# churchill-lab/alntools

Hardware: AMD Instinct MI355X
Metric: alignments/sec BAM->EC (100M PE reads, 8-hap) at 1/2/4/8 MI355X (higher is better)
Workload: dtype u32

## Files before the change

### alntools_amd/csrc/ecb.hip

```cpp
#include <hip/hip_runtime.h>

#include <algorithm>
#include <climits>
#include <cstddef>
#include <cstdarg>
#include <cstdio>
#include <cstring>
#include <cstdlib>
#include <memory>
#include <mutex>
#include <string>
#include <vector>

#include "../../include/ecb.h"

namespace {

typedef unsigned long long u64;
typedef unsigned int u32;
typedef unsigned short u16;

constexpr int TPB = 256;
constexpr u32 MAX_PROBE = 256;
constexpr u32 PENDING = 0xFFFFFFFFu;
// ... 50 lines not shown
__device__ __forceinline__ u64 arena_alloc(Counters* ctr, u64 arena_cap, u32 n, u32 hint) {
    const u32 R = arena_regions(arena_cap);
    const u64 per = arena_cap / R;
    for (u32 t = 0; t < R; ++t) {
        const u32 r = (hint + t) % R;
        const u64 at = atomicAdd(&ctr->arena_reg[r], (u64)n);
        if (at + n <= (u64)(r + 1) * per) return at;
    }
    return ~0ull;
}

__device__ __forceinline__ u32 fmix32(u32 h) {
    h ^= h >> 16; h *= 0x85EBCA6Bu;
    h ^= h >> 13; h *= 0xC2B2AE35u;
    h ^= h >> 16;
    return h;
}
__device__ __forceinline__ u64 pair_hash64(u32 locus, u32 mask) {
    const u32 h0 = fmix32(locus * 0x9E3779B1u + mask * 0x85EBCA77u + 0x7F4A7C15u);
    const u32 h1 = fmix32((h0 ^ locus) * 0xC2B2AE3Du + mask);
    return ((u64)h1 << 32) | h0;
}
__device__ __forceinline__ u64 finish_hash(u64 s0, u32 n) { return (s0 + ((u64)n << 32) + n) | 1ull; }

__device__ __forceinline__ bool rec_valid(u32 hf) {
    if (hf & 0x4u) return false;
    if (hf & 0x1u) {
        if ((hf & 0x80u) || !(hf & 0x2u) || (hf & (ECB_FLAG_MATE_OTHER_REF | ECB_FLAG_NEXT_POS_NEG))) return false;
    }
    return true;
}

enum { ST_NONE = 0, ST_LOOK, ST_HIT, ST_CREATED, ST_PENDING, ST_FULL, ST_OTHER, ST_STUCK };
enum { CMP_EQUAL = 0, CMP_DIFFERENT, CMP_INCOMPLETE, CMP_UNSURE };
struct SlotView { u32 n, off; uint2 p[INL]; };

__device__ __forceinline__ u64 fresh64(u64* p) { return atomicOr(p, 0ull); }
__device__ __forceinline__ void store_wt64(u64* p, u64 v) { __hip_atomic_store(p, v, __ATOMIC_RELAXED, __HIP_MEMORY_SCOPE_AGENT); }
__device__ __forceinline__ u64 pack2(uint2 v) { return ((u64)v.y << 32) | v.x; }
__device__ __forceinline__ uint2 unpack2(u64 v) { return make_uint2((u32)v, (u32)(v >> 32)); }
__device__ __forceinline__ void publish_key(Slot* s, u32 n1, u32 off) { store_wt64(reinterpret_cast<u64*>(&s->n1), ((u64)off << 32) | n1); }
__device__ __forceinline__ uint2 key_pair(const Slot& s, const uint2* arena, u32 i) { return i < INL ? s.pair[i] : arena[(u64)s.off + (i - INL)]; }
__device__ __forceinline__ uint2 key_pair_fresh(Slot* s, uint2* arena, u32 off, u32 i) {
    return unpack2(fresh64(reinterpret_cast<u64*>(i < INL ? &s->pair[i] : arena + ((u64)off + (i - INL)))));
}

__device__ __forceinline__ SlotView make_view(uint4 a, uint4 b, uint4 c, uint4 d) {
    SlotView v;
    v.n = a.z - 1u; v.off = a.w;
    v.p[0] = make_uint2(b.z, b.w); v.p[1] = make_uint2(c.x, c.y); v.p[2] = make_uint2(c.z, c.w);
    v.p[3] = make_uint2(d.x, d.y); v.p[4] = make_uint2(d.z, d.w);
    return v;
}
constexpr u32 RANKED_MAX = 16;
template <class F>
__device__ __forceinline__ void ranked_pairs(const SlotView& v, const uint2* arena, F&& emit) {
    const u32 sn = v.n;
    u32 X[RANKED_MAX], Y[RANKED_MAX];
#pragma unroll
    for (u32 i = 0; i < INL; ++i) { X[i] = i < sn ? v.p[i].x : 0xFFFFFFFFu; Y[i] = v.p[i].y; }
    if (sn <= INL) {
#pragma unroll
        for (u32 i = 0; i < INL; ++i) {
            u32 r = 0;
#pragma unroll
            for (u32 j = 0; j < INL; ++j) r += X[j] < X[i] ? 1u : 0u;
            if (i < sn) emit(r, X[i], Y[i]);
        }
    } else {
#pragma unroll
        for (u32 k = 0; k < RANKED_MAX - INL; ++k) {
            const uint2 t = INL + k < sn ? arena[(u64)v.off + k] : make_uint2(0xFFFFFFFFu, 0u);
            X[INL + k] = t.x; Y[INL + k] = t.y;
        }
#pragma unroll
        for (u32 i = 0; i < RANKED_MAX; ++i) {
            u32 r = 0;
#pragma unroll
            for (u32 j = 0; j < RANKED_MAX; ++j) r += X[j] < X[i] ? 1u : 0u;
            if (i < sn) emit(r, X[i], Y[i]);
        }
    }
}
constexpr u32 BIG_LDS = 2048;
template <class F>
__device__ __forceinline__ void ranked_pairs_wave(const Slot& s, const uint2* arena, u32 sn, u32* sx, u32 lane, F&& emit) {
    const bool in_lds = sn <= BIG_LDS;
    if (in_lds) {
        for (u32 i = lane; i < sn; i += 64) sx[i] = key_pair(s, arena, i).x;
        __builtin_amdgcn_fence(__ATOMIC_ACQ_REL, "wavefront");
        __builtin_amdgcn_wave_barrier();
    }
    for (u32 i = lane; i < sn; i += 64) {
        const uint2 pi = key_pair(s, arena, i);
        u32 r = 0;
        if (in_lds) {
            u32 j = 0;
            for (; j + 4u <= sn; j += 4u) {
                const uint4 v = *reinterpret_cast<const uint4*>(&sx[j]);
                r += (v.x < pi.x ? 1u : 0u) + (v.y < pi.x ? 1u : 0u) + (v.z < pi.x ? 1u : 0u) + (v.w < pi.x ? 1u : 0u);
            }
            for (; j < sn; ++j) r += sx[j] < pi.x ? 1u : 0u;
        } else {
            for (u32 j = 0; j < sn; ++j) r += key_pair(s, arena, j).x < pi.x;
        }
        emit(r, pi.x, pi.y);
    }
    if (in_lds) {
        __builtin_amdgcn_fence(__ATOMIC_ACQ_REL, "wavefront");
        __builtin_amdgcn_wave_barrier();
    }
}
template <class Cmp>
__device__ __forceinline__ int table_lookup(Slot* table, u64 cap_mask, u64 lo, u64& j, u32& probes, const Cmp& cmp, u32 abl = 0u, u32* first_inv_seen = nullptr) {
    for (; probes < MAX_PROBE; ++probes, j = (j + 1) & cap_mask) {
        Slot* s = table + j;
        const uint4* q = reinterpret_cast<const uint4*>(s);
        if (first_inv_seen) *first_inv_seen = 0u;
        uint4 a = q[0], b = a, c = a, d = a;
        if (!(abl & 16u)) { b = q[1]; c = q[2]; d = q[3]; }
        u64 clo = ((u64)a.y << 32) | a.x;
        if (clo == 0ull) {
            clo = atomicCAS(&s->lo, 0ull, lo);
            if (clo == 0ull) return ST_CREATED;
            if (clo == lo) return ST_PENDING;
            continue;
        }
        if (clo != lo) continue;
        if (a.z == 0u) return ST_PENDING;
        if (a.z == DEAD_KEY) continue;
        if (first_inv_seen) *first_inv_seen = b.y;
        if (abl & 8u) return ST_HIT;
        const int r = cmp.quick(make_view(a, b, c, d));
        if (r == CMP_EQUAL) return ST_HIT;
        if (r != CMP_DIFFERENT) return ST_PENDING;
    }
    return ST_FULL;
}
template <class Cmp>
__device__ __forceinline__ int table_settle(Slot* s, const Cmp& cmp) {
    for (u32 spin = 0; spin < SPIN_MAX; ++spin) {
        const u64 w = fresh64(reinterpret_cast<u64*>(&s->n1));
        const u32 n1 = (u32)w;
        if (n1 == DEAD_KEY) return ST_OTHER;
        if (n1) {
            const int r = cmp.full(s, n1 - 1u, (u32)(w >> 32));
            if (r == CMP_EQUAL) return ST_HIT;
            if (r == CMP_DIFFERENT) return ST_OTHER;
        }
        __builtin_amdgcn_s_sleep(4);
    }
    return ST_STUCK;
}

#ifndef ECB_RPL
#define ECB_RPL 8
#endif
constexpr int RPL = ECB_RPL;
static_assert(RPL == 8, "only 8 records per lane is validated (16 was measured: 233 VGPRs, 2 waves/SIMD, 11-25 % slower; it also needs a 32-bit ent[])");
constexpr int NG = RPL / 4;
constexpr int WT = 64 * RPL;
constexpr int NWAVE = TPB / 64;
struct StreamCold {
    uint2* arena; u64 arena_cap;
    u64* queue; u64 queue_cap;
    u64* resume;
    u32* wave_counts;
    u64* wave_arena;
    u64* timing;
    u64 chunk;
    u32 prev_rid;
    const int* pos; int2* rng; u32 n_loci, n_haps;
};
__device__ __forceinline__ void queue_defer(Counters* ctr, const StreamCold* C, u64 head) {
    const u32 st = (u32)((head * 0x9E3779B97F4A7C15ull) >> 58);
    static_assert(QSTRIPES == 64, "six bits of the hash pick the stripe");
    const u64 seg = C->queue_cap / QSTRIPES;
    const u64 qi = atomicAdd(&ctr->n_queue_s[st], 1ull);
    if (qi < seg) C->queue[(u64)st * seg + qi] = head; else atomicOr(&ctr->err, ERR_QUEUE);
}
#ifdef ECB_ABLATE_RT
#define ABL(A, bits) ((A).ablate & (bits))
#else
#define ABL(A, bits) 0u
#endif
struct StreamArgs {
    const u32* rid; const u32* loc; const u32* hf;
    u64 n;
    Slot* table; u64 cap_mask;
    Counters* ctr;
    u32* read_slot;
    u64 reads_hi;
    const StreamCold* cold;
    u32 ablate;
    const int* pos; int2* rng;
};
__device__ __forceinline__ u32 stream_tw(const u32* rid, const u32* loc, const u32* hf) { return (loc == rid + 512 && hf == rid + 1024) ? 1536u : 512u; }
#define A_TW(A) stream_tw((A).rid, (A).loc, (A).hf)
__host__ __device__ __forceinline__ u64 rec_at(u64 i, u32 tw) { return (i >> 9) * (u64)tw + (i & 511ull); }

__device__ __forceinline__ void wave_sync() {
    __builtin_amdgcn_fence(__ATOMIC_ACQ_REL, "wavefront");
    __builtin_amdgcn_wave_barrier();
}
template <int CTRL, int ROW_MASK>
__device__ __forceinline__ u32 dpp_add(u32 v) { return v + (u32)__builtin_amdgcn_update_dpp(0, (int)v, CTRL, ROW_MASK, 0xf, false); }
__device__ __forceinline__ u32 wave_incl_scan(u32 v) {
    v = dpp_add<0x111, 0xf>(v); v = dpp_add<0x112, 0xf>(v); v = dpp_add<0x114, 0xf>(v); v = dpp_add<0x118, 0xf>(v);
    v = dpp_add<0x142, 0xa>(v);
    v = dpp_add<0x143, 0xc>(v);
    return v;
}
__device__ __forceinline__ u32 wave_sum(u32 v) { return (u32)__builtin_amdgcn_readlane((int)wave_incl_scan(v), 63); }
__device__ __forceinline__ u32 lane_above(u32 v) { return (u32)__builtin_amdgcn_update_dpp(0, (int)v, 0x138, 0xf, 0xf, false); }
__device__ __forceinline__ int clamp04(int x, int, int) { return min(max(x, 0), 4); }

struct TileRegs { u32 rr[RPL], ll[RPL], hh[RPL]; };


#ifdef ECB_TIMING
#define TICK(i) do { const u64 t_ = __builtin_readcyclecounter(); tacc[i] += t_ - tlast; tlast = t_; } while (0)
#else
#define TICK(i) do { } while (0)
#endif

__device__ __forceinline__ u64 tile_head(const u32* rid, u64 b, u64 e, u32 rd, u32 tw) {
    while (b < e) { const u64 m = b + ((e - b) >> 1); if ((int)(rid[rec_at(m, tw)] - rd) < 0) b = m + 1; else e = m; }
    return b;
}
__device__ __forceinline__ void load_tile(const StreamArgs& A, u64 tb, u64 te, u32 lane, TileRegs& R) {
    typedef unsigned int u32x4 __attribute__((ext_vector_type(4)));
    tb = ((u64)(u32)__builtin_amdgcn_readfirstlane((int)(u32)(tb >> 32)) << 32) | (u32)__builtin_amdgcn_readfirstlane((int)(u32)tb);
    if (tb + (u64)WT <= te) {
        const u64 tbw = (tb >> 9) * (u64)A_TW(A);
        const char* pr = reinterpret_cast<const char*>(A.rid + tbw);
        const char* pl = reinterpret_cast<const char*>(A.loc + tbw);
        const char* ph = reinterpret_cast<const char*>(A.hf + tbw);
        const u32 off = lane * 16u;
#pragma unroll
        for (int g = 0; g < NG; ++g) {
            u32x4 v = __builtin_nontemporal_load(reinterpret_cast<const u32x4*>(pr + (off + (u32)g * 1024u)));
            R.rr[4 * g] = v.x; R.rr[4 * g + 1] = v.y; R.rr[4 * g + 2] = v.z; R.rr[4 * g + 3] = v.w;
            v = __builtin_nontemporal_load(reinterpret_cast<const u32x4*>(pl + (off + (u32)g * 1024u)));
            R.ll[4 * g] = v.x; R.ll[4 * g + 1] = v.y; R.ll[4 * g + 2] = v.z; R.ll[4 * g + 3] = v.w;
            v = __builtin_nontemporal_load(reinterpret_cast<const u32x4*>(ph + (off + (u32)g * 1024u)));
            R.hh[4 * g] = v.x; R.hh[4 * g + 1] = v.y; R.hh[4 * g + 2] = v.z; R.hh[4 * g + 3] = v.w;
        }
        return;
    }
#pragma unroll
    for (int g = 0; g < NG; ++g) {
        const u64 i0 = tb + (u64)g * 256 + 4u * lane;
#pragma unroll
        for (int j = 0; j < 4; ++j) {
            const bool in = i0 + j < te;
            R.rr[4 * g + j] = A.rid[rec_at(in ? i0 + j : te - 1, A_TW(A))];
            R.ll[4 * g + j] = in ? A.loc[rec_at(i0 + j, A_TW(A))] : 0u;
            R.hh[4 * g + j] = in ? A.hf[rec_at(i0 + j, A_TW(A))] : 0x4u;
        }
    }
}

__device__ __forceinline__ void load_pos(const int* pos, u64 tb, u64 te, u32 lane, int* P) {
    typedef int i32x4 __attribute__((ext_vector_type(4)));
    tb = ((u64)(u32)__builtin_amdgcn_readfirstlane((int)(u32)(tb >> 32)) << 32) | (u32)__builtin_amdgcn_readfirstlane((int)(u32)tb);
    if (tb + (u64)WT <= te) {
        const char* pp = reinterpret_cast<const char*>(pos + tb);
        const u32 off = lane * 16u;
#pragma unroll
        for (int g = 0; g < NG; ++g) {
            const i32x4 v = __builtin_nontemporal_load(reinterpret_cast<const i32x4*>(pp + (off + (u32)g * 1024u)));
            P[4 * g] = v.x; P[4 * g + 1] = v.y; P[4 * g + 2] = v.z; P[4 * g + 3] = v.w;
        }
        return;
    }
#pragma unroll
    for (int g = 0; g < NG; ++g) {
        const u64 i0 = tb + (u64)g * 256 + 4u * lane;
#pragma unroll
        for (int j = 0; j < 4; ++j) P[4 * g + j] = i0 + j < te ? pos[i0 + j] : 0;
    }
}

#define ECB_KS_SHORT 0
#define ECB_KS_PAR 0
namespace ks_std {
#include "k_stream.inc"
}
#undef ECB_KS_SHORT
#define ECB_KS_SHORT 1
namespace ks_short {
#include "k_stream.inc"
}
#undef ECB_KS_SHORT
#undef ECB_KS_PAR
#define ECB_KS_SHORT 0
#define ECB_KS_PAR 1
namespace ks_par {
#include "k_stream.inc"
}
#undef ECB_KS_PAR
#undef ECB_KS_SHORT

__global__ void k_init_resume(u64* resume, u64 slices, u64 chunk, Counters* ctr = nullptr) {
    const u64 b = blockIdx.x * (u64)blockDim.x + threadIdx.x;
    if (b < slices) { resume[2 * b] = b * chunk; resume[2 * b + 1] = b * chunk; }
    if (b == 0 && ctr) { ctr->n_queue = 0; ctr->full = 0; ctr->next_slice = 0; }
    if (b < QSTRIPES && ctr) ctr->n_queue_s[b] = 0;
}

__global__ __launch_bounds__(1024) void k_sum_counts(const u32* wave_counts, u64 waves, Counters* ctr, u32 verify, u64 offered, u64 queue_cap, const u32* d_last = nullptr) {
    __shared__ u64 s[3][16];
    u64 a = 0, v = 0, e = 0;
    for (u64 i = threadIdx.x; i < waves; i += 1024) { a += wave_counts[3 * i]; v += wave_counts[3 * i + 1]; e += wave_counts[3 * i + 2]; }
#pragma unroll
    for (int d = 32; d > 0; d >>= 1) { a += __shfl_xor(a, d); v += __shfl_xor(v, d); e += __shfl_xor(e, d); }
    if ((threadIdx.x & 63u) == 0) { s[0][threadIdx.x >> 6] = a; s[1][threadIdx.x >> 6] = v; s[2][threadIdx.x >> 6] = e; }
    __syncthreads();
    if (threadIdx.x == 0) {
        a = v = e = 0;
        for (int k = 0; k < 16; ++k) { a += s[0][k]; v += s[1][k]; e += s[2][k]; }
        if (verify) ctr->n_mismatch += e;
        else { ctr->all += offered; ctr->valid += v; ctr->n_ecs += e; ctr->n_probe_tiles += a; }
        if (d_last) ctr->last_rid = *d_last;
        u64 nq = 0;
        for (u32 st = 0; st < QSTRIPES; ++st) nq += min(ctr->n_queue_s[st], queue_cap / QSTRIPES);
        ctr->n_queue = nq;
    }
}
__global__ void k_queue_compact(const u64* queue, u64 queue_cap, const Counters* ctr, u64* out) {
    const u64 seg = queue_cap / QSTRIPES;
    u64 at = 0;
    for (u32 st = 0; st < blockIdx.x; ++st) at += min(ctr->n_queue_s[st], seg);
    const u64 n = min(ctr->n_queue_s[blockIdx.x], seg);
    for (u64 i = threadIdx.x; i < n; i += blockDim.x) out[at + i] = queue[(u64)blockIdx.x * seg + i];
}

constexpr u32 BIN_BITS = 14;
constexpr u32 MAX_BIN_BITS = 15;
constexpr u32 MIN_BIN_BITS = 11;
constexpr u32 MAX_BUCKETS = 8192;
static_assert(MAX_BIN_BITS <= 16, "a slot's index within its range is kept in 16 bits (k_part_scatter*, k_count_bins)");

constexpr int TPB_PART = 1024;
constexpr u32 PART_G = 512;
__device__ __forceinline__ u64 part_per(u64 n_reads, u64 G) { return (((n_reads + G - 1) / G) + 3ull) & ~3ull; }
__global__ __launch_bounds__(TPB_PART) void k_part_hist(const u32* read_slot, u64 n_reads, u32 n_buckets, u32 bb, u32* hist) {
    extern __shared__ u32 sh[];
    const u64 G = gridDim.x, g = blockIdx.x, per = part_per(n_reads, G);
    const u64 r0 = min(g * per, n_reads), r1 = min(r0 + per, n_reads);
    for (u32 b = threadIdx.x; b < n_buckets; b += TPB_PART) sh[b] = 0;
    __syncthreads();
    const u64 a0 = min((r0 + 3) & ~3ull, r1), a1 = max(r1 & ~3ull, a0);
    for (u64 r = r0 + threadIdx.x; r < a0; r += TPB_PART) { const u32 s = read_slot[r]; if (s != PENDING) atomicAdd(&sh[s >> bb], 1u); }
    for (u64 r = a0 + 4ull * threadIdx.x; r < a1; r += 4ull * TPB_PART) {
        const uint4 v = *reinterpret_cast<const uint4*>(read_slot + r);
        if (v.x != PENDING) atomicAdd(&sh[v.x >> bb], 1u);
        if (v.y != PENDING) atomicAdd(&sh[v.y >> bb], 1u);
        if (v.z != PENDING) atomicAdd(&sh[v.z >> bb], 1u);
        if (v.w != PENDING) atomicAdd(&sh[v.w >> bb], 1u);
    }
    for (u64 r = a1 + threadIdx.x; r < r1; r += TPB_PART) { const u32 s = read_slot[r]; if (s != PENDING) atomicAdd(&sh[s >> bb], 1u); }
    __syncthreads();
    for (u32 b = threadIdx.x; b < n_buckets; b += TPB_PART) hist[(u64)b * G + g] = sh[b];
}

__global__ __launch_bounds__(TPB_PART) void k_part_scatter(const u32* read_slot, u64 n_reads, u32 n_buckets, u32 bb, const u32* offs,
                                                      u16* pairs) {
    extern __shared__ u32 sh[];
    const u64 G = gridDim.x, g = blockIdx.x, per = part_per(n_reads, G);
    const u64 r0 = min(g * per, n_reads), r1 = min(r0 + per, n_reads);
    for (u32 b = threadIdx.x; b < n_buckets; b += TPB_PART) sh[b] = offs[(u64)b * G + g];
    __syncthreads();
    for (u64 rb = r0; rb < r1; rb += 4 * TPB_PART) {
        u32 s[4], pos[4];
        u64 r[4];
#pragma unroll
        for (int k = 0; k < 4; ++k) {
            r[k] = rb + (u64)k * TPB_PART + threadIdx.x;
            s[k] = r[k] < r1 ? read_slot[r[k]] : PENDING;
        }
#pragma unroll
        for (int k = 0; k < 4; ++k) if (s[k] != PENDING) pos[k] = atomicAdd(&sh[s[k] >> bb], 1u);
#pragma unroll
        for (int k = 0; k < 4; ++k) if (s[k] != PENDING) pairs[pos[k]] = (u16)(s[k] & ((1u << bb) - 1u));
    }
}

constexpr u32 STAGE = 8 * TPB_PART;
constexpr u32 STAGE_MAX_BUCKETS = 4096;
__global__ __launch_bounds__(TPB_PART) void k_part_scatter_staged(const u32* read_slot, u64 n_reads, u32 n_buckets, u32 bb, const u32* offs,
                                                             u16* pairs) {
    extern __shared__ u32 sh[];
    u32 *cnt = sh, *start = sh + n_buckets, *gcur = sh + 2 * n_buckets;
    u32* stage = sh + 3 * n_buckets;
    __shared__ u32 s_wave[TPB_PART / 64];
    const u64 G = gridDim.x, g = blockIdx.x, per = part_per(n_reads, G);
    const u64 r0 = min(g * per, n_reads), r1 = min(r0 + per, n_reads);
    const u32 tid = threadIdx.x, lane = tid & 63u, w = tid >> 6;
    const u32 bpt = (n_buckets + TPB_PART - 1) / TPB_PART;
    for (u32 b = tid; b < n_buckets; b += TPB_PART) gcur[b] = offs[(u64)b * G + g];
    for (u64 rb = r0; rb < r1; rb += STAGE) {
        for (u32 b = tid; b < n_buckets; b += TPB_PART) cnt[b] = 0;
        __syncthreads();
        u32 s[8], lr[8];
#pragma unroll
        for (int k4 = 0; k4 < 2; ++k4) {
            const u64 r = rb + ((u64)k4 * TPB_PART + tid) * 4u;
            if (r + 4 <= r1) {
                const uint4 v = *reinterpret_cast<const uint4*>(read_slot + r);
                s[4 * k4] = v.x; s[4 * k4 + 1] = v.y; s[4 * k4 + 2] = v.z; s[4 * k4 + 3] = v.w;
            } else {
#pragma unroll
                for (int j = 0; j < 4; ++j) s[4 * k4 + j] = r + j < r1 ? read_slot[r + j] : PENDING;
            }
        }
#pragma unroll
        for (int k = 0; k < 8; ++k) if (s[k] != PENDING) lr[k] = atomicAdd(&cnt[s[k] >> bb], 1u);
        __syncthreads();
        u32 mine = 0;
        for (u32 j = 0; j < bpt; ++j) { const u32 b = tid * bpt + j; mine += b < n_buckets ? cnt[b] : 0u; }
        const u32 incl = wave_incl_scan(mine);
        if (lane == 63) s_wave[w] = incl;
        __syncthreads();
        u32 run = incl - mine;
        for (u32 k = 0; k < w; ++k) run += s_wave[k];
        for (u32 j = 0; j < bpt; ++j) { const u32 b = tid * bpt + j; if (b < n_buckets) { start[b] = run; run += cnt[b]; } }
        __syncthreads();
#pragma unroll
        for (int k = 0; k < 8; ++k)
            if (s[k] != PENDING) stage[start[s[k] >> bb] + lr[k]] = s[k];
        __syncthreads();
        u32 n_here = 0;
        for (u32 k = 0; k < TPB_PART / 64; ++k) n_here += s_wave[k];
        for (u32 i = tid; i < n_here; i += TPB_PART) {
            const u32 e = stage[i];
            const u32 b = e >> bb;
            pairs[gcur[b] + (i - start[b])] = (u16)(e & ((1u << bb) - 1u));
        }
        __syncthreads();
        for (u32 b = tid; b < n_buckets; b += TPB_PART) gcur[b] += cnt[b];
    }
}

constexpr int TPB_COUNT = 1024;
struct CountWork { u32 bucket, start, end, shared; };
__global__ __launch_bounds__(1024) void k_build_work(const u32* offs, u32 G, const u64* total, u32 n_buckets, u32 piece, CountWork* work, u32 max_work, u32* n_work) {
    __shared__ u32 s_w[16];
    __shared__ u32 s_carry;
    const u32 tid = threadIdx.x, lane = tid & 63u, w = tid >> 6;
    if (tid == 0) s_carry = 0;
    __syncthreads();
    for (u32 b0 = 0; b0 < n_buckets; b0 += 1024) {
        const u32 b = b0 + tid;
        u32 s0 = 0, s1 = 0, np = 0;
        if (b < n_buckets) { s0 = offs[(u64)b * G]; s1 = b + 1 < n_buckets ? offs[(u64)(b + 1) * G] : (u32)*total; }
        const u32 len = s1 - s0;
        const bool cut = len > piece + piece / 2;
        if (len) np = cut ? (len + piece - 1) / piece : 1u;
        const u32 incl = wave_incl_scan(np);
        if (lane == 63) s_w[w] = incl;
        __syncthreads();
        u32 at = s_carry + incl - np, tot = 0;
        for (u32 k = 0; k < 16; ++k) { if (k < w) at += s_w[k]; tot += s_w[k]; }
        for (u32 k = 0; k < np; ++k)
            if (at + k < max_work) work[at + k] = cut ? CountWork{b, s0 + k * piece, min(s0 + (k + 1) * piece, s1), 1u} : CountWork{b, s0, s1, 0u};
        __syncthreads();
        if (tid == 0) s_carry += tot;
        __syncthreads();
    }
    if (tid == 0) *n_work = min(s_carry, max_work);
}
struct CompactSink { u32* list; u64 max_list; u64* n_list; u32* bitmap; u64 n_bits; uint2* list_fn; };
__global__ __launch_bounds__(TPB_COUNT) void k_count_bins(const u16* pairs, const CountWork* work, const u32* n_work, u32 bb, Slot* table, CompactSink sink) {
    extern __shared__ u32 cnt[];
    const u32 N_BINS = 1u << bb;
    if (blockIdx.x >= *n_work) return;
    const CountWork wk = work[blockIdx.x];
    const u32 b = wk.bucket, lane = threadIdx.x & 63u;
    const u32 start = wk.start, end = wk.end;
    for (u32 q = threadIdx.x; q < N_BINS; q += TPB_COUNT) cnt[q] = 0;
    __syncthreads();
    auto add = [&](u32 bin, bool have) {
        const u64 hm = __ballot(have);
        if (!hm) return;
        const u32 v = (u32)__builtin_amdgcn_readlane((int)bin, __ffsll((long long)hm) - 1);
        const bool same = have && bin == v;
        const u64 m = __ballot(same);
        if (__popcll(m) >= 8) {
            if (lane == (u32)(__ffsll((long long)m) - 1)) atomicAdd(&cnt[v], (u32)__popcll(m));
            if (have && !same) atomicAdd(&cnt[bin], 1u);
        } else if (have) {
            atomicAdd(&cnt[bin], 1u);
        }
    };
    const u32 a0 = min((start + 7u) & ~7u, end), a1 = max(end & ~7u, a0);
    { const u32 i = start + threadIdx.x; const bool have = i < a0; add(have ? (u32)pairs[i] : 0u, have); }
    { const u32 i = a1 + threadIdx.x; const bool have = i < end; add(have ? (u32)pairs[i] : 0u, have); }
    for (u32 i0 = a0; i0 < a1; i0 += 32 * TPB_COUNT) {
        uint4 pv[4];
#pragma unroll
        for (int k = 0; k < 4; ++k) {
            const u32 i = i0 + (k * TPB_COUNT + threadIdx.x) * 8u;
            pv[k] = i < a1 ? *reinterpret_cast<const uint4*>(pairs + i) : make_uint4(0u, 0u, 0u, 0u);
        }
#pragma unroll
        for (int k = 0; k < 4; ++k) {
            const bool have = i0 + (k * TPB_COUNT + threadIdx.x) * 8u < a1;
            const u32 w[4] = {pv[k].x, pv[k].y, pv[k].z, pv[k].w};
#pragma unroll
            for (int j = 0; j < 8; ++j) add((w[j >> 1] >> (16 * (j & 1))) & 0xFFFFu, have);
        }
    }
    __syncthreads();
    const bool once = sink.list && !wk.shared;
    u32 mine = 0;
    for (u32 q = threadIdx.x; q < N_BINS; q += TPB_COUNT) {
        const u32 c = cnt[q];
        u32 first = 0;
        if (once) first = c != 0u;
        else if (c) {
            Slot* s = table + (((u64)b << bb) | q);
            if (wk.shared) first = atomicAdd(&s->count, c) == 0u;
            else { s->count += c; first = 1u; }
        }
        if (sink.list && !once) cnt[q] = first;
        mine += first;
    }
    if (!sink.list) return;
    __shared__ u32 s_wtot[TPB_COUNT / 64];
    __shared__ u64 s_base;
    const u32 incl = wave_incl_scan(mine);
    if (lane == 63) s_wtot[threadIdx.x >> 6] = incl;
    __syncthreads();
    if (threadIdx.x == 0) {
        u32 run = 0;
        for (int k = 0; k < TPB_COUNT / 64; ++k) { const u32 c = s_wtot[k]; s_wtot[k] = run; run += c; }
        s_base = run ? atomicAdd(sink.n_list, (u64)run) : 0ull;
    }
    __syncthreads();
    u64 at = s_base + s_wtot[threadIdx.x >> 6] + (incl - mine);
    if (once) {
        for (u32 q0 = threadIdx.x; q0 < N_BINS; q0 += 8 * TPB_COUNT) {
            u32 c[8];
            uint2 vk[8], vc[8];
#pragma unroll
            for (int k = 0; k < 8; ++k) { const u32 q = q0 + k * TPB_COUNT; c[k] = q < N_BINS ? cnt[q] : 0u; }
#pragma unroll
            for (int k = 0; k < 8; ++k)
                if (c[k]) {
                    const Slot* sl = table + (((u64)b << bb) | (q0 + k * TPB_COUNT));
                    vk[k] = *reinterpret_cast<const uint2*>(&sl->n1); vc[k] = *reinterpret_cast<const uint2*>(&sl->count);
                }
#pragma unroll
            for (int k = 0; k < 8; ++k) {
                if (!c[k]) continue;
                const u64 i = ((u64)b << bb) | (q0 + k * TPB_COUNT);
                table[i].count = vc[k].x + c[k];
                if (at < sink.max_list) {
                    sink.list[at] = (u32)i;
                    if (sink.list_fn) {
                        const u32 f = ~vc[k].y;
                        sink.list_fn[at] = make_uint2(f, vk[k].x - 1u);
                        if (f < sink.n_bits) atomicOr(&sink.bitmap[f >> 5], 1u << (f & 31u));
                    }
                }
                ++at;
            }
        }
        return;
    }
    for (u32 q = threadIdx.x; q < N_BINS; q += TPB_COUNT) {
        if (!cnt[q]) continue;
        const u64 i = ((u64)b << bb) | q;
        if (at < sink.max_list) {
            const Slot* s = table + i;
            sink.list[at] = (u32)i;
            if (sink.list_fn) {
                const u32 f = ~s->first_inv;
                sink.list_fn[at] = make_uint2(f, s->n1 - 1u);
                if (f < sink.n_bits) atomicOr(&sink.bitmap[f >> 5], 1u << (f & 31u));
            }
        }
        ++at;
    }
}

__global__ __launch_bounds__(TPB) void k_slow_len(const u32* rid, u64 n, const u64* queue, u64 nq, u64* len, u32 tw) {
    const u64 q = blockIdx.x;
    if (q >= nq) return;
    __shared__ u64 s_end;
    const u64 h = queue[q];
    const u32 r0 = rid[rec_at(h, tw)];
    if (threadIdx.x == 0) s_end = n;
    __syncthreads();
    for (u64 b = h; b < n; b += TPB) {
        const u64 i = b + threadIdx.x;
        if (i < n && rid[rec_at(i, tw)] != r0) atomicMin(&s_end, i);
        __syncthreads();
        const bool found = (s_end != n);
        __syncthreads();
        if (found) break;
    }
    __syncthreads();
    if (threadIdx.x == 0) len[q] = s_end - h;
}

struct SlowArgs {
    const u32* rid; const u32* loc; const u32* hf;
    const u64* queue; const u64* len; const u64* scr_off;
    u32* scr_key; u32* scr_mask;
    u32 n_loci, n_haps;
    Slot* table; u64 cap_mask;
    uint2* arena; u64 arena_cap;
    Counters* ctr;
    u32* read_slot; u64 reads_hi;
    u64* requeue; u64* n_requeue;
    u32 verify;
};

__device__ __forceinline__ u64 slow_probe_start(u32 lc, u64 cap2) { return __umul64hi((u64)(lc * 0x9E3779B1u) << 32, cap2); }

constexpr u32 SLOW_LDS = 4096;
template <bool IN_LDS> __device__ __forceinline__ u32 slow_ld(const u32* p) {
    if constexpr (IN_LDS) return *p; else return __hip_atomic_load(p, __ATOMIC_RELAXED, __HIP_MEMORY_SCOPE_AGENT);
}
template <bool IN_LDS>
__device__ __forceinline__ void slow_body(const SlowArgs& A, u32* key, u32* msk, const u64 q, const u64 h, const u64 L) {
    const u32 tid = threadIdx.x, lane = tid & 63u;
    const u64 cap2 = 2 * L;
    if (IN_LDS) {
        for (u32 p = tid; p < (u32)cap2; p += TPB) { key[p] = 0; msk[p] = 0; }
        __syncthreads();
    }
    __shared__ u64 s_acc[TPB / 64];
    __shared__ u32 s_n[TPB / 64];
    __shared__ u64 s_lo, s_j;
    __shared__ u32 s_np, s_st, s_n1, s_off, s_cnt, s_diff, s_inc, s_probes;

    for (u64 i = tid; i < L; i += TPB) {
        const u32 f = A.hf[rec_at(h + i, A_TW(A))];
        if (!rec_valid(f)) continue;
        const u32 lc = A.loc[rec_at(h + i, A_TW(A))], hap = (f >> ECB_HAP_SHIFT) & 0xFFu;
        if (lc >= A.n_loci || hap >= A.n_haps) { atomicOr(&A.ctr->err, ERR_RANGE); continue; }
        u64 p = slow_probe_start(lc, cap2);
        for (;;) {
            const u32 old = atomicCAS(&key[p], 0u, lc + 1u);
            if (old == 0u || old == lc + 1u) { atomicOr(&msk[p], 1u << hap); break; }
            if (++p == cap2) p = 0;
        }
    }
    if (!IN_LDS) __threadfence();
    __syncthreads();
    u64 a0 = 0;
    u32 np = 0;
    for (u64 p = tid; p < cap2; p += TPB) {
        const u32 k = slow_ld<IN_LDS>(&key[p]);
        if (k) {
            const u32 m = slow_ld<IN_LDS>(&msk[p]);
            ++np;
            a0 += pair_hash64(k - 1u, m);
        }
    }
#pragma unroll
    for (int d = 32; d > 0; d >>= 1) a0 += __shfl_xor(a0, d);
    np = wave_sum(np);
    if (lane == 0) { s_acc[tid >> 6] = a0; s_n[tid >> 6] = np; }
    __syncthreads();
    const u32 r0 = A.rid[rec_at(h, A_TW(A))];
    if (tid == 0) {
        a0 = 0; np = 0;
        for (int w = 0; w < TPB / 64; ++w) { a0 += s_acc[w]; np += s_n[w]; }
        s_np = np; s_lo = finish_hash(a0, np); s_j = s_lo & A.cap_mask; s_probes = 0; s_cnt = 0;
        if ((u64)r0 >= A.reads_hi) { atomicOr(&A.ctr->err, ERR_CONTRACT); s_st = ST_NONE; }
        else s_st = ST_PENDING;
    }
    __syncthreads();
    np = s_np;
    auto same_key = [&]() -> int {
        for (u32 spin = 0; spin < SPIN_MAX; ++spin) {
            __syncthreads();
            if (tid == 0) {
                const u64 w = fresh64(reinterpret_cast<u64*>(&A.table[s_j].n1));
                s_n1 = (u32)w; s_off = (u32)(w >> 32); s_diff = 0; s_inc = 0;
            }
            __syncthreads();
            const u32 n1 = s_n1;
            if (n1 == DEAD_KEY) return CMP_DIFFERENT;
            if (n1 == 0u) { __builtin_amdgcn_s_sleep(8); continue; }
            const u32 n = n1 - 1u;
            if (n != np) return CMP_DIFFERENT;
            Slot* sl = A.table + s_j;
            bool diff = false, inc = false;
            for (u32 i = tid; i < n && !diff && !inc; i += TPB) {
                u64* src = reinterpret_cast<u64*>(i < INL ? &sl->pair[i] : A.arena + ((u64)s_off + (i - INL)));
                uint2 pr = unpack2(*src);
                if (pr.y == 0u) pr = unpack2(fresh64(src));
                if (pr.y == 0u) { inc = true; break; }
                diff = true;
                if (pr.x < A.n_loci) {
                    u64 p = slow_probe_start(pr.x, cap2);
                    for (u64 t = 0; t < cap2; ++t) {
                        const u32 k = slow_ld<IN_LDS>(&key[p]);
                        if (k == pr.x + 1u) { diff = slow_ld<IN_LDS>(&msk[p]) != pr.y; break; }
                        if (k == 0u) break;
                        if (++p == cap2) p = 0;
                    }
                }
            }
            if (diff) atomicOr(&s_diff, 1u);
            if (inc) atomicOr(&s_inc, 1u);
            __syncthreads();
            if (s_diff) return CMP_DIFFERENT;
            if (!s_inc) return CMP_EQUAL;
            __builtin_amdgcn_s_sleep(8);
        }
        return CMP_INCOMPLETE;
    };
    if (A.verify) {
        if (s_st != ST_NONE) {
            if (tid == 0) s_j = A.read_slot[r0];
            __syncthreads();
            const bool same = s_j != (u64)PENDING && same_key() == CMP_EQUAL;
            if (tid == 0 && !same) atomicAdd(&A.ctr->n_mismatch, 1ull);
        }
    } else {
        for (u32 round = 0; round < 4 * MAX_PROBE && s_st == ST_PENDING; ++round) {
            __syncthreads();
            if (tid == 0) {
                u64 j = s_j; u32 probes = s_probes;
                struct Defer { __device__ int quick(const SlotView&) const { return CMP_UNSURE; } };
                const int st = table_lookup(A.table, A.cap_mask, s_lo, j, probes, Defer());
                s_j = j; s_probes = probes; s_st = (u32)st; s_off = 0; s_n1 = 0;
                if (st == ST_CREATED) {
                    u64 off = 0;
                    if (np > INL) off = arena_alloc(A.ctr, A.arena_cap, np - INL, blockIdx.x);
                    atomicAdd(&A.ctr->n_ecs, 1ull);
                    s_off = (u32)off;
                    if (off == ~0ull) { atomicOr(&A.ctr->err, ERR_ARENA); s_n1 = DEAD_KEY; }
                } else if (st == ST_FULL) {
                    A.requeue[atomicAdd(A.n_requeue, 1ull)] = h;
                }
            }
            __syncthreads();
            if (s_st == ST_PENDING) {
                const int r = same_key();
                __syncthreads();
                if (tid == 0) {
                    if (r == CMP_EQUAL) { s_st = ST_HIT; A.read_slot[r0] = (u32)s_j; atomicMax(&A.table[s_j].first_inv, ~r0); }
                    else if (r == CMP_INCOMPLETE) { s_st = ST_NONE; atomicOr(&A.ctr->err, ERR_INTERNAL); }
                    else { s_j = (s_j + 1) & A.cap_mask; s_probes += 1; if (s_probes >= MAX_PROBE) { s_st = ST_FULL; A.requeue[atomicAdd(A.n_requeue, 1ull)] = h; } }
                }
// ... 24 lines not shown
    if (!IN_LDS) for (u64 p = tid; p < cap2; p += TPB) {
        if (slow_ld<IN_LDS>(&key[p])) { key[p] = 0; msk[p] = 0; }
    }
}
__global__ __launch_bounds__(TPB) void k_slow(SlowArgs A) {
    extern __shared__ u32 sh_scr[];
    const u64 q = blockIdx.x;
    const u64 h = A.queue[q], L = A.len[q];
    if (2 * L <= (u64)SLOW_LDS) slow_body<true>(A, sh_scr, sh_scr + SLOW_LDS, q, h, L);
    else slow_body<false>(A, A.scr_key + A.scr_off[q], A.scr_mask + A.scr_off[q], q, h, L);
}

__global__ void k_rehash(const Slot* old_t, u64 old_cap, Slot* new_t, u64 new_mask, u32* new_of_old) {
    for (u64 i = blockIdx.x * (u64)blockDim.x + threadIdx.x; i < old_cap; i += (u64)gridDim.x * blockDim.x) {
        const Slot s = old_t[i];
        if (!s.n1) continue;
        u64 j = s.lo & new_mask;
        for (;; j = (j + 1) & new_mask) {
            if (atomicCAS(&new_t[j].lo, 0ull, s.lo) == 0ull) {
                Slot t = s;
                uint4* d = reinterpret_cast<uint4*>(new_t + j);
                const uint4* v = reinterpret_cast<const uint4*>(&t);
                d[1] = v[1]; d[2] = v[2]; d[3] = v[3];
                new_t[j].off = s.off; new_t[j].n1 = s.n1;
                new_of_old[i] = (u32)j;
                break;
            }
        }
    }
}

__global__ void k_remap_read_slot(u32* read_slot, u64 n_reads, const u32* new_of_old) {
    for (u64 r = blockIdx.x * (u64)blockDim.x + threadIdx.x; r < n_reads; r += (u64)gridDim.x * blockDim.x) {
        const u32 os = read_slot[r];
        if (os != PENDING) read_slot[r] = new_of_old[os];
    }
}

constexpr int TPB_COMPACT = 1024;
__global__ __launch_bounds__(TPB_COMPACT) void k_compact(const Slot* table, u64 cap, u32* list, u64 max_list, u64* n_list,
                                                         u32* bitmap, u64 n_bits, uint2* list_fn) {
    __shared__ u32 s_w[TPB_COMPACT / 64];
    __shared__ u64 s_base;
    const u32 tid = threadIdx.x, lane = tid & 63u, w = tid >> 6;
    for (u64 b = (u64)blockIdx.x * 4 * TPB_COMPACT; b < cap; b += (u64)gridDim.x * 4 * TPB_COMPACT) {
        u32 occ = 0, off[4], tot = 0;
#pragma unroll
        for (int k = 0; k < 4; ++k) {
            const u64 i = b + (u64)k * TPB_COMPACT + tid;
            const bool o = i < cap && table[i].n1 != 0u;
            const u64 m = __ballot(o);
            off[k] = tot + __builtin_amdgcn_mbcnt_hi((u32)(m >> 32), __builtin_amdgcn_mbcnt_lo((u32)m, 0u));
            tot += (u32)__popcll(m);
            occ |= (u32)o << k;
        }
        if (lane == 0) s_w[w] = tot;
        __syncthreads();
        if (tid == 0) {
            u32 run = 0;
            for (int k = 0; k < TPB_COMPACT / 64; ++k) { const u32 c = s_w[k]; s_w[k] = run; run += c; }
            s_base = run ? atomicAdd(n_list, (u64)run) : 0ull;
        }
        __syncthreads();
        const u64 base = s_base + s_w[w];
#pragma unroll
        for (int k = 0; k < 4; ++k)
            if ((occ >> k & 1u) && base + off[k] < max_list) {
                const u64 i = b + (u64)k * TPB_COMPACT + tid;
                list[base + off[k]] = (u32)i;
                if (list_fn) {
                    const u32 f = ~table[i].first_inv;
                    list_fn[base + off[k]] = make_uint2(f, table[i].n1 - 1u);
                    if (f < n_bits) atomicOr(&bitmap[f >> 5], 1u << (f & 31u));
                }
            }
        __syncthreads();
    }
}

__global__ void k_list_fn(const Slot* table, const u32* list, u64 max_list, const u64* n_list, u64* n_out, u32* bitmap, u64 n_bits, uint2* list_fn) {
    const u64 e = blockIdx.x * (u64)blockDim.x + threadIdx.x;
    const u64 n = *n_list;
    if (e == 0) *n_out = n;
    if (e >= n || e >= max_list) return;
    const Slot* s = table + list[e];
    const u32 f = ~s->first_inv;
    list_fn[e] = make_uint2(f, s->n1 - 1u);
    if (f < n_bits) atomicOr(&bitmap[f >> 5], 1u << (f & 31u));
}

constexpr u32 MAX_PARTS = 64;
__device__ __forceinline__ u32 part_of(u64 lo, u32 n_parts) { return (u32)((lo >> 40) % n_parts); }

constexpr u32 PARTS_PER_BLOCK = 16 * TPB;
__global__ __launch_bounds__(TPB) void k_parts_count(const Slot* table, const u32* list, u64 n, u32 n_parts, u64* cnt) {
    __shared__ u32 ce[MAX_PARTS], cp[MAX_PARTS];
    if (threadIdx.x < MAX_PARTS) { ce[threadIdx.x] = 0; cp[threadIdx.x] = 0; }
    __syncthreads();
    const u64 e0 = blockIdx.x * (u64)PARTS_PER_BLOCK, e1 = min(e0 + PARTS_PER_BLOCK, n);
    for (u64 eb = e0; eb < e1; eb += TPB) {
        const u64 e = eb + threadIdx.x;
        u32 q = MAX_PARTS, np = 0;
        if (e < e1) { const Slot& s = table[list[e]]; q = part_of(s.lo, n_parts); np = s.n1 - 1u; }
        for (u32 t = 0; t < n_parts; ++t) {
            const u64 m = __ballot(q == t);
            if (!m) continue;
            const u32 tot = wave_sum(q == t ? np : 0u);
            if ((threadIdx.x & 63u) == 0) { atomicAdd(&ce[t], (u32)__popcll(m)); atomicAdd(&cp[t], tot); }
        }
    }
    __syncthreads();
    if (threadIdx.x < n_parts) {
        if (ce[threadIdx.x]) atomicAdd(&cnt[threadIdx.x], (u64)ce[threadIdx.x]);
        if (cp[threadIdx.x]) atomicAdd(&cnt[n_parts + threadIdx.x], (u64)cp[threadIdx.x]);
    }
}
constexpr u32 EXPORT_SMALL = RANKED_MAX;
__global__ __launch_bounds__(TPB) void k_parts_export(const Slot* table, const u32* list, u64 n, const uint2* arena, u32 n_parts,
                                                      u64* cur, const u64* pair_base, Entry* out_e, uint2* out_p, u32 read_base,
                                                      u64* big, u32* n_big) {
    __shared__ u32 ce[MAX_PARTS], cp[MAX_PARTS];
    __shared__ u64 be[MAX_PARTS], bp[MAX_PARTS];
    const u32 lane = threadIdx.x & 63u;
    const u64 e0 = blockIdx.x * (u64)PARTS_PER_BLOCK, e1 = min(e0 + PARTS_PER_BLOCK, n);
    for (int pass = 0; pass < 2; ++pass) {
        if (threadIdx.x < MAX_PARTS) { ce[threadIdx.x] = 0; cp[threadIdx.x] = 0; }
        __syncthreads();
        for (u64 eb = e0; eb < e1; eb += TPB) {
            const u64 e = eb + threadIdx.x;
            uint4 sa = make_uint4(0u, 0u, 1u, 0u), sb = sa, sc = sa, sd = sa;
            u32 q = MAX_PARTS, re = 0, rp = 0, sn = 0;
            if (e < e1) {
                const uint4* sl = reinterpret_cast<const uint4*>(table + list[e]);
                sa = sl[0]; sb = sl[1]; sc = sl[2]; sd = sl[3];
                q = part_of(((u64)sa.y << 32) | sa.x, n_parts); sn = sa.z - 1u;
            }
            for (u32 t = 0; t < n_parts; ++t) {
                const bool mine = q == t;
                const u64 m = __ballot(mine);
                if (!m) continue;
                const u32 v = mine ? sn : 0u, incl = wave_incl_scan(v);
                const u32 tot = (u32)__builtin_amdgcn_readlane((int)incl, 63);
                u32 b_e = 0, b_p = 0;
                if (lane == 0) { b_e = atomicAdd(&ce[t], (u32)__popcll(m)); b_p = atomicAdd(&cp[t], tot); }
                b_e = (u32)__builtin_amdgcn_readfirstlane((int)b_e); b_p = (u32)__builtin_amdgcn_readfirstlane((int)b_p);
                if (mine) { re = b_e + __builtin_amdgcn_mbcnt_hi((u32)(m >> 32), __builtin_amdgcn_mbcnt_lo((u32)m, 0u)); rp = b_p + incl - v; }
            }
            if (pass == 1 && e < e1) {
                const u64 po = bp[q] + rp;
                if (sn <= EXPORT_SMALL) {
                    ranked_pairs(make_view(sa, sb, sc, sd), arena, [&](u32 r, u32 x, u32 y) { out_p[po + r] = make_uint2(x, y); });
                } else {
                    const u32 bi = atomicAdd(n_big, 1u);
                    big[2 * (u64)bi] = po; big[2 * (u64)bi + 1] = ((u64)list[e] << 32) | sn;
                }
                Entry en;
                en.lo = ((u64)sa.y << 32) | sa.x; en.reserved = 0; en.count = sb.x;
                en.first_inv = ~(~sb.y + read_base);
                en.off = (u32)(po - pair_base[q]); en.n = sn;
                out_e[be[q] + re] = en;
            }
        }
        __syncthreads();
        if (pass == 0 && threadIdx.x < n_parts) {
            be[threadIdx.x] = ce[threadIdx.x] ? atomicAdd(&cur[threadIdx.x], (u64)ce[threadIdx.x]) : 0ull;
            bp[threadIdx.x] = cp[threadIdx.x] ? atomicAdd(&cur[n_parts + threadIdx.x], (u64)cp[threadIdx.x]) : 0ull;
        }
        __syncthreads();
    }
}
__global__ __launch_bounds__(TPB) void k_parts_sort_big(const Slot* table, const uint2* arena, const u64* big, u32 n_big, uint2* out_p) {
    __shared__ __attribute__((aligned(16))) u32 sx[TPB / 64][BIG_LDS];
    const u32 b = (blockIdx.x * TPB + threadIdx.x) >> 6, lane = threadIdx.x & 63u;
    if (b >= n_big) return;
    const u64 po = big[2 * (u64)b];
    const u32 n = (u32)big[2 * (u64)b + 1];
    const Slot& s = table[big[2 * (u64)b + 1] >> 32];
    ranked_pairs_wave(s, arena, n, sx[threadIdx.x >> 6], lane, [&](u32 r, u32 x, u32 y) { out_p[po + r] = make_uint2(x, y); });
}
__global__ void k_adopt(const Entry* ent, u64 n, const uint2* pairs, Slot* table, u64 slot_base, u32 arena_base) {
    const u64 e = blockIdx.x * (u64)blockDim.x + threadIdx.x;
    if (e >= n) return;
    const Entry en = ent[e];
    Slot s{};
    s.lo = en.lo; s.n1 = en.n + 1u; s.off = arena_base + en.off + INL; s.count = en.count; s.first_inv = en.first_inv;
    for (u32 i = 0; i < INL && i < en.n; ++i) s.pair[i] = pairs[(u64)en.off + i];
    table[slot_base + e] = s;
}

struct ListCmp {
    const uint2* inc; u32 n; uint2* arena;
    __device__ __forceinline__ int quick(const SlotView& v) const { return v.n != n ? CMP_DIFFERENT : CMP_UNSURE; }
    __device__ __noinline__ int full(Slot* s, u32 sn, u32 off) const {
        if (sn != n) return CMP_DIFFERENT;
        bool same = true, inc_ = false;
        for (u32 i = 0; i < n && same; ++i) {
            const uint2 a = key_pair_fresh(s, arena, off, i), b = inc[i];
            inc_ |= a.y == 0u;
            same = a.x == b.x && a.y == b.y;
        }
        if (same) return CMP_EQUAL;
        if (inc_) return CMP_INCOMPLETE;
        for (u32 i = 0; i < n; ++i) {
            const uint2 a = key_pair_fresh(s, arena, off, i);
            if (a.y == 0u) return CMP_INCOMPLETE;
            bool found = false;
            for (u32 k = 0; k < n && !found; ++k) found = inc[k].x == a.x && inc[k].y == a.y;
            if (!found) return CMP_DIFFERENT;
        }
        return CMP_EQUAL;
    }
};
constexpr u32 MERGE_PER_BLOCK = 2 * TPB;
struct MergeDesc { const Entry* ent; const uint2* pairs; u64 n, n_pairs; };
__global__ __launch_bounds__(TPB) void k_merge(const MergeDesc* D, Slot* table, u64 cap_mask, uint2* arena, u64 arena_cap, Counters* ctr,
                                               u32* list, u64 list_cap, u64* n_list) {
    const MergeDesc d = D[blockIdx.y];
    const Entry* const ent = d.ent; const uint2* const pairs = d.pairs;
    const u64 n = d.n, n_pairs = d.n_pairs;
    if (blockIdx.x * (u64)MERGE_PER_BLOCK >= n) return;
    __shared__ u32 s_new;
    __shared__ u32 s_found[MERGE_PER_BLOCK];
    __shared__ u32 s_nfound;
    __shared__ u64 s_lbase;
    if (threadIdx.x == 0) { s_new = 0; s_nfound = 0; }
    __syncthreads();
    const u32 lane = threadIdx.x & 63u;
    const u64 e0 = blockIdx.x * (u64)MERGE_PER_BLOCK, e1 = min(e0 + MERGE_PER_BLOCK, n);
    u32 my_new = 0;
    for (u64 eb = e0; eb < e1; eb += TPB) {
        const u64 e = eb + threadIdx.x;
        const bool on = e < e1;
        Entry s{};
        if (on) s = ent[e];
        const bool ok = on && (u64)s.off + s.n <= n_pairs && s.lo != 0ull;
        if (on && !ok) atomicOr(&ctr->err, ERR_CONTRACT);
        ListCmp cmp{pairs + s.off, s.n, arena};
        u64 j = s.lo & cap_mask;
        u32 probes = 0;
        int st = ST_NONE;
        if (ok) st = table_lookup(table, cap_mask, s.lo, j, probes, cmp);
        bool created = false;
        for (u32 round = 0;; ++round) {
            const u64 cm = __ballot(st == ST_CREATED);
            if (cm) {
                const bool cr = st == ST_CREATED;
                const u32 want = cr && s.n > INL ? s.n - INL : 0u;
                u64 at = 0;
                if (__ballot(want != 0u)) {
                    const u32 incl = wave_incl_scan(want);
                    const u32 total = (u32)__builtin_amdgcn_readlane((int)incl, 63);
                    if (lane == 0) at = arena_alloc(ctr, arena_cap, total, (blockIdx.y * gridDim.x + blockIdx.x) * (TPB / 64) + (threadIdx.x >> 6));
                    at = ((u64)(u32)__builtin_amdgcn_readfirstlane((int)(u32)(at >> 32)) << 32) | (u32)__builtin_amdgcn_readfirstlane((int)(u32)at);
                    if (at == ~0ull) { if (lane == 0) atomicOr(&ctr->err, ERR_ARENA); }
                    else at += incl - want;
                }
                my_new += (u32)__popcll(cm);
                if (list) {
                    const int first = __ffsll((long long)cm) - 1;
                    u32 lb = 0;
                    if ((int)lane == first) lb = atomicAdd(&s_nfound, (u32)__popcll(cm));
                    lb = (u32)__builtin_amdgcn_readlane((int)lb, first);
                    if (cr) s_found[lb + __builtin_amdgcn_mbcnt_hi((u32)(cm >> 32), __builtin_amdgcn_mbcnt_lo((u32)cm, 0u))] = (u32)j;
                }
                if (cr) {
                    const bool dead = at == ~0ull;
                    if (!dead)
                        for (u32 t = 0; t < s.n; ++t) {
                            uint2* dst = t < INL ? &table[j].pair[t] : arena + (at + (t - INL));
                            store_wt64(reinterpret_cast<u64*>(dst), pack2(pairs[(u64)s.off + t]));
                        }
                    publish_key(table + j, dead ? DEAD_KEY : s.n + 1u, (u32)at);
                    st = ST_HIT; created = true;
                }
            }
            if (!__ballot(st == ST_PENDING)) break;
            if (round >= 64u) { if (st == ST_PENDING) { atomicOr(&ctr->err, ERR_INTERNAL); st = ST_NONE; } break; }
            if (st == ST_PENDING) {
                const int r = table_settle(table + j, cmp);
                if (r == ST_HIT) st = ST_HIT;
                else if (r == ST_STUCK) { atomicOr(&ctr->err, ERR_INTERNAL); st = ST_NONE; }
                else { j = (j + 1) & cap_mask; ++probes; st = table_lookup(table, cap_mask, s.lo, j, probes, cmp); }
            }
        }
        (void)created;
        if (st == ST_FULL) atomicAdd(&ctr->n_queue, 1ull);
        else if (st == ST_HIT) {
            atomicAdd(&table[j].count, s.count);
            atomicMax(&table[j].first_inv, s.first_inv);
        }
    }
    if (lane == 0 && my_new) atomicAdd(&s_new, my_new);
    __syncthreads();
    if (threadIdx.x == 0 && s_new) atomicAdd(&ctr->n_ecs, (u64)s_new);
    if (list) {
        if (threadIdx.x == 0) s_lbase = s_nfound ? atomicAdd(n_list, (u64)s_nfound) : 0ull;
        __syncthreads();
        for (u32 i = threadIdx.x; i < s_nfound; i += TPB) if (s_lbase + i < list_cap) list[s_lbase + i] = s_found[i];
    }
}

constexpr u32 BM_LINE = 16;
inline u64 bitmap_words(u64 n_bits) { return ((n_bits + 31) / 32 + BM_LINE) / BM_LINE * BM_LINE; }
__global__ void k_popc(const u32* in, u64 n_lines, u32* out) {
    const u64 i = blockIdx.x * (u64)blockDim.x + threadIdx.x;
    if (i >= n_lines) return;
    const uint4* q = reinterpret_cast<const uint4*>(in + i * BM_LINE);
    u32 c = 0;
#pragma unroll
    for (int k = 0; k < (int)BM_LINE / 4; ++k) { const uint4 v = q[k]; c += __popc(v.x) + __popc(v.y) + __popc(v.z) + __popc(v.w); }
    out[i] = c;
}
__device__ __forceinline__ u32 bit_rank(const u32* bitmap, const u32* lprefix, u32 f) {
    const uint4* q = reinterpret_cast<const uint4*>(bitmap + ((f >> 5) & ~(BM_LINE - 1u)));
    const uint4 v0 = q[0], v1 = q[1], v2 = q[2], v3 = q[3];
    const u32 w[BM_LINE] = {v0.x, v0.y, v0.z, v0.w, v1.x, v1.y, v1.z, v1.w, v2.x, v2.y, v2.z, v2.w, v3.x, v3.y, v3.z, v3.w};
    const u32 k = (f >> 5) & (BM_LINE - 1u), below = (1u << (f & 31u)) - 1u;
    u32 r = lprefix[f >> 9];
    static_assert(BM_LINE == 16, "f >> 9: 512 bits per line");
#pragma unroll
    for (u32 i = 0; i < BM_LINE; ++i) r += __popc(w[i] & (i < k ? 0xFFFFFFFFu : i == k ? below : 0u));
    return r;
}

constexpr int SCB_TPB = 1024, SCB_ITEMS = 16, SCB = SCB_TPB * SCB_ITEMS;
constexpr u64 SC_AGG = 1ull << 62, SC_PFX = 2ull << 62, SC_VAL = (1ull << 62) - 1ull;
inline u64 scan_blocks(u64 n) { return std::max<u64>(1, (n + SCB - 1) / SCB); }
inline u64 scan_words(u64 n) { return 2 * (scan_blocks(n) + 2); }
__global__ __launch_bounds__(SCB_TPB) void k_scan_lb(const u32* in, u64 n, u32* out, u64* st, u64 nb, u64* d_total, u32 stride, u32* last32) {
    __shared__ u64 s_b, s_excl;
    __shared__ u32 s_w[SCB_TPB / 64];
    const u32 tid = threadIdx.x, lane = tid & 63u, w = tid >> 6;
    if (tid == 0) s_b = atomicAdd(reinterpret_cast<unsigned long long*>(&st[nb]), 1ull);
    __syncthreads();
    const u64 b = s_b;
    if (b >= nb) return;
    const u64 base = b * SCB + (u64)tid * SCB_ITEMS;
    u32 v[SCB_ITEMS];
    const bool whole = base + SCB_ITEMS <= n;
    if (stride == 1u && whole && (reinterpret_cast<uintptr_t>(in) & 15u) == 0u) {
#pragma unroll
        for (int k = 0; k < SCB_ITEMS / 4; ++k) {
            const uint4 q = reinterpret_cast<const uint4*>(in + base)[k];
            v[4 * k] = q.x; v[4 * k + 1] = q.y; v[4 * k + 2] = q.z; v[4 * k + 3] = q.w;
        }
    } else {
#pragma unroll
        for (int k = 0; k < SCB_ITEMS; ++k) v[k] = base + k < n ? in[(base + k) * stride] : 0u;
    }
    u32 s = 0;
#pragma unroll
    for (int k = 0; k < SCB_ITEMS; ++k) s += v[k];
    const u32 incl = wave_incl_scan(s);
    if (lane == 63) s_w[w] = incl;
    __syncthreads();
    u32 before = 0, tot = 0;
#pragma unroll
    for (u32 k = 0; k < SCB_TPB / 64; ++k) { const u32 c = s_w[k]; if (k < w) before += c; tot += c; }
    if (w == 0) {
        u64 excl = 0;
        if (lane == 0) __hip_atomic_store(&st[b], (b == 0 ? SC_PFX : SC_AGG) | (u64)tot, __ATOMIC_RELAXED, __HIP_MEMORY_SCOPE_AGENT);
        if (b > 0) {
            long long t = (long long)b - 1;
            for (u32 spins = 0; spins < (1u << 24);) {
                const long long idx = t - (long long)lane;
                const u64 x = idx >= 0 ? __hip_atomic_load(&st[idx], __ATOMIC_RELAXED, __HIP_MEMORY_SCOPE_AGENT) : SC_PFX;
                const u64 ready = __ballot(x != 0ull), pfx = __ballot(x >= SC_PFX);
                u64 take = 0;
                if (pfx) {
                    const int p = __ffsll((long long)pfx) - 1;
                    const u64 need = p == 63 ? ~0ull : (1ull << (p + 1)) - 1ull;
                    if ((ready & need) == need) take = need;
                } else if (ready == ~0ull) take = ~0ull;
                if (!take) { ++spins; __builtin_amdgcn_s_sleep(1); continue; }
                u64 val = (take >> lane & 1ull) ? (x & SC_VAL) : 0ull;
#pragma unroll
                for (int d = 32; d > 0; d >>= 1) val += __shfl_xor(val, d);
                excl += val;
                if (pfx) break;
                t -= 64;
            }
            if (lane == 0) __hip_atomic_store(&st[b], SC_PFX | ((excl + tot) & SC_VAL), __ATOMIC_RELAXED, __HIP_MEMORY_SCOPE_AGENT);
        }
        if (lane == 0) {
            s_excl = excl;
            if (b + 1 == nb && d_total) *d_total = excl + tot;
            if (b + 1 == nb && last32) *last32 = (u32)(excl + tot);
        }
    }
    __syncthreads();
    u32 run = (u32)s_excl + before + incl - s;
    if (whole && (reinterpret_cast<uintptr_t>(out) & 15u) == 0u) {
#pragma unroll
        for (int k = 0; k < SCB_ITEMS / 4; ++k) {
            uint4 q;
            q.x = run; run += v[4 * k]; q.y = run; run += v[4 * k + 1]; q.z = run; run += v[4 * k + 2]; q.w = run; run += v[4 * k + 3];
            reinterpret_cast<uint4*>(out + base)[k] = q;
        }
    } else {
#pragma unroll
        for (int k = 0; k < SCB_ITEMS; ++k) { if (base + k < n) out[base + k] = run; run += v[k]; }
    }
}
inline hipError_t scan_launch(hipStream_t st, const u32* in, u64 n, u32* out, u32* scratch, u64* d_total, u32 stride = 1, u32* last32 = nullptr) {
    const u64 nb = scan_blocks(n);
    u64* words = reinterpret_cast<u64*>(scratch);
    hipError_t e = hipMemsetAsync(words, 0, ((nb + 1) * 8 + 15) & ~15ull, st);
    if (e != hipSuccess) return e;
    k_scan_lb<<<(unsigned)nb, SCB_TPB, 0, st>>>(in, n, out, words, nb, d_total, stride, last32);
    return hipGetLastError();
}

__global__ void k_rank(const u32* list, const uint2* list_fn, u64 n, u64 n_bits, const u32* bitmap, const u32* wprefix,
                       uint2* ord2) {
    const u64 e = blockIdx.x * (u64)blockDim.x + threadIdx.x;
    if (e >= n) return;
    const u32 si = list[e];
    const uint2 fn = list_fn[e];
    const u32 f = fn.x;
    if (f >= n_bits) return;
    const u32 r = bit_rank(bitmap, wprefix, f);
    if (r >= n) return;
    ord2[r] = make_uint2(si, fn.y);
}
__global__ void k_slot_ranks(const u32* order, u64 n, u32* rank_of_slot) {
    const u64 r = blockIdx.x * (u64)blockDim.x + threadIdx.x;
    if (r < n) rank_of_slot[order[r]] = (u32)r;
}

constexpr u32 EMIT_SMALL = RANKED_MAX;
__global__ __launch_bounds__(TPB) void k_emit_small(const Slot* table, const uint2* ord2, u32* order, u64 n, const uint2* arena,
                                                     const u32* indptr, int* indices, int* data, int* counts,
                                                     u32 n_loci, u32 n_haps, u32* big, u32* n_big, Counters* ctr) {
    __shared__ u32 sx[TPB / 64][64 * EMIT_SMALL], sy[TPB / 64][64 * EMIT_SMALL];
    const u64 e = (u64)blockIdx.x * TPB + threadIdx.x;
    const u32 lane = threadIdx.x & 63u, w = threadIdx.x >> 6;
    const bool have = e < n;
    const u64 hm = __ballot(have);
    if (!hm) return;
    uint4 a = make_uint4(0u, 0u, 1u, 0u), b = a, c = a, d = a;
    u32 dst = 0;
    if (have) {
        const u32 si = ord2[e].x;
        order[e] = si;
        const uint4* q = reinterpret_cast<const uint4*>(table + si);
        a = q[0]; b = q[1]; c = q[2]; d = q[3];
        counts[e] = (int)b.x;
        dst = indptr[e];
    }
    const SlotView v = make_view(a, b, c, d);
    const bool is_big = have && v.n > EMIT_SMALL;
    if (is_big) big[atomicAdd(n_big, 1u)] = (u32)e;
    const u32 base = (u32)__builtin_amdgcn_readfirstlane((int)dst);
    const u32 end = (u32)__builtin_amdgcn_readlane((int)(dst + v.n), 63 - __builtin_clzll(hm));
    const bool staged = __ballot(is_big) == 0ull && end - base <= 64u * EMIT_SMALL;
    bool bad = false;
    if (!is_big)
        ranked_pairs(v, arena, [&](u32 r, u32 x, u32 y) {
            if (staged) { const u32 at = min(dst - base + r, 64u * EMIT_SMALL - 1u); sx[w][at] = x; sy[w][at] = y; }
            else { indices[dst + r] = (int)x; data[dst + r] = (int)y; }
            bad |= x >= n_loci || (y >> n_haps) != 0u;
        });
    if (staged) {
        wave_sync();
        for (u32 i = lane; i < end - base; i += 64u) { indices[base + i] = (int)sx[w][i]; data[base + i] = (int)sy[w][i]; }
    }
    if (bad) atomicOr(&ctr->err, ERR_RANGE);
}
__global__ __launch_bounds__(TPB) void k_emit_big(const Slot* table, const u32* order, const u32* big, const u32* n_big,
                                                   const uint2* arena, const u32* indptr, int* indices, int* data,
                                                   u32 n_loci, u32 n_haps, Counters* ctr) {
    __shared__ __attribute__((aligned(16))) u32 sx[TPB / 64][BIG_LDS];
    const u32 lane = threadIdx.x & 63u, w = threadIdx.x >> 6, nb = *n_big;
    bool bad = false;
    for (u32 b = (blockIdx.x * TPB + threadIdx.x) >> 6; b < nb; b += (gridDim.x * TPB) >> 6) {
        const u32 e = big[b];
        const Slot& s = table[order[e]];
        const u32 dst = indptr[e];
        ranked_pairs_wave(s, arena, s.n1 - 1u, sx[w], lane, [&](u32 r, u32 x, u32 y) {
            indices[dst + r] = (int)x;
            data[dst + r] = (int)y;
            bad |= x >= n_loci || (y >> n_haps) != 0u;
        });
    }
    if (bad) atomicOr(&ctr->err, ERR_RANGE);
}

constexpr u32 MS_FILE_BITS = 32 - ECB_CELL_BITS;
__host__ __device__ __forceinline__ u32 ms_swz(u32 meta) { return ((meta & ((1u << ECB_CELL_BITS) - 1u)) << MS_FILE_BITS) | (meta >> ECB_CELL_BITS); }
__host__ __device__ __forceinline__ u32 ms_unswz(u32 s) { return (s >> MS_FILE_BITS) | (s << ECB_CELL_BITS); }
__host__ __device__ __forceinline__ u64 ms_swz_key(u64 key) { return (key & 0xFFFFFFFF00000000ull) | ms_swz((u32)key); }
__global__ void k_ms_keys(const u32* read_slot, const u32* rank_of_slot, const u32* meta, u64 n, u64* keys, u32* vals) {
    const u64 i = blockIdx.x * (u64)blockDim.x + threadIdx.x;
    if (i < n) { keys[i] = ((u64)rank_of_slot[read_slot[i]] << 32) | ms_swz(meta[i]); vals[i] = (u32)i; }
}
__global__ void k_ms_swz_keys(u64* keys, u64 n) {
    const u64 i = blockIdx.x * (u64)blockDim.x + threadIdx.x;
    if (i < n) keys[i] = ms_swz_key(keys[i]);
}
__global__ void k_run_heads(const u64* keys, u64 n, u32* flag) {
    const u64 i = blockIdx.x * (u64)blockDim.x + threadIdx.x;
    if (i < n) flag[i] = (i == 0 || keys[i] != keys[i - 1]) ? 1u : 0u;
}
__global__ void k_ms_emit(const u64* keys, const u32* vals, const u32* flag, const u32* pos, u64 n, u32 n_out,
                          u64* okey, u32* ofirst, u32* ostart) {
    const u64 i = blockIdx.x * (u64)blockDim.x + threadIdx.x;
    if (i < n && flag[i]) { okey[pos[i]] = (keys[i] & 0xFFFFFFFF00000000ull) | ms_unswz((u32)keys[i]); ofirst[pos[i]] = vals[i]; ostart[pos[i]] = (u32)i; }
    if (i == 0) ostart[n_out] = (u32)n;
}
__global__ void k_ms_split(const u64* okey, const u32* ostart, const u32* ocount, u64 n, u32* ec, u32* meta, u32* count) {
    const u64 i = blockIdx.x * (u64)blockDim.x + threadIdx.x;
    if (i < n) { ec[i] = (u32)(okey[i] >> 32); meta[i] = (u32)okey[i]; count[i] = ocount ? ocount[i] : ostart[i + 1] - ostart[i]; }
}
__global__ void k_export_keys(const Slot* table, const u32* order, u64 n, u64* out) {
    const u64 e = blockIdx.x * (u64)blockDim.x + threadIdx.x;
    if (e < n) out[e] = table[order[e]].lo;
}
__global__ void k_row_keys(const u32* indptr, const int* indices, const int* data, u64 n, u64* out) {
    const u64 e = blockIdx.x * (u64)blockDim.x + threadIdx.x;
    if (e >= n) return;
    const u32 a = indptr[e], z = indptr[e + 1];
    u64 acc = 0;
    for (u32 i = a; i < z; ++i) acc += pair_hash64((u32)indices[i], (u32)data[i]);
    out[e] = finish_hash(acc, z - a);
}
__global__ void k_set_global_rank(const u64* keys, const int* indptr, const int* indices, const int* data, u64 n,
                                  const Slot* table, u64 cap_mask, const uint2* arena, u32* grank) {
    const u64 e = blockIdx.x * (u64)blockDim.x + threadIdx.x;
    if (e >= n) return;
    const u64 lo = keys[e];
    const u32 r0 = (u32)indptr[e], rn = (u32)indptr[e + 1] - r0;
    u64 j = lo & cap_mask;
    for (u64 probe = 0; probe <= cap_mask; ++probe, j = (j + 1) & cap_mask) {
        const Slot& s = table[j];
        if (s.lo == 0ull) return;
        if (s.lo != lo || s.n1 != rn + 1u) continue;
        bool same = true;
        for (u32 i = 0; i < rn && same; ++i) {
            const uint2 pr = key_pair(s, arena, i);
            u32 a = 0, b = rn;
            while (a < b) { const u32 m = (a + b) >> 1; if ((u32)indices[r0 + m] < pr.x) a = m + 1; else b = m; }
            same = a < rn && (u32)indices[r0 + a] == pr.x && (u32)data[r0 + a] == pr.y;
        }
        if (same) { grank[j] = (u32)e; return; }
    }
}
__global__ void k_ms_out(const u64* okey, const u32* ofirst, const u32* ostart, u64 n, u32 read_base, u64* key, u32* count, u32* first) {
    const u64 i = blockIdx.x * (u64)blockDim.x + threadIdx.x;
    if (i < n) { key[i] = okey[i]; count[i] = ostart[i + 1] - ostart[i]; first[i] = ofirst[i] + read_base; }
}
__global__ void k_ms_combine(const u64* keys, const u32* idx, const u32* flag, const u32* pos, u64 n, const u32* cnt_in, const u32* first_in,
                             u64* okey, u32* ocount, u32* ofirst) {
    const u64 i = blockIdx.x * (u64)blockDim.x + threadIdx.x;
    if (i >= n) return;
    const u32 o = pos[i] - (flag[i] ? 0u : 1u);
    if (flag[i]) okey[o] = (keys[i] & 0xFFFFFFFF00000000ull) | ms_unswz((u32)keys[i]);
    atomicAdd(&ocount[o], cnt_in[idx[i]]);
    atomicMin(&ofirst[o], first_in[idx[i]]);
}


__device__ __forceinline__ u64 lower_bound_u64(const u64* a, u64 n, u64 v) {
    u64 lo = 0, hi = n;
    while (lo < hi) { const u64 m = (lo + hi) >> 1; if (a[m] < v) lo = m + 1; else hi = m; }
    return lo;
}
constexpr u32 CVU_PIECE = 1536;
constexpr u32 CVU_MAX = 3072;
constexpr u32 CVU_TSZ = 4096;
constexpr u32 CVU_TPB = 512;
constexpr u32 CVU_K = CVU_MAX / CVU_TPB;
constexpr u32 CVB_ERR_PTR = 1u, CVB_ERR_EC = 2u, CVB_ERR_ORDER = 4u;
__global__ void k_cvb_last(const int* cscptr, u32 n_loci, u32 n_haps, int* last) {
    const u32 h = threadIdx.x;
    if (h < n_haps) last[h] = cscptr[(u64)h * (n_loci + 1) + n_loci];
}
__global__ void k_cvu_colsum(const int* cscptr, u32 n_loci, u32 n_haps, u32* S, u32* err) {
    const u64 l = blockIdx.x * (u64)blockDim.x + threadIdx.x;
    if (l > n_loci) return;
    u32 sum = 0, bad = 0;
    for (u32 h = 0; h < n_haps; ++h) {
        const int* ptr = cscptr + (u64)h * (n_loci + 1);
        const int v = ptr[l];
        if (v < 0 || (l == 0 && v != 0) || (l > 0 && ptr[l - 1] > v)) bad = CVB_ERR_PTR;
        sum += (u32)v;
    }
    S[l] = sum;
    if (bad) atomicOr(err, bad);
}
__global__ void k_cvu_pieces(const u32* S, u32 n_loci, u32* pieces) {
    const u64 l = blockIdx.x * (u64)blockDim.x + threadIdx.x;
    if (l >= n_loci) return;
    const u32 n = S[l + 1] - S[l];
    pieces[l] = n <= CVU_PIECE + CVU_PIECE / 2 ? (n ? 1u : 0u) : (n + CVU_PIECE - 1u) / CVU_PIECE;
}
__global__ void k_cvu_items(const u32* pieces, const u32* pbase, u32 n_loci, u32* item_col) {
    const u64 l = blockIdx.x * (u64)blockDim.x + threadIdx.x;
    if (l >= n_loci) return;
    const u32 n = pieces[l], at = pbase[l];
    for (u32 r = 0; r < n; ++r) item_col[at + r] = (u32)l;
}
__device__ __forceinline__ u32 cvu_width(u32 n_ecs, u32 np) { return (u32)(((u64)n_ecs + np - 1u) / np); }
__global__ void k_cvu_bounds(const int* cscptr, const int* cscidx, const u64* hs, const u32* pieces, const u32* pbase, const u32* item_col,
                             u32 n_items, u32 n_loci, u32 n_haps, u32 n_ecs, u32* bnd) {
    const u64 t = blockIdx.x * (u64)blockDim.x + threadIdx.x;
    if (t >= (u64)n_items * n_haps) return;
    const u32 i = (u32)(t / n_haps), h = (u32)(t % n_haps);
    const u32 l = item_col[i], np = pieces[l], r = i - pbase[l];
    const int* ptr = cscptr + (u64)h * (n_loci + 1);
    const u64 nh = hs[h + 1] - hs[h];
    u64 a = min((u64)(u32)ptr[l], nh), b = min((u64)(u32)ptr[l + 1], nh);
    if (r) {
        const u64 lo = (u64)r * cvu_width(n_ecs, np);
        const int* base = cscidx + hs[h];
        while (a < b) { const u64 m = a + ((b - a) >> 1); if ((u64)(u32)base[m] < lo) a = m + 1; else b = m; }
    }
    bnd[t] = (u32)a;
}
__device__ __forceinline__ bool cvb_contains(const int* cscptr, const int* cscidx, const u64* hs, u32 n_loci, u32 hh, u32 l, u32 e) {
    const int* p = cscptr + (u64)hh * (n_loci + 1);
    const u64 nh = hs[hh + 1] - hs[hh];
    u64 a = min((u64)(u32)p[l], nh), b = min((u64)(u32)p[l + 1], nh);
    const int* base = cscidx + hs[hh];
    while (a < b) { const u64 m = a + ((b - a) >> 1); const u32 v = (u32)base[m]; if (v < e) a = m + 1; else if (v > e) b = m; else return true; }
    return false;
}
template <bool EMIT>
__global__ __launch_bounds__(CVU_TPB) void k_cvu_union(const int* cscptr, const int* cscidx, const u64* hs, const u32* pieces, const u32* pbase,
                                                       const u32* item_col, const u32* bnd, u32 n_items, u32 n_loci, u32 n_haps, u32 n_ecs,
                                                       u32* colcnt, const u32* colbase, u32* colcur, u64 nnz, u64* keys, u32* vals, u32* err) {
    __shared__ u32 tkey[CVU_TSZ];
    __shared__ u32 tmask[CVU_TSZ];
    __shared__ u32 seg[64];
    __shared__ u32 segp[33];
    __shared__ u64 shs[32];
    __shared__ u32 s_n, s_base;
    const u32 i = blockIdx.x;
    const u32 l = item_col[i], np = pieces[l], r = i - pbase[l];
    const u32 w = cvu_width(n_ecs, np);
    const u32 e_lo = (u32)min((u64)r * w, (u64)n_ecs), e_hi = r + 1u == np ? n_ecs : (u32)min((u64)(r + 1u) * w, (u64)n_ecs);
    if (threadIdx.x < n_haps) {
        const u32 h = threadIdx.x;
        const u64 h0 = hs[h], nh = hs[h + 1] - h0;
        shs[h] = h0;
        seg[2 * h] = bnd[(u64)i * n_haps + h];
        seg[2 * h + 1] = r + 1u < np ? bnd[(u64)(i + 1u) * n_haps + h] : (u32)min((u64)(u32)cscptr[(u64)h * (n_loci + 1) + l + 1], nh);
    }
    if (threadIdx.x == 0) s_n = 0;
    __syncthreads();
    if (threadIdx.x == 0) { u32 run = 0; for (u32 h = 0; h < n_haps; ++h) { segp[h] = run; run += seg[2 * h + 1] - seg[2 * h]; } segp[n_haps] = run; }
    __syncthreads();
    const u32 tot = segp[n_haps];
    if (tot == 0) return;
    if (tot > CVU_MAX) {
        for (u32 h = 0; h < n_haps; ++h) {
            const int* base = cscidx + hs[h];
            for (u32 j = seg[2 * h] + threadIdx.x; j < seg[2 * h + 1]; j += CVU_TPB) {
                const u32 e = (u32)base[j];
                u32 bad = e >= n_ecs ? CVB_ERR_EC : 0u;
                if (e < e_lo || e >= e_hi || (j > seg[2 * h] && (u32)base[j - 1] >= e)) bad |= CVB_ERR_ORDER;
                if (bad) { atomicOr(err, bad); continue; }
                bool first = true;
                for (u32 hh = h; hh-- > 0 && first;) first = !cvb_contains(cscptr, cscidx, hs, n_loci, hh, l, e);
                if (!first) continue;
                if (!EMIT) { atomicAdd(&colcnt[l], 1u); continue; }
                u32 mask = 1u << h;
                for (u32 hh = h + 1; hh < n_haps; ++hh) if (cvb_contains(cscptr, cscidx, hs, n_loci, hh, l, e)) mask |= 1u << hh;
                const u64 pos = (u64)colbase[l] + atomicAdd(&colcur[l], 1u);
                if (pos < nnz) { keys[pos] = ((u64)e << 32) | l; vals[pos] = mask; }
            }
        }
        return;
    }
    u32 tsz = 64;
    while (tsz < CVU_TSZ && tsz < tot + tot / 3u + 1u) tsz <<= 1;
    static_assert(CVU_MAX < CVU_TSZ && (CVU_TSZ & (CVU_TSZ - 1u)) == 0, "a free slot is always found");
    u32 ev[CVU_K], hv[CVU_K];
#pragma unroll
    for (u32 k = 0; k < CVU_K; ++k) {
        const u32 u = threadIdx.x + k * CVU_TPB;
        hv[k] = 0xFFFFFFFFu; ev[k] = 0;
        if (u < tot) {
            u32 h = 0;
            while (segp[h + 1] <= u) ++h;
            hv[k] = h;
            ev[k] = (u32)cscidx[shs[h] + seg[2 * h] + (u - segp[h])];
        }
    }
    for (u32 q = threadIdx.x; q < tsz; q += CVU_TPB) { tkey[q] = 0xFFFFFFFFu; tmask[q] = 0u; }
    __syncthreads();
#pragma unroll
    for (u32 k = 0; k < CVU_K; ++k) {
        if (hv[k] == 0xFFFFFFFFu) continue;
        const u32 e = ev[k];
        if (e >= n_ecs) { atomicOr(err, CVB_ERR_EC); continue; }
        if (e < e_lo || e >= e_hi) { atomicOr(err, CVB_ERR_ORDER); continue; }
        u32 q = (e * 0x9E3779B1u) >> 7 & (tsz - 1u);
        for (u32 it = 0; it < tsz; ++it) {
            const u32 old = atomicCAS(&tkey[q], 0xFFFFFFFFu, e);
            if (old == 0xFFFFFFFFu || old == e) { atomicOr(&tmask[q], 1u << hv[k]); break; }
            q = (q + 1u) & (tsz - 1u);
        }
    }
    __syncthreads();
    u32 mine = 0;
    for (u32 q = threadIdx.x; q < tsz; q += CVU_TPB) mine += tkey[q] != 0xFFFFFFFFu ? 1u : 0u;
    const u32 at = mine ? atomicAdd(&s_n, mine) : 0u;
    __syncthreads();
    if (threadIdx.x == 0 && s_n) { if (EMIT) s_base = colbase[l] + atomicAdd(&colcur[l], s_n); else atomicAdd(&colcnt[l], s_n); }
    if (!EMIT) return;
    __syncthreads();
    u32 rnk = at;
    for (u32 q = threadIdx.x; q < tsz; q += CVU_TPB) {
        const u32 e = tkey[q];
        if (e == 0xFFFFFFFFu) continue;
        const u64 pos = (u64)s_base + rnk++;
        if (pos < nnz) { keys[pos] = ((u64)e << 32) | l; vals[pos] = tmask[q]; }
// ... 255 lines not shown
                if (done || used != k || t - k < 0) continue;
                if (v[k] < RS_AGG) continue;
                excl += v[k] & RS_VAL;
                used = k + 1;
                if (v[k] >= RS_PFX) done = true;
            }
            t -= used;
            if (!used) {
                if (++spins > RS_SPIN_MAX) { atomicOr(err, 1u); break; }
                __builtin_amdgcn_s_sleep(1);
            }
        }
        __hip_atomic_store(mine, RS_PFX | ((excl + tot) & RS_VAL), __ATOMIC_RELAXED, __HIP_MEMORY_SCOPE_AGENT);
    }
    if (dig) gbase[tid] = base[tid] + excl;
    {
        const u32 incl = wave_incl_scan(tot);
        if (lane == 63) s_wsum[w] = incl;
        __syncthreads();
        u32 before = 0;
        for (u32 k = 0; k < w; ++k) before += s_wsum[k];
        if (dig) dstart[tid] = before + incl - tot;
    }
    __syncthreads();
#pragma unroll
    for (int r = 0; r < RS_ITEMS; ++r) {
        const u64 i = w0 + (u64)r * 64 + lane;
        if (i < n) {
            const u32 d = (u32)(key[r] >> shift) & 255u;
            const u32 lp = dstart[d] + cnt[w][d] + rk[r];
            skey[lp] = key[r]; sval[lp] = val[r];
        }
    }
    __syncthreads();
    const u32 n_tile = (u32)min((u64)RS_TILE, n - t0);
    for (u32 i = tid; i < n_tile; i += RS_TPB) {
        const u64 k = skey[i];
        const u32 d = (u32)(k >> shift) & 255u;
        const u64 pos = (u64)gbase[d] + (i - dstart[d]);
        if (pos < n) { kout[pos] = k; vout[pos] = sval[i]; }
    }
}
__global__ __launch_bounds__(TPB) void k_or_reduce(const u64* keys, u64 n, u64* out) {
    u64 v = 0;
    for (u64 i = blockIdx.x * (u64)TPB + threadIdx.x; i < n; i += (u64)gridDim.x * TPB) v |= keys[i];
#pragma unroll
    for (int d = 32; d > 0; d >>= 1) v |= __shfl_xor(v, d);
    if ((threadIdx.x & 63u) == 0 && v) atomicOr(out, v);
}
constexpr u32 MSF_LDS_CELLS = 8192;
constexpr int TPB_MSF = 1024;
__global__ __launch_bounds__(TPB_MSF) void k_msf2_cells(const u32* meta, const u32* cnt, u64 n, u32 n_cells, u64* total, u32* firstfile, u32* err) {
    extern __shared__ u32 sh32[];
    const bool lds = n_cells <= MSF_LDS_CELLS;
    u32 *lfile = sh32, *lcnt = sh32 + (lds ? n_cells : 0);
    if (lds) {
        for (u32 c = threadIdx.x; c < n_cells; c += TPB_MSF) { lfile[c] = 0xFFFFFFFFu; lcnt[c] = 0; }
        __syncthreads();
    }
    const u64 per = (n + gridDim.x - 1) / gridDim.x, t0 = blockIdx.x * per, t1 = min(t0 + per, n);
    for (u64 t = t0 + threadIdx.x; t < t1; t += TPB_MSF) {
        const u32 m = meta[t], c = m & ((1u << ECB_CELL_BITS) - 1u), f = m >> ECB_CELL_BITS;
        if (c >= n_cells) { atomicOr(err, 2u); continue; }
        if (lds) { atomicAdd(&lcnt[c], cnt[t]); atomicMin(&lfile[c], f); }
        else { atomicAdd(&total[c], (u64)cnt[t]); atomicMin(&firstfile[c], f); }
    }
    if (!lds) return;
    __syncthreads();
    for (u32 c = threadIdx.x; c < n_cells; c += TPB_MSF)
        if (lfile[c] != 0xFFFFFFFFu) { atomicAdd(&total[c], (u64)lcnt[c]); atomicMin(&firstfile[c], lfile[c]); }
}
__global__ void k_msf2_seg(const u32* ec, u64 n, u32 n_ecs, u32* seg, u32* err) {
    const u64 t = blockIdx.x * (u64)blockDim.x + threadIdx.x;
    if (t >= n) return;
    const u32 e = ec[t];
    if (e >= n_ecs) { atomicOr(err, 1u); return; }
    const long long ep = t ? (long long)ec[t - 1] : -1ll;
    for (long long x = ep + 1; x <= (long long)e; ++x) seg[x] = (u32)t;
    if (t == n - 1) for (u64 x = (u64)e + 1; x <= n_ecs; ++x) seg[x] = (u32)n;
}
constexpr u32 MSF_SMALL = 256;
constexpr u32 MSF_FILES = 1u << MS_FILE_BITS;
constexpr u32 MSF_GIANT = 1u << 15;
__global__ void k_msf2_ecs_small(const u32* meta, const u32* first, const u32* seg, u32 n_ecs, u32 n_cells, const u64* total, const u32* firstfile,
                                 u64 min_count, u64* cellkey, u32* keep_ec, u32* big, u32* n_big, u32* giant, u32* n_giant) {
    const u64 e = blockIdx.x * (u64)blockDim.x + threadIdx.x;
    if (e >= n_ecs) return;
    const u32 a = seg[e], b = seg[e + 1];
    if (b - a > MSF_GIANT) { giant[atomicAdd(n_giant, 1u)] = (u32)e; return; }
    if (b - a > MSF_SMALL) { big[atomicAdd(n_big, 1u)] = (u32)e; return; }
    bool keep = false;
    u32 last_f = 0xFFFFFFFFu, last_fec = 0;
    for (u32 t = a; t < b; ++t) {
        const u32 m = meta[t], c = m & ((1u << ECB_CELL_BITS) - 1u), f = m >> ECB_CELL_BITS;
        if (c >= n_cells) continue;
        keep |= total[c] >= min_count;
        if (firstfile[c] != f) continue;
        if (f != last_f) {
            u32 fec = first[t];
            for (u32 x = a; x < b; ++x) if ((meta[x] >> ECB_CELL_BITS) == f) fec = min(fec, first[x]);
            last_f = f; last_fec = fec;
        }
        const u32 fec = last_fec;
        const u64 offer = ((u64)fec << 32) | first[t];
        if (offer < cellkey[c]) atomicMin(&cellkey[c], offer);
    }
    if (keep) keep_ec[e] = 1u;
}
__global__ __launch_bounds__(TPB) void k_msf2_ecs_big(const u32* meta, const u32* first, const u32* seg, const u32* big, const u32* n_big, u32 n_cells,
                                                      const u64* total, const u32* firstfile, u64 min_count, u64* cellkey, u32* keep_ec) {
    __shared__ u32 fec[MSF_FILES];
    __shared__ u32 s_keep;
    for (u32 q = blockIdx.x; q < *n_big; q += gridDim.x) {
        const u32 e = big[q], a = seg[e], b = seg[e + 1];
        for (u32 f = threadIdx.x; f < MSF_FILES; f += TPB) fec[f] = 0xFFFFFFFFu;
        if (threadIdx.x == 0) s_keep = 0;
        __syncthreads();
        bool keep = false;
        for (u32 t = a + threadIdx.x; t < b; t += TPB) {
            const u32 m = meta[t], c = m & ((1u << ECB_CELL_BITS) - 1u);
            if (c >= n_cells) continue;
            atomicMin(&fec[m >> ECB_CELL_BITS], first[t]);
            keep |= total[c] >= min_count;
        }
        if (keep) s_keep = 1u;
        __syncthreads();
        for (u32 t = a + threadIdx.x; t < b; t += TPB) {
            const u32 m = meta[t], c = m & ((1u << ECB_CELL_BITS) - 1u), f = m >> ECB_CELL_BITS;
            if (c < n_cells && firstfile[c] == f) {
                const u64 offer = ((u64)fec[f] << 32) | first[t];
                if (offer < cellkey[c]) atomicMin(&cellkey[c], offer);
            }
        }
        if (threadIdx.x == 0 && s_keep) keep_ec[e] = 1u;
        __syncthreads();
    }
}
__global__ __launch_bounds__(TPB) void k_msf2_giant_fec(const u32* meta, const u32* first, const u32* seg, const u32* giant, const u32* n_giant, u32 n_cells,
                                                        const u64* total, u64 min_count, u32* gfec, u32* keep_ec) {
    __shared__ u32 fec[MSF_FILES];
    __shared__ u32 s_keep;
    for (u32 g = 0; g < *n_giant; ++g) {
        const u32 e = giant[g], a = seg[e], b = seg[e + 1];
        for (u32 f = threadIdx.x; f < MSF_FILES; f += TPB) fec[f] = 0xFFFFFFFFu;
        if (threadIdx.x == 0) s_keep = 0;
        __syncthreads();
        bool keep = false;
        for (u64 t = (u64)a + (u64)blockIdx.x * TPB + threadIdx.x; t < b; t += (u64)gridDim.x * TPB) {
            const u32 m = meta[t], c = m & ((1u << ECB_CELL_BITS) - 1u);
            if (c >= n_cells) continue;
            atomicMin(&fec[m >> ECB_CELL_BITS], first[t]);
            keep |= total[c] >= min_count;
        }
        if (keep) s_keep = 1u;
        __syncthreads();
        for (u32 f = threadIdx.x; f < MSF_FILES; f += TPB) if (fec[f] != 0xFFFFFFFFu) atomicMin(&gfec[(u64)g * MSF_FILES + f], fec[f]);
        if (threadIdx.x == 0 && s_keep) keep_ec[e] = 1u;
        __syncthreads();
    }
}
__global__ __launch_bounds__(TPB) void k_msf2_giant_offer(const u32* meta, const u32* first, const u32* seg, const u32* giant, const u32* n_giant, u32 n_cells,
                                                          const u32* firstfile, const u32* gfec, u64* cellkey) {
    for (u32 g = 0; g < *n_giant; ++g) {
        const u32 e = giant[g], a = seg[e], b = seg[e + 1];
        for (u64 t = (u64)a + (u64)blockIdx.x * TPB + threadIdx.x; t < b; t += (u64)gridDim.x * TPB) {
            const u32 m = meta[t], c = m & ((1u << ECB_CELL_BITS) - 1u), f = m >> ECB_CELL_BITS;
            if (c < n_cells && firstfile[c] == f) {
                const u64 offer = ((u64)gfec[(u64)g * MSF_FILES + f] << 32) | first[t];
                if (offer < cellkey[c]) atomicMin(&cellkey[c], offer);
            }
        }
    }
}
__global__ void k_msf2_cellflag(const u64* total, u32 n_cells, u32* flag) {
    const u64 c = blockIdx.x * (u64)blockDim.x + threadIdx.x;
    if (c < n_cells) flag[c] = total[c] ? 1u : 0u;
}
__global__ void k_msf2_celllist(const u64* total, const u32* firstfile, const u64* cellkey, const u32* flag, const u32* pos, u32 n_cells,
                                u32* cell_id, u64* ctotal, u64* bhi, u64* blo) {
    const u64 c = blockIdx.x * (u64)blockDim.x + threadIdx.x;
    if (c >= n_cells || !flag[c]) return;
    const u32 o = pos[c];
    cell_id[o] = (u32)c; ctotal[o] = total[c]; bhi[o] = firstfile[c]; blo[o] = cellkey[c];
}
__global__ void k_msf2_pairflag(const u32* ec, const u32* meta, u64 n, const u32* new_cell, u32* flag) {
    const u64 t = blockIdx.x * (u64)blockDim.x + threadIdx.x;
    if (t >= n) return;
    const u32 c = meta[t] & ((1u << ECB_CELL_BITS) - 1u);
    const bool head = t == 0 || ec[t - 1] != ec[t] || (meta[t - 1] & ((1u << ECB_CELL_BITS) - 1u)) != c;
    flag[t] = (head && new_cell[c] != 0xFFFFFFFFu) ? 1u : 0u;
}
__global__ void k_msf2_pairs(const u32* ec, const u32* meta, const u32* cnt, const u32* flag, const u32* pos, u64 n, const u32* new_cell,
                             const u32* new_rank, u64* key, u32* val, u32* err) {
    const u64 t = blockIdx.x * (u64)blockDim.x + threadIdx.x;
    if (t >= n || !flag[t]) return;
    const u32 e = ec[t], c = meta[t] & ((1u << ECB_CELL_BITS) - 1u);
    u64 sum = 0;
    for (u64 x = t; x < n && ec[x] == e && (meta[x] & ((1u << ECB_CELL_BITS) - 1u)) == c; ++x) sum += cnt[x];
    if (sum > 0x7FFFFFFFull) atomicOr(err, 4u);
    key[pos[t]] = ((u64)new_cell[c] << 32) | new_rank[e];
    val[pos[t]] = (u32)sum;
}
__global__ void k_msf_gather64(const u64* src, const u32* idx, u64 n, u64* dst) { const u64 i = blockIdx.x * (u64)blockDim.x + threadIdx.x; if (i < n) dst[i] = src[idx[i]]; }
__global__ void k_msf_keepflag(const u32* order, const u64* total, u64 n, u64 min_count, u32* flag) {
    const u64 i = blockIdx.x * (u64)blockDim.x + threadIdx.x;
    if (i < n) flag[i] = total[order[i]] >= min_count ? 1u : 0u;
}
__global__ void k_msf_newcell(const u32* order, const u32* flag, const u32* pos, const u32* cell_id, u64 n, u32* new_cell, u32* kept_cells) {
    const u64 i = blockIdx.x * (u64)blockDim.x + threadIdx.x;
    if (i < n && flag[i]) { const u32 c = cell_id[order[i]]; new_cell[c] = pos[i]; kept_cells[pos[i]] = c; }
}
__global__ void k_msf_rowlen(const u32* indptr, const u32* keep_ec, const u32* new_rank, u64 n_ecs, u32* rowlen2) {
    const u64 e = blockIdx.x * (u64)blockDim.x + threadIdx.x;
    if (e < n_ecs && keep_ec[e]) rowlen2[new_rank[e]] = indptr[e + 1] - indptr[e];
}
__global__ void k_msf_rows(const u32* indptr, const int* indices, const int* data, const u32* keep_ec, const u32* new_rank,
                           const u32* indptr2, u64 n_ecs, int* indices2, int* data2) {
    const u64 e = blockIdx.x * (u64)blockDim.x + threadIdx.x;
    if (e >= n_ecs || !keep_ec[e]) return;
    const u32 a = indptr[e], b = indptr[e + 1], o = indptr2[new_rank[e]];
    for (u32 i = a; i < b; ++i) { indices2[o + (i - a)] = indices[i]; data2[o + (i - a)] = data[i]; }
}

constexpr int POISON_BYTE = 0x01;
inline bool poison_scratch() { const char* e = getenv("ECB_POISON_SCRATCH"); return e && *e && strcmp(e, "0") != 0; }
template <class T = void>
struct DevBuf {
    void* p = nullptr;
    u64 bytes = 0;
    int dev = 0;
    DevBuf() = default;
    DevBuf(const DevBuf&) = delete;
    DevBuf& operator=(const DevBuf&) = delete;
    DevBuf(DevBuf&& o) noexcept : p(o.p), bytes(o.bytes), dev(o.dev) { o.p = nullptr; o.bytes = 0; }
    DevBuf& operator=(DevBuf&& o) noexcept {
        if (this != &o) { reset(); p = o.p; bytes = o.bytes; dev = o.dev; o.p = nullptr; o.bytes = 0; }
        return *this;
    }
    ~DevBuf() { reset(); }
    operator T*() const { return static_cast<T*>(p); }
    T* operator->() const { return static_cast<T*>(p); }
    template <class U> U* as() const { return static_cast<U*>(p); }
    hipError_t reset() {
        hipError_t e = hipSuccess;
        if (p) { hipSetDevice(dev); e = hipFree(p); }
        p = nullptr; bytes = 0;
        return e;
    }
    hipError_t alloc(u64 n, u64 at_least = 0) {
        reset();
        n = std::max(n, at_least);
        hipError_t e = hipGetDevice(&dev);
        if (e == hipSuccess) e = hipMalloc(&p, n);
        if (e != hipSuccess) { p = nullptr; return e; }
        bytes = n;
        if (n && poison_scratch()) {
            e = hipMemset(p, POISON_BYTE, n);
            if (e == hipSuccess) e = hipDeviceSynchronize();
            if (e != hipSuccess) { reset(); return e; }
        }
        return hipSuccess;
    }
    hipError_t regrow(u64 need, u64 slack) { return bytes >= need ? hipSuccess : alloc(need + slack); }
    hipError_t grow(u64 n, int fill, u64 keep, hipStream_t st) {
        DevBuf q;
        hipError_t e = q.alloc(n);
        if (e == hipSuccess && fill >= 0) e = hipMemsetAsync(q.p, fill, n, st);
        if (e == hipSuccess && p) {
            e = hipMemcpyAsync(q.p, p, keep, hipMemcpyDeviceToDevice, st);
            if (e == hipSuccess) e = hipStreamSynchronize(st);
        }
        if (e != hipSuccess) return e;
        e = reset();
        *this = std::move(q);
        return e;
    }
};
struct HostFree { void operator()(void* q) const { hipHostFree(q); } };
template <class T> using Pinned = std::unique_ptr<T, HostFree>;
template <class T> hipError_t pin(Pinned<T>& out) {
    void* q = nullptr;
    const hipError_t e = hipHostMalloc(&q, sizeof(T), hipHostMallocDefault);
    out.reset(static_cast<T*>(q));
    return e;
}

}

enum class Stage { OPEN,
                   COUNTED,
                   FINAL };
enum class Origin { OWN,
                    ADOPTED,
                    ASSEMBLED };
enum class Triples { NONE, OWN , ADOPTED  };
enum StreamVariant { SV_STD, SV_STD_RANGES, SV_SHORT, SV_PAR, SV_VERIFY, SV_N };

struct ecb_handle {
    ecb_config cfg{};
    int device = 0;
    hipStream_t stream = nullptr;
    std::string err;
    u64 wave_arena_n = 0;
    bool scatter_attr_set = false, count_attr_set = false;
    u64 resident_blocks[SV_VERIFY] = {}, rounds = 24, min_tiles = 32;
    bool par_stream = false;
    bool ctr_synced = false;

    u64 cap = 0, arena_cap = 0;
    Counters hctr{};
    struct PinOut { Counters c; u64 tot[8]; };
    u64 read_slot_cap = 0;
    u64 meta_cap = 0;
    u64 queue_cap = 0;
    u64 n_ecs() const { return hctr.n_ecs; }
    u64 reads_hint = 0;

    u32 *st_loc = nullptr, *st_hf = nullptr; int* st_pos = nullptr; u64 st_cap = 0;

    struct Run {
        Stage stage = Stage::OPEN;
        Origin origin = Origin::OWN;
        u32 prev_rid = 0xFFFFFFFFu;
        u64 n_reads = 0;
        u64 reads_hi = 0;
        u64 records_pushed = 0;
        u64 meta_hi = 0;
        u64 extra_all = 0, extra_valid = 0, extra_reads = 0;
        u64 n_mismatch = 0;
        int refused = ECB_OK;
        std::string refusal;
        std::vector<u32> c_rid, c_loc, c_hf; std::vector<int> c_pos;
        u64* d_list_n = nullptr;
        struct Csr { u32 *order = nullptr, *rank_of_slot = nullptr , *indptr = nullptr;
                     int *indices = nullptr, *data = nullptr, *counts = nullptr; } csr;
        u64 n_list = 0;
        ecb_sizes sizes{};
        struct Tri { u64 n = 0; u64* okey = nullptr; u32 *ofirst = nullptr, *ostart = nullptr, *ocount = nullptr; } tri;
        Triples triples = Triples::NONE;
        struct Filtered { u32* cells = nullptr; int *ipa = nullptr, *ixa = nullptr, *daa = nullptr, *ipn = nullptr, *ixn = nullptr, *dan = nullptr; } flt;
        ecb_ms_sizes msf{};
    } run;
    bool multisample() const { return (cfg.flags & ECB_F_MULTISAMPLE) != 0; }
    bool can_push() const { return run.stage == Stage::OPEN; }
    bool counted() const { return run.stage >= Stage::COUNTED; }
    bool has_result() const { return run.stage == Stage::FINAL; }
    bool has_ms_result() const { return has_result() && multisample(); }
    bool open_read() const { return !run.c_rid.empty(); }
    bool holds_nothing() const { return !n_ecs() && !run.n_reads && !open_read(); }
    bool entries_from_elsewhere() const { return run.origin != Origin::OWN; }
    u32* slot_list() const { return pool[P_LIST].as<u32>(); }
    bool awaits_triples() const { return entries_from_elsewhere() && run.triples != Triples::ADOPTED; }

    enum { P_RESUME, P_SUMS, P_HIST, P_OFFS, P_PAIRS, P_CNT, P_PARTS, P_WORK, P_LIST, P_BITMAP, P_WPOP, P_WPREFIX, P_ROWLEN, P_ORDER,
           P_WCOUNTS, P_RANK, P_INDPTR, P_COUNTS, P_INDICES, P_DATA, P_MS_KEYS, P_MS_KEYS2, P_MS_VALS, P_MS_VALS2, P_MS_TMP,
           P_MS_FLAG, P_MS_POS, P_MS_OKEY, P_MS_OFIRST, P_MS_OSTART, P_MS_X, P_MS_OCOUNT, P_MS_GRANK, P_MS_CIN, P_MS_FIN, P_LISTFN,
           P_REMAP, P_TOTALS, P_SLOW_LEN, P_SLOW_OFF, P_SLOW_NRE, P_SLOW_REQ, P_SLOW_REQ2, P_QCOMPACT, P_SLOW_KEY, P_SLOW_MASK, P_BIG, P_RS_HIST, P_RS_OFFS,
           P_F_CELLS, P_F_IPA, P_F_IXA, P_F_DAA, P_F_IPN, P_F_IXN, P_F_DAN, P_EXPORT, P_N };

    bool prof = false; double prof_ms = 0; u64 prof_launches = 0, prof_records = 0;
    int last_variant = SV_N;
    hipEvent_t ev0 = nullptr, ev1 = nullptr;

    DevBuf<u32> st_rid;
    DevBuf<> pool[P_N];
    DevBuf<StreamCold> d_cold;
    Pinned<StreamCold> pin_cold;
    Pinned<PinOut> pin_out;
    Pinned<Counters> pin_ctr;
    DevBuf<u64> wave_arena;
    DevBuf<u64> queue;
    DevBuf<int2> rng;
    DevBuf<u32> meta;
    DevBuf<u32> read_slot;
    DevBuf<Counters> ctr;
    DevBuf<uint2> arena;
    DevBuf<Slot> table;

    ~ecb_handle() {
        if (ev0) hipEventDestroy(ev0);
        if (ev1) hipEventDestroy(ev1);
        if (stream) hipStreamDestroy(stream);
    }
};

namespace {

thread_local std::string t_err;

int fail(ecb_handle* h, int code, const char* fmt, ...) {
    char buf[512];
    va_list ap; va_start(ap, fmt); vsnprintf(buf, sizeof buf, fmt, ap); va_end(ap);
    if (h) h->err = buf; else t_err = buf;
    return code;
}
int run_refused(ecb_handle* h, int rc) {
    if (rc != ECB_OK && h->run.refused == ECB_OK) { h->run.refused = rc; h->run.refusal = h->err; }
    return rc;
}
int refused_run(ecb_handle* h) {
    if (h->run.refused == ECB_OK) return ECB_OK;
    return fail(h, ECB_ERR_STATE, "this run was refused (%d: %s): ecb_reset the handle", h->run.refused, h->run.refusal.c_str());
}
#define HIPCHK_AS(h, prefix, call) do { hipError_t e_ = (call); if (e_ != hipSuccess) \
    return fail(h, ECB_ERR_HIP, "%s%s: %s", prefix, #call, hipGetErrorString(e_)); } while (0)
#define HIPCHK(h, call) HIPCHK_AS(h, "", call)
#define RCCHK(call) do { const int rc_ = (call); if (rc_ != ECB_OK) return rc_; } while (0)

struct ErrBit { u32 bit; int code; const char* text; };
template <size_t N> int refuse_bits(ecb_handle* h, const ErrBit (&table)[N], u32 bits, unsigned long long arg = 0) {
    for (const ErrBit& e : table) if (bits & e.bit) return fail(h, e.code, e.text, arg);
    return ECB_OK;
}
const ErrBit COUNTER_ERRS[] = {
    {ERR_CONTRACT, ECB_ERR_CONTRACT, "read_id run counter violates the tuple contract (see ecb.h)"},
    {ERR_RANGE, ECB_ERR_CONTRACT, "locus or haplotype index out of range in a valid record"},
    {ERR_ARENA, ECB_ERR_TABLE_FULL, "EC key arena exhausted (%llu pairs): raise arena_capacity"},
    {ERR_QUEUE, ECB_ERR_TABLE_FULL, "deferred-read queue exhausted"},
    {ERR_INTERNAL, ECB_ERR_HIP, "internal: an EC-table slot was claimed but its key never published"},
    {ERR_COUNT, ECB_ERR_LIMIT, "an EC's count is above 2^31-1"},
};

u64 next_pow2(u64 x) { u64 p = 1; while (p < x) p <<= 1; return p; }
u64 msb_mask(u64 x) { return x ? ~0ull >> __builtin_clzll(x) : 0ull; }
inline unsigned nblk(u64 n, unsigned per) { return (unsigned)((n + per - 1) / per); }

#define POOL(h, id, ptr, count) do { const u64 need_ = std::max<u64>(count, 1) * sizeof(*(ptr)); \
    HIPCHK(h, h->pool[ecb_handle::id].regrow(need_, need_ / 4)); \
    (ptr) = h->pool[ecb_handle::id].as<std::remove_reference_t<decltype(*(ptr))>>(); } while (0)
template <class T> T* fresh(std::vector<DevBuf<>>& keep, u64 n) {
    keep.emplace_back();
    return keep.back().alloc(std::max<u64>(n, 1) * sizeof(T)) == hipSuccess ? keep.back().as<T>() : nullptr;
}
bool missing(const std::vector<DevBuf<>>& keep) { return std::any_of(keep.begin(), keep.end(), [](const DevBuf<>& b) { return !b.p; }); }

int clear_counters(ecb_handle* h) {
    Counters c{};
    const u32 R = arena_regions(h->arena_cap);
    const u64 per = h->arena_cap / R;
    for (u32 r = 0; r < ARENA_REGIONS; ++r) c.arena_reg[r] = r < R ? r * per : h->arena_cap;
    h->hctr = c;
    if (h->pin_ctr) {
        *h->pin_ctr = c;
        HIPCHK(h, hipMemcpyAsync(h->ctr, h->pin_ctr.get(), sizeof(Counters), hipMemcpyHostToDevice, h->stream));
    } else {
        HIPCHK(h, hipMemcpyAsync(h->ctr, &h->hctr, sizeof(Counters), hipMemcpyHostToDevice, h->stream));
        HIPCHK(h, hipStreamSynchronize(h->stream));
    }
    h->ctr_synced = true;
    return ECB_OK;
}
u64 arena_used(const ecb_handle* h) {
    const u32 R = arena_regions(h->arena_cap);
    const u64 per = h->arena_cap / R;
    u64 used = h->hctr.arena_top;
    for (u32 r = 0; r < R; ++r) used += std::min<u64>(h->hctr.arena_reg[r], (u64)(r + 1) * per) - r * per;
    return used;
}

int sync_counters(ecb_handle* h) {
    HIPCHK(h, hipMemcpyAsync(&h->pin_out->c, h->ctr, sizeof(Counters), hipMemcpyDeviceToHost, h->stream));
    HIPCHK(h, hipStreamSynchronize(h->stream));
    h->hctr = h->pin_out->c;
    h->ctr_synced = true;
    return refuse_bits(h, COUNTER_ERRS, h->hctr.err, h->arena_cap);
}

int grow_table(ecb_handle* h, u64 new_cap) {
    DevBuf<Slot> nt;
    u32* remap = nullptr;
    if (new_cap > (1ull << 32)) return fail(h, ECB_ERR_LIMIT, "EC table beyond 2^32 slots");
    POOL(h, P_REMAP, remap, h->cap);
    HIPCHK(h, nt.alloc(new_cap * sizeof(Slot)));
    HIPCHK_AS(h, "grow_table: ", hipMemsetAsync(nt, 0, new_cap * sizeof(Slot), h->stream));
    HIPCHK_AS(h, "grow_table: ", hipMemsetAsync(remap, 0xFF, h->cap * sizeof(u32), h->stream));
    k_rehash<<<2048, TPB, 0, h->stream>>>(h->table, h->cap, nt, new_cap - 1, remap);
    if (h->run.reads_hi)
        k_remap_read_slot<<<2048, TPB, 0, h->stream>>>(h->read_slot, h->run.reads_hi, remap);
    HIPCHK_AS(h, "grow_table: ", hipStreamSynchronize(h->stream));
    HIPCHK(h, h->table.reset());
    h->table = std::move(nt);
    h->cap = new_cap; h->run.d_list_n = nullptr;
    return ECB_OK;
}

int ensure_read_slot(ecb_handle* h, u64 need) {
    if (need <= h->read_slot_cap) return ECB_OK;
    u64 nc = std::max<u64>(need, h->read_slot_cap * 2);
    nc = std::max<u64>(nc, 1024);
    HIPCHK(h, h->read_slot.grow(nc * sizeof(u32), 0xFF, h->run.n_reads * sizeof(u32), h->stream));
    h->read_slot_cap = nc;
    return ECB_OK;
}

int ensure_meta(ecb_handle* h, u64 need) {
    if (need <= h->meta_cap) return ECB_OK;
    const u64 nc = std::max<u64>(need, h->meta_cap * 2);
    HIPCHK(h, h->meta.grow(nc * sizeof(u32), -1, h->run.meta_hi * sizeof(u32), h->stream));
    h->meta_cap = nc;
    return ECB_OK;
}

int run_slow(ecb_handle* h, const u32* d_rid, const u32* d_loc, const u32* d_hf, u64 n, u64* d_q, u64 nq, bool verify = false, u32 tw = 512u) {
    int rc = ECB_OK;
    int flip = 0;
    while (nq) {
        u64 *d_len = nullptr, *d_off = nullptr, *d_nre = nullptr, *nre_buf = nullptr;
        POOL(h, P_SLOW_LEN, d_len, nq); POOL(h, P_SLOW_OFF, d_off, nq); POOL(h, P_SLOW_NRE, d_nre, 1);
        if (flip) POOL(h, P_SLOW_REQ2, nre_buf, nq); else POOL(h, P_SLOW_REQ, nre_buf, nq);
        HIPCHK(h, hipMemsetAsync(d_nre, 0, sizeof(u64), h->stream));
        k_slow_len<<<(unsigned)nq, TPB, 0, h->stream>>>(d_rid, n, d_q, nq, d_len, tw);
        std::vector<u64> len(nq), off(nq);
        HIPCHK(h, hipMemcpyAsync(len.data(), d_len, nq * sizeof(u64), hipMemcpyDeviceToHost, h->stream));
        HIPCHK(h, hipStreamSynchronize(h->stream));
        u64 tot = 0;
        for (u64 i = 0; i < nq; ++i) { off[i] = tot; tot += 2 * len[i]; }
        u32 *sk = nullptr, *sm = nullptr;
        const DevBuf<>& bk = h->pool[ecb_handle::P_SLOW_KEY];
        const DevBuf<>& bm = h->pool[ecb_handle::P_SLOW_MASK];
        const u64 had_k = bk.bytes, had_m = bm.bytes;
        POOL(h, P_SLOW_KEY, sk, tot); POOL(h, P_SLOW_MASK, sm, tot);
        if (bk.bytes != had_k) HIPCHK(h, hipMemsetAsync(sk, 0, bk.bytes, h->stream));
        if (bm.bytes != had_m) HIPCHK(h, hipMemsetAsync(sm, 0, bm.bytes, h->stream));
        HIPCHK(h, hipMemcpyAsync(d_off, off.data(), nq * sizeof(u64), hipMemcpyHostToDevice, h->stream));
        SlowArgs a{d_rid, d_loc, d_hf, d_q, d_len, d_off, sk, sm, h->cfg.n_loci, h->cfg.n_haplotypes,
                   h->table, h->cap - 1, h->arena, h->arena_cap, h->ctr, h->read_slot, h->run.reads_hi, nre_buf, d_nre, verify ? 1u : 0u};
        k_slow<<<(unsigned)nq, TPB, 2 * SLOW_LDS * sizeof(u32), h->stream>>>(a);
        u64 nre = 0;
        HIPCHK(h, hipMemcpyAsync(&nre, d_nre, sizeof(u64), hipMemcpyDeviceToHost, h->stream));
        rc = sync_counters(h);
        if (rc != ECB_OK || verify) break;
        d_q = nre_buf; nq = nre; flip ^= 1;
        if (nq) { rc = grow_table(h, h->cap * 4); if (rc != ECB_OK) break; }
    }
    return rc;
}

int excl_scan(ecb_handle* h, const u32* in, u64 n, u32* out, u64* total);

struct StreamVariantRow { void (*kernel)(StreamArgs); const char* name; int blocks_per_cu; };
const StreamVariantRow STREAM_VARIANTS[SV_N] = {
    {ks_std::k_stream<false>, "ks_std::k_stream<false, false>", 4},
    {ks_std::k_stream<false, true>, "ks_std::k_stream<false, true>", 4},
    {ks_short::k_stream<false>, "ks_short::k_stream<false, false>", 4},
    {ks_par::k_stream<false>, "ks_par::k_stream<false, false>", 5},
    {ks_std::k_stream<true>, "", 0},
};

struct StreamPlan { u64 slices, chunk, blocks, pwaves; };
int plan_stream(ecb_handle* h, u64 n, StreamPlan* P, StreamVariant v) {
    if (!h->resident_blocks[SV_STD]) {
        int cus = 256;
        hipDeviceGetAttribute(&cus, hipDeviceAttributeMultiprocessorCount, h->device);
        for (int i = 0; i < SV_VERIFY; ++i) {
            int bpc = STREAM_VARIANTS[i].blocks_per_cu;
            hipOccupancyMaxActiveBlocksPerMultiprocessor(&bpc, STREAM_VARIANTS[i].kernel, TPB, 0);
            h->resident_blocks[i] = (u64)std::max(cus, 1) * std::max(bpc, 1);
        }
        h->rounds = getenv("ECB_ROUNDS") ? std::max(1, atoi(getenv("ECB_ROUNDS"))) : 24;
        h->min_tiles = getenv("ECB_MIN_TILES") ? std::max(2, atoi(getenv("ECB_MIN_TILES"))) : 32;
    }
    const u64 rounds = h->rounds, resident_blocks = h->resident_blocks[v == SV_VERIFY ? SV_STD : v];
    const u64 MIN_TILES = h->min_tiles;
    const u64 res_waves = resident_blocks * NWAVE;
    u64 waves = std::min<u64>(res_waves * rounds, std::max<u64>(n / (MIN_TILES * WT), res_waves));
    waves = std::min<u64>(waves, (n + 2 * WT - 1) / (2 * WT));
    waves = std::max<u64>(waves, 1);
    u64 chunk = (n + waves - 1) / waves;
    chunk = (chunk + WT - 1) / WT * WT;
    waves = (n + chunk - 1) / chunk;
    P->slices = waves; P->chunk = chunk;
    P->blocks = std::min<u64>((waves + NWAVE - 1) / NWAVE, resident_blocks);
    P->pwaves = P->blocks * NWAVE;
    const u64 need_q = P->pwaves * (u64)(WT + 1) + n / 64 + 16;
    if (h->queue_cap < need_q) {
        h->queue_cap = 0;
        HIPCHK(h, h->queue.alloc(need_q * sizeof(u64)));
        h->queue_cap = need_q;
    }
    return ECB_OK;
}

int run_deferred(ecb_handle* h, const u32* d_rid, const u32* d_loc, const u32* d_hf, u64 n, bool verify, u32 tw, u64* n_done = nullptr) {
    const u64 nq = h->hctr.n_queue;
    if (n_done) *n_done = nq;
    if (!nq) return ECB_OK;
    u64* d_q = nullptr;
    POOL(h, P_QCOMPACT, d_q, nq);
    k_queue_compact<<<QSTRIPES, TPB, 0, h->stream>>>(h->queue, h->queue_cap, h->ctr, d_q);
    HIPCHK(h, hipGetLastError());
    return run_slow(h, d_rid, d_loc, d_hf, n, d_q, nq, verify, tw);
}

StreamVariant pick_variant(const ecb_handle* h, u64 n) {
    if (h->rng) return SV_STD_RANGES;
    const bool few = h->run.n_reads ? h->run.records_pushed < 7 * h->run.n_reads : (n >= h->reads_hint && n < 7 * h->reads_hint);
    if (h->reads_hint != 0 && h->cfg.n_loci < MAX_LOCI_SHORT && h->cfg.n_haplotypes <= 8 && !getenv("ECB_NO_SHORT") &&
        (getenv("ECB_FORCE_SHORT") || few)) return SV_SHORT;
    if (!getenv("ECB_NO_PAR") && (getenv("ECB_FORCE_PAR") || h->par_stream)) return SV_PAR;
    return SV_STD;
}

int zero_launch_words(ecb_handle* h) {
    HIPCHK(h, hipMemsetAsync(&h->ctr->n_queue, 0, (1 + QSTRIPES) * sizeof(u64), h->stream));
    HIPCHK(h, hipMemsetAsync(&h->ctr->full, 0, sizeof(u32), h->stream));
    HIPCHK(h, hipMemsetAsync(&h->ctr->next_slice, 0, sizeof(u64), h->stream));
    return ECB_OK;
}

int launch_stream(ecb_handle* h, StreamVariant v, const StreamPlan& P, const u32* d_rid, const u32* d_loc, const u32* d_hf, const int* d_pos, u64 n,
                  u32 prev_rid, const u32* d_last, u32 launch, u64 offered, u64* timing = nullptr) {
    const bool verify = v == SV_VERIFY;
    int2* const rng = verify ? nullptr : (int2*)h->rng;
    u64* d_resume = nullptr; u32* d_wcounts = nullptr;
    POOL(h, P_RESUME, d_resume, 2 * P.slices);
    if (!launch) k_init_resume<<<nblk(P.slices, TPB), TPB, 0, h->stream>>>(d_resume, P.slices, P.chunk, verify ? nullptr : (Counters*)h->ctr);
    POOL(h, P_WCOUNTS, d_wcounts, 3 * P.pwaves);
    if (launch) RCCHK(zero_launch_words(h));
    else {
        if (verify) {
            HIPCHK(h, hipMemsetAsync(d_wcounts, 0, 3 * P.pwaves * sizeof(u32), h->stream));
            RCCHK(zero_launch_words(h));
            HIPCHK(h, hipMemsetAsync(&h->ctr->n_mismatch, 0, sizeof(u64), h->stream));
        } else if (h->wave_arena_n < P.pwaves) {
            HIPCHK(h, h->wave_arena.grow(2 * P.pwaves * sizeof(u64), 0, 2 * h->wave_arena_n * sizeof(u64), h->stream));
            h->wave_arena_n = P.pwaves;
        }
        *h->pin_cold = StreamCold{h->arena, h->arena_cap, h->queue, h->queue_cap, d_resume, d_wcounts, verify ? nullptr : (u64*)h->wave_arena, timing,
                                  P.chunk, prev_rid, d_pos, rng, verify ? 0u : h->cfg.n_loci, verify ? 0u : h->cfg.n_haplotypes};
        HIPCHK(h, hipMemcpyAsync(h->d_cold, h->pin_cold.get(), sizeof(StreamCold), hipMemcpyHostToDevice, h->stream));
    }
    const StreamArgs a{d_rid, d_loc, d_hf, n, h->table, h->cap - 1, h->ctr, h->read_slot, h->run.reads_hi, h->d_cold,
                       !verify && getenv("ECB_ABLATE") ? (u32)atoi(getenv("ECB_ABLATE")) : 0u, d_pos, rng};
    if (h->prof && !verify) hipEventRecord(h->ev0, h->stream);
    STREAM_VARIANTS[v].kernel<<<(unsigned)P.blocks, TPB, 0, h->stream>>>(a);
    if (h->prof && !verify) hipEventRecord(h->ev1, h->stream);
    k_sum_counts<<<1, 1024, 0, h->stream>>>(d_wcounts, P.pwaves, h->ctr, verify ? 1u : 0u, offered, h->queue_cap, d_last);
    HIPCHK(h, hipGetLastError());
    if (!verify) h->last_variant = v;
    return ECB_OK;
}

int verify_pass(ecb_handle* h, const StreamPlan& P, const u32* d_rid, const u32* d_loc, const u32* d_hf, u64 n, u32 prev_rid, u64* n_long, u32 tw) {
    RCCHK(launch_stream(h, SV_VERIFY, P, d_rid, d_loc, d_hf, nullptr, n, prev_rid, nullptr, 0, 0));
    RCCHK(sync_counters(h));
    return run_deferred(h, d_rid, d_loc, d_hf, n, true, tw, n_long);
}
int verify_batch(ecb_handle* h, const u32* d_rid, const u32* d_loc, const u32* d_hf, u64 n, u32 prev_rid, u64* n_mismatch, u64* n_long, u32 tw = 512u) {
    StreamPlan P;
    RCCHK(plan_stream(h, n, &P, SV_VERIFY));
    u64 nq = 0;
    if (const int rc = verify_pass(h, P, d_rid, d_loc, d_hf, n, prev_rid, &nq, tw); rc != ECB_OK) {
        if (h->hctr.err) {
            const std::string refusal = h->err;
            HIPCHK(h, hipMemsetAsync(&h->ctr->err, 0, sizeof(u32), h->stream));
            HIPCHK(h, hipMemsetAsync(&h->ctr->n_queue, 0, (1 + QSTRIPES) * sizeof(u64), h->stream));
            h->hctr.err = 0; h->hctr.n_queue = 0;
            h->err = refusal;
        }
        return rc;
    }
    *n_mismatch = h->hctr.n_mismatch;
    *n_long = nq;
    HIPCHK(h, hipMemsetAsync(&h->ctr->n_queue, 0, (1 + QSTRIPES) * sizeof(u64), h->stream));
    h->hctr.n_queue = 0;
    return ECB_OK;
}

int build_batch(ecb_handle* h, const u32* d_rid, const u32* d_loc, const u32* d_hf, const int* d_pos, u64 n, u32 tw, bool* launched) {
    if (n == 0) return ECB_OK;
    const bool hinted = h->reads_hint != 0;
    u32 last_rid = 0;
    u64 reads_after = std::max<u64>(h->reads_hint, h->run.n_reads);
    if (!hinted) {
        HIPCHK(h, hipMemcpyAsync(&last_rid, d_rid + rec_at(n - 1, tw), sizeof(u32), hipMemcpyDeviceToHost, h->stream));
        HIPCHK(h, hipStreamSynchronize(h->stream));
        reads_after = (u64)(u32)(last_rid + 1u);
        if (reads_after < h->run.n_reads) return fail(h, ECB_ERR_CONTRACT, "read_id went backwards across pushes");
    }
    RCCHK(ensure_read_slot(h, reads_after));
    h->run.reads_hi = reads_after;
    while (h->n_ecs() * 2 > h->cap) { RCCHK(grow_table(h, h->cap * 4)); }
    const StreamVariant v = pick_variant(h, n);
    StreamPlan P;
    RCCHK(plan_stream(h, n, &P, v));
    u64* timing = nullptr;
#ifdef ECB_TIMING
    HIPCHK(h, hipMalloc(&timing, 8 * sizeof(u64)));
    HIPCHK(h, hipMemset(timing, 0, 8 * sizeof(u64)));
#endif
    h->ctr_synced = false;
    *launched = true;
    const u64 probe_before = h->hctr.n_probe_tiles;
    int rc = ECB_OK;
    for (u32 launch = 0;; ++launch) {
        rc = launch_stream(h, v, P, d_rid, d_loc, d_hf, d_pos, n, h->run.prev_rid, d_rid + rec_at(n - 1, tw), launch, launch ? 0 : n, timing);
        if (rc != ECB_OK) break;
        rc = sync_counters(h);
        if (h->prof) {
            float ms = 0; hipEventElapsedTime(&ms, h->ev0, h->ev1);
            h->prof_ms += ms; h->prof_launches += 1;
        }
        if (rc != ECB_OK) break;
        const bool parked = h->hctr.full != 0;
        rc = run_deferred(h, d_rid, d_loc, d_hf, n, false, tw);
        if (rc != ECB_OK) break;
        if (!parked) break;
        rc = grow_table(h, h->cap * 4);
        if (rc != ECB_OK) break;
    }
#ifdef ECB_TIMING
    {
        u64 t[8];
        hipMemcpy(t, timing, sizeof(t), hipMemcpyDeviceToHost); hipFree(timing);
        static const char* nm[8] = {"(a) filter+heads", "tile decisions", "prefetch issue+clear+geometry", "(b) LDS tables", "hash entries", "(c) lookup", "publish/settle/slot stores", "-"};
        u64 tot = 0; for (int i = 0; i < 7; ++i) tot += t[i];
        fprintf(stderr, "[ecb timing] %llu waves, clocks per wave:", (unsigned long long)P.slices);
        for (int i = 0; i < 7; ++i) fprintf(stderr, "  %s %.0f (%.1f%%)", nm[i], (double)t[i] / P.slices, 100.0 * t[i] / std::max<u64>(tot, 1));
        fprintf(stderr, "  tile visits on the probe-on path %llu of %llu tiles", (unsigned long long)t[7], (unsigned long long)((n + WT - 1) / WT));
        fprintf(stderr, "\n");
    }
#endif
    RCCHK(rc);
    {
        const u64 tiles = (n + WT - 1) / WT, on_path = h->hctr.n_probe_tiles - probe_before;
        if (on_path * 4 > tiles) h->par_stream = true; else if (on_path * 16 < tiles) h->par_stream = false;
    }
    if (h->prof) h->prof_records += n;
    if (h->cfg.flags & ECB_F_VERIFY) {
        u64 bad = 0, nl = 0;
        RCCHK(verify_batch(h, d_rid, d_loc, d_hf, n, h->run.prev_rid, &bad, &nl, tw));
        h->run.n_mismatch += bad;
        if (bad) return fail(h, ECB_ERR_VERIFY, "exactness pass: %llu read(s) of this batch sit in an EC whose key is not their target set", (unsigned long long)bad);
    }
    if (hinted) {
        last_rid = h->hctr.last_rid;
        reads_after = (u64)(u32)(last_rid + 1u);
        if (reads_after < h->run.n_reads) return fail(h, ECB_ERR_CONTRACT, "read_id went backwards across pushes");
    }
    h->run.prev_rid = last_rid;
    h->run.n_reads = reads_after;
    h->run.records_pushed += n;
    return ECB_OK;
}
int process_batch(ecb_handle* h, const u32* d_rid, const u32* d_loc, const u32* d_hf, const int* d_pos, u64 n, u32 tw = 512u) {
    bool launched = false;
    const int rc = build_batch(h, d_rid, d_loc, d_hf, d_pos, n, tw, &launched);
    return launched ? run_refused(h, rc) : rc;
}

int ensure_staging(ecb_handle* h, u64 need) {
    if (need <= h->st_cap) return ECB_OK;
    h->st_loc = h->st_hf = nullptr; h->st_pos = nullptr; h->st_cap = 0;
    const u64 cap = std::max<u64>(need, h->cfg.max_batch_records);
    const u64 stride = (cap * sizeof(u32) + (2ull << 20) - 1) / (2ull << 20) * (2ull << 20) / sizeof(u32);
    const bool rg = (h->cfg.flags & ECB_F_RANGES) != 0;
    HIPCHK(h, h->st_rid.alloc((rg ? 4 : 3) * stride * sizeof(u32)));
    h->st_cap = cap;
    h->st_loc = h->st_rid + stride; h->st_hf = h->st_rid + 2 * stride;
    if (rg) h->st_pos = reinterpret_cast<int*>(h->st_rid + 3 * stride);
    return ECB_OK;
}

int stage_and_process(ecb_handle* h, const u32* rid, const u32* loc, const u32* hf, const int* pos, u64 m) {
    const u64 nc = h->run.c_rid.size();
    const u64 n = nc + m;
    if (!n) return ECB_OK;
    RCCHK(ensure_staging(h, n));
    const bool rg = (h->cfg.flags & ECB_F_RANGES) != 0;
    const struct { void* st; const void *carry, *window; } streams[4] = {
        {h->st_rid, h->run.c_rid.data(), rid}, {h->st_loc, h->run.c_loc.data(), loc}, {h->st_hf, h->run.c_hf.data(), hf}, {h->st_pos, h->run.c_pos.data(), pos}};
    for (int w = 0; w < 2; ++w)
        for (int i = 0; i < (rg ? 4 : 3) && (w ? m : nc); ++i)
            HIPCHK(h, hipMemcpyAsync((u32*)streams[i].st + (w ? nc : 0), w ? streams[i].window : streams[i].carry, (w ? m : nc) * 4, hipMemcpyHostToDevice, h->stream));
    HIPCHK(h, hipStreamSynchronize(h->stream));
    h->run.c_rid.clear(); h->run.c_loc.clear(); h->run.c_hf.clear(); h->run.c_pos.clear();
    return process_batch(h, h->st_rid, h->st_loc, h->st_hf, rg ? h->st_pos : nullptr, n);
}

int excl_scan_dev(ecb_handle* h, const u32* in, u64 n, u32* out, u64* d_total, u32 stride = 1, u32* last32 = nullptr) {
    u32* sums = nullptr;
    POOL(h, P_SUMS, sums, scan_words(n));
    HIPCHK(h, scan_launch(h->stream, in, n, out, sums, d_total, stride, last32));
    return ECB_OK;
}
int excl_scan(ecb_handle* h, const u32* in, u64 n, u32* out, u64* total) {
    u64* d_tot = nullptr;
    POOL(h, P_TOTALS, d_tot, 8);
    RCCHK(excl_scan_dev(h, in, n, out, d_tot + 7));
    HIPCHK(h, hipMemcpyAsync(total, d_tot + 7, sizeof(u64), hipMemcpyDeviceToHost, h->stream));
    HIPCHK(h, hipStreamSynchronize(h->stream));
    return ECB_OK;
}

struct SortBufs {
    u64* k[2];
    u32* v[2];
    int at = 0;
    u64* keys() const { return k[at]; }
    u32* vals() const { return v[at]; }
    u64* spare_keys() const { return k[at ^ 1]; }
    u32* spare_vals() const { return v[at ^ 1]; }
};
struct SortScratch { u32 *hist, *offs; u64* d_word; };
inline u64 rs_tiles(u64 n) { return std::max<u64>(1, (n + RS_TILE - 1) / RS_TILE); }
constexpr u64 RS_AUX_WORDS = 2 * RS_MAX_PASSES * 256 + 64;
inline u64 rs_words(u64 n) { return std::max<u64>(256 * rs_tiles(n), RS_AUX_WORDS); }
hipError_t radix_sort_pairs64(hipStream_t st, SortBufs& b, u64 n, const SortScratch& sc, u64 bit_mask = ~0ull) {
    b.at = 0;
    if (n < 2) return hipSuccess;
    if (n >= (1ull << 30)) return hipErrorInvalidValue;
    hipError_t e = hipSuccess;
    u64 ormask = bit_mask;
    if (bit_mask == ~0ull) {
        if ((e = hipMemsetAsync(sc.d_word, 0, 8, st)) != hipSuccess) return e;
        k_or_reduce<<<(unsigned)std::min<u64>(1024, (n + TPB - 1) / TPB), TPB, 0, st>>>(b.k[0], n, sc.d_word);
        if ((e = hipMemcpyAsync(&ormask, sc.d_word, 8, hipMemcpyDeviceToHost, st)) != hipSuccess) return e;
        if ((e = hipStreamSynchronize(st)) != hipSuccess) return e;
    }
    RsShifts sh{};
    for (u32 shift = 0; shift < 64; shift += 8)
        if ((ormask >> shift) & 255ull) sh.s[sh.n++] = shift;
    if (!sh.n) return hipSuccess;
    const u32 nt = (u32)rs_tiles(n);
    u32 *ghist = sc.offs, *base = sc.offs + RS_MAX_PASSES * 256, *ticket = sc.offs + 2 * RS_MAX_PASSES * 256, *err = ticket + 1;
    if ((e = hipMemsetAsync(sc.offs, 0, RS_AUX_WORDS * 4, st)) != hipSuccess) return e;
    k_rs_hist_all<<<(unsigned)std::min<u64>(2048, (n + 16 * RS_TPB - 1) / (16 * RS_TPB)), RS_TPB, 0, st>>>(b.k[0], n, sh, ghist);
    k_rs_bases<<<1, 256, 0, st>>>(ghist, sh.n, base);
    for (u32 p = 0; p < sh.n; ++p) {
        if ((e = hipMemsetAsync(sc.hist, 0, (u64)nt * 256 * 4, st)) != hipSuccess) return e;
        if ((e = hipMemsetAsync(ticket, 0, 4, st)) != hipSuccess) return e;
        k_rs_pass<<<nt, RS_TPB, 0, st>>>(b.keys(), b.vals(), n, sh.s[p], base + p * 256, sc.hist, ticket, err, b.spare_keys(), b.spare_vals());
        b.at ^= 1;
    }
    if ((e = hipGetLastError()) != hipSuccess) return e;
    u32 gave_up = 0;
    if ((e = hipMemcpyAsync(&gave_up, err, 4, hipMemcpyDeviceToHost, st)) != hipSuccess) return e;
    if ((e = hipStreamSynchronize(st)) != hipSuccess) return e;
    return gave_up ? hipErrorUnknown : hipSuccess;
}
int handle_sort(ecb_handle* h, SortBufs& b, u64 n, u64 bit_mask = ~0ull) {
    SortScratch sc{};
    u64* tot = nullptr;
    POOL(h, P_RS_HIST, sc.hist, rs_words(n)); POOL(h, P_RS_OFFS, sc.offs, RS_AUX_WORDS); POOL(h, P_TOTALS, tot, 8);
    sc.d_word = tot + 6;
    HIPCHK_AS(h, "radix sort: ", radix_sort_pairs64(h->stream, b, n, sc, bit_mask));
    return ECB_OK;
}
int sorted_runs(ecb_handle* h, SortBufs& b, u64 n, u32* flag, u32* pos, u64* n_runs) {
    RCCHK(handle_sort(h, b, n));
    k_run_heads<<<nblk(n, TPB), TPB, 0, h->stream>>>(b.keys(), n, flag);
    return excl_scan(h, flag, n, pos, n_runs);
}

int ensure_slot_ranks(ecb_handle* h, u64 E) {
    if (h->run.csr.rank_of_slot) return ECB_OK;
    POOL(h, P_RANK, h->run.csr.rank_of_slot, h->cap);
    k_slot_ranks<<<nblk(E, TPB), TPB, 0, h->stream>>>(h->run.csr.order, E, h->run.csr.rank_of_slot);
    HIPCHK(h, hipGetLastError());
    return ECB_OK;
}

int ensure_counts(ecb_handle* h, const CompactSink* sink = nullptr, bool* listed = nullptr) {
    if (h->counted()) return ECB_OK;
    const u64 R = h->run.n_reads;
    CompactSink own{nullptr, 0, nullptr, nullptr, 0, nullptr};
    if (R && !sink && h->run.origin != Origin::ADOPTED && h->n_ecs()) {
        u32* list = nullptr;
        u64* d_n = nullptr;
        POOL(h, P_LIST, list, h->n_ecs());
        POOL(h, P_CNT, d_n, 1);
        HIPCHK(h, hipMemsetAsync(d_n, 0, sizeof(u64), h->stream));
        own = CompactSink{list, h->n_ecs(), d_n, nullptr, 0, nullptr};
        sink = &own;
    }
    if (R) {
        u32 bb = BIN_BITS;
        {
            u32 lc = 0;
            while ((1ull << (lc + 1)) <= h->cap) ++lc;
            bb = std::min<u32>(std::max<u32>(lc, 9u + MIN_BIN_BITS) - 9u, BIN_BITS);
        }
        if (const char* e = getenv("ECB_BIN_BITS")) bb = (u32)std::min<long>(std::max<long>(atol(e), MIN_BIN_BITS), MAX_BIN_BITS);
        while (bb < MAX_BIN_BITS && (h->cap >> bb) > MAX_BUCKETS) ++bb;
        const u32 nb = (u32)std::max<u64>(1, h->cap >> bb);
        if (nb > MAX_BUCKETS) return fail(h, ECB_ERR_LIMIT, "EC table larger than 2^28 slots is not supported");
        if (bb > 14 && !h->count_attr_set) {
            HIPCHK(h, hipFuncSetAttribute((const void*)k_count_bins, hipFuncAttributeMaxDynamicSharedMemorySize, 4 << MAX_BIN_BITS));
            h->count_attr_set = true;
        }
        const u32 G = (u32)std::min<u64>(PART_G, (R + 4095) / 4096);
        u32 *hist = nullptr, *offs = nullptr;
        u16* pairs = nullptr;
        u64* d_tot = nullptr;
        POOL(h, P_HIST, hist, (u64)nb * G); POOL(h, P_OFFS, offs, (u64)nb * G);
        POOL(h, P_PAIRS, pairs, R);
        POOL(h, P_TOTALS, d_tot, 8);
        k_part_hist<<<G, TPB_PART, nb * 4, h->stream>>>(h->read_slot, R, nb, bb, hist);
        d_tot += 6;
        RCCHK(excl_scan_dev(h, hist, (u64)nb * G, offs, d_tot));
        if (nb <= STAGE_MAX_BUCKETS) {
            if (!h->scatter_attr_set) {
                HIPCHK(h, hipFuncSetAttribute((const void*)k_part_scatter_staged, hipFuncAttributeMaxDynamicSharedMemorySize,
                                              3 * STAGE_MAX_BUCKETS * 4 + STAGE * 4));
                h->scatter_attr_set = true;
            }
            k_part_scatter_staged<<<G, TPB_PART, 3 * nb * 4 + STAGE * 4, h->stream>>>(h->read_slot, R, nb, bb, offs, pairs);
        } else
            k_part_scatter<<<G, TPB_PART, nb * 4, h->stream>>>(h->read_slot, R, nb, bb, offs, pairs);
        const u32 piece = std::max<u32>(32768u, 2u * (u32)((R + nb - 1) / nb));
        const u32 max_work = nb + (u32)(R / piece) + 1;
        CountWork* d_work = nullptr;
        POOL(h, P_WORK, d_work, (u64)max_work + 1);
        u32* d_nwork = reinterpret_cast<u32*>(d_work + max_work);
        k_build_work<<<1, 1024, 0, h->stream>>>(offs, G, d_tot, nb, piece, d_work, max_work, d_nwork);
        k_count_bins<<<max_work, TPB_COUNT, 4u << bb, h->stream>>>(pairs, d_work, d_nwork, bb, h->table, sink ? *sink : CompactSink{nullptr, 0, nullptr, nullptr, 0, nullptr});
        if (sink == &own) h->run.d_list_n = own.n_list;
        else if (sink && listed) *listed = true;
        HIPCHK(h, hipGetLastError());
    }
    h->run.stage = Stage::COUNTED;
    return ECB_OK;
}

int compact_table_dev(ecb_handle* h, u64* d_n, u32* bitmap = nullptr, u64 n_bits = 0, uint2* list_fn = nullptr) {
    u32* list = nullptr;
    HIPCHK(h, hipMemsetAsync(d_n, 0, sizeof(u64), h->stream));
    POOL(h, P_LIST, list, h->n_ecs());
    k_compact<<<(unsigned)std::min<u64>(2048, (h->cap + 4 * TPB_COMPACT - 1) / (4 * TPB_COMPACT)), TPB_COMPACT, 0, h->stream>>>(h->table, h->cap, list, std::max<u64>(h->n_ecs(), 1), d_n, bitmap, n_bits, list_fn);
    return ECB_OK;
}
int compact_table(ecb_handle* h) {
    u64* d_n = h->run.d_list_n;
    if (!d_n) {
        POOL(h, P_CNT, d_n, 1);
        RCCHK(compact_table_dev(h, d_n));
    }
    HIPCHK(h, hipMemcpyAsync(&h->run.n_list, d_n, sizeof(u64), hipMemcpyDeviceToHost, h->stream));
    HIPCHK(h, hipStreamSynchronize(h->stream));
    if (h->run.n_list != h->n_ecs()) return fail(h, ECB_ERR_HIP, "internal: %llu occupied slots but %llu ECs created",
                                             (unsigned long long)h->run.n_list, (unsigned long long)h->n_ecs());
    return ECB_OK;
}

int ms_reduce(ecb_handle* h, const u32* ec_of_slot) {
    const u64 R = h->run.n_reads;
    if (h->run.meta_hi < R) return fail(h, ECB_ERR_STATE, "ecb_push_cells covered %llu of %llu reads",
                                    (unsigned long long)h->run.meta_hi, (unsigned long long)R);
    u64 *keys = nullptr, *keys2 = nullptr; u32 *vals = nullptr, *vals2 = nullptr, *flag = nullptr, *pos = nullptr;
    POOL(h, P_MS_KEYS, keys, R); POOL(h, P_MS_KEYS2, keys2, R); POOL(h, P_MS_VALS, vals, R); POOL(h, P_MS_VALS2, vals2, R);
    POOL(h, P_MS_FLAG, flag, R); POOL(h, P_MS_POS, pos, R);
    k_ms_keys<<<nblk(R, TPB), TPB, 0, h->stream>>>(h->read_slot, ec_of_slot, h->meta, R, keys, vals);
    SortBufs s{{keys, keys2}, {vals, vals2}};
    u64 nt = 0;
    RCCHK(sorted_runs(h, s, R, flag, pos, &nt));
    POOL(h, P_MS_OKEY, h->run.tri.okey, nt); POOL(h, P_MS_OFIRST, h->run.tri.ofirst, nt); POOL(h, P_MS_OSTART, h->run.tri.ostart, (u64)nt + 1);
    k_ms_emit<<<nblk(R, TPB), TPB, 0, h->stream>>>(s.keys(), s.vals(), flag, pos, R, nt, h->run.tri.okey, h->run.tri.ofirst, h->run.tri.ostart);
    HIPCHK(h, hipStreamSynchronize(h->stream));
    h->run.tri.n = nt; h->run.tri.ocount = nullptr; h->run.triples = Triples::OWN;
    return ECB_OK;
}

__global__ void k_rebase(Entry* e, u64 n, u32 base, u32 limit, Counters* ctr) {
    const u64 i = blockIdx.x * (u64)blockDim.x + threadIdx.x;
    if (i >= n) return;
    const u32 first = ~e[i].first_inv;
    if (first >= limit) { atomicOr(&ctr->err, ERR_CONTRACT); return; }
    e[i].first_inv = ~(first + base);
}

__global__ void k_export_firsts(const Slot* table, const u32* order, u64 n, u32* firsts) {
    const u64 e = blockIdx.x * (u64)blockDim.x + threadIdx.x;
    if (e < n) firsts[e] = ~table[order[e]].first_inv;
}
struct PieceDesc { const u32* firsts; const int *indptr, *indices, *data, *counts; u64 n, nnz, at; };
__global__ void k_mark_bits(const PieceDesc* P, u64 n_bits, u32* bitmap, Counters* ctr) {
    const PieceDesc d = P[blockIdx.y];
    const u64 e = blockIdx.x * (u64)blockDim.x + threadIdx.x;
    if (e >= d.n) return;
    const u32 f = d.firsts[e];
    if (f >= n_bits) { atomicOr(&ctr->err, ERR_CONTRACT); return; }
    atomicOr(&bitmap[f >> 5], 1u << (f & 31u));
}
__global__ void k_piece_place(const PieceDesc* P, u64 n_total, u64 n_bits, const u32* bitmap, const u32* wprefix, uint4* place, Counters* ctr) {
    const PieceDesc d = P[blockIdx.y];
    const u64 e = blockIdx.x * (u64)blockDim.x + threadIdx.x;
    if (e >= d.n) return;
    const u32 f = d.firsts[e];
    if (f >= n_bits) return;
    const long long s0 = d.indptr[e], s1 = d.indptr[e + 1];
    if (s0 < 0 || s1 < s0 || (u64)s1 > d.nnz) { atomicOr(&ctr->err, ERR_CONTRACT); return; }
    const u32 r = bit_rank(bitmap, wprefix, f);
    if (r >= n_total) return;
    const u32 cnt = (u32)d.counts[e];
    if (cnt > 0x7FFFFFFFu) atomicOr(&ctr->err, ERR_COUNT);
    place[r] = make_uint4((u32)e + 1u, (u32)(s1 - s0), cnt, blockIdx.y);
}
__global__ void k_piece_rows(const PieceDesc* P, u32 n_pieces, const uint4* place, u64 n_total, const u32* indptr, int* indices, int* data, int* counts) {
    const u64 r = blockIdx.x * (u64)blockDim.x + threadIdx.x;
    if (r >= n_total) return;
    const uint4 pl = place[r];
    counts[r] = (int)pl.z;
    if (pl.x == 0u || pl.w >= n_pieces) return;
    const u32 q = pl.w;
    const u64 e = pl.x - 1u;
    const int* ip = P[q].indptr;
    const int s0 = ip[e], s1 = ip[e + 1];
    const u32 d0 = indptr[r];
    if (indptr[r + 1] - d0 != (u32)(s1 - s0) || pl.y != (u32)(s1 - s0)) return;
    const int *sj = P[q].indices, *sd = P[q].data;
    for (int i = s0; i < s1; ++i) { indices[d0 + (u32)(i - s0)] = sj[i]; data[d0 + (u32)(i - s0)] = sd[i]; }
}

int push_refused(ecb_handle* h, size_t n, bool streams_given) {
    if (!h) return ECB_ERR_ARG;
    RCCHK(refused_run(h));
    if (!h->can_push()) return fail(h, ECB_ERR_STATE, "push after finalize / table export");
    if (n && !streams_given) return fail(h, ECB_ERR_ARG, "null tuple stream");
    return ECB_OK;
}
int device_push_refused(ecb_handle* h, const char* who, uintptr_t ptr_bits) {
    if (ptr_bits & 15) return fail(h, ECB_ERR_ARG, "device streams must be 16-byte aligned");
    if (h->open_read()) return fail(h, ECB_ERR_STATE, "%s while a host push has an open read", who);
    HIPCHK(h, hipSetDevice(h->device));
    return ECB_OK;
}
int verify_streams(ecb_handle* h, const void* d_rid, const void* d_loc, const void* d_hf, size_t n, u32 tw, u64* n_mismatch, u64* n_long) {
    RCCHK(refused_run(h));
    if (!n || !d_rid || !d_loc || !d_hf) return fail(h, ECB_ERR_ARG, "null tuple stream");
    if (((uintptr_t)d_rid | (uintptr_t)d_loc | (uintptr_t)d_hf) & 15) return fail(h, ECB_ERR_ARG, "device streams must be 16-byte aligned");
    HIPCHK(h, hipSetDevice(h->device));
    return verify_batch(h, (const u32*)d_rid, (const u32*)d_loc, (const u32*)d_hf, n, 0xFFFFFFFFu, n_mismatch, n_long, tw);
}
int push_cells(ecb_handle* h, const void* meta, uint64_t first_read, size_t n, hipMemcpyKind kind) {
    if (!h) return ECB_ERR_ARG;
    RCCHK(refused_run(h));
    if (!h->multisample()) return fail(h, ECB_ERR_STATE, "handle was created without ECB_F_MULTISAMPLE");
    if (h->has_result()) return fail(h, ECB_ERR_STATE, "push after finalize");
    if (!n) return ECB_OK;
    if (!meta) return fail(h, ECB_ERR_ARG, "null meta");
    HIPCHK(h, hipSetDevice(h->device));
    if (first_read >= (1ull << 32) - 1 || (u64)n >= (1ull << 32) - 1 - first_read) return fail(h, ECB_ERR_LIMIT, "more than 2^32-2 reads");
    const u64 need = first_read + n;
    RCCHK(ensure_meta(h, need));
    HIPCHK(h, hipMemcpyAsync(h->meta + first_read, meta, n * sizeof(u32), kind, h->stream));
    if (kind == hipMemcpyHostToDevice) HIPCHK(h, hipStreamSynchronize(h->stream));
    h->run.meta_hi = std::max<u64>(h->run.meta_hi, need);
    return ECB_OK;
}
int refuse_no_ecs(ecb_handle* h, u64 E, u64 valid) {
    if (E == 0 || valid == 0) return fail(h, ECB_ERR_EMPTY, "no valid alignments: nothing to build (the reference fails here too)");
    if (E >= (1ull << 31) - 1) return fail(h, ECB_ERR_LIMIT, "more than 2^31-2 equivalence classes");
    return ECB_OK;
}
int refuse_nnz(ecb_handle* h, u64 nnz) {
    if (nnz >= (1ull << 31)) return fail(h, ECB_ERR_LIMIT, "A has more than 2^31-1 non-zeros");
    return ECB_OK;
}
ecb_sizes result_sizes(u64 E, u64 nnz, u64 all, u64 valid, u64 reads) {
    ecb_sizes s{};
    s.n_ecs = E; s.nnz_a = nnz; s.n_samples = 1; s.nnz_n = E;
    s.all_alignments = all; s.valid_alignments = valid; s.n_reads = reads;
    return s;
}
int export_result(ecb_handle* h, void* ia, void* ja, void* da, void* in_, void* jn, void* dn, hipMemcpyKind kind) {
    HIPCHK(h, hipSetDevice(h->device));
    const bool on_device = kind == hipMemcpyDeviceToDevice;
    const u64 E = h->run.sizes.n_ecs, nnz = h->run.sizes.nnz_a;
    const ecb_handle::Run::Csr& r = h->run.csr;
    if (ia) HIPCHK(h, hipMemcpyAsync(ia, r.indptr, (E + 1) * 4, kind, h->stream));
    if (ja) HIPCHK(h, hipMemcpyAsync(ja, r.indices, nnz * 4, kind, h->stream));
    if (da) HIPCHK(h, hipMemcpyAsync(da, r.data, nnz * 4, kind, h->stream));
    if (on_device) {
        if (in_) { const int v[2] = {0, (int)E}; HIPCHK(h, hipMemcpyAsync(in_, v, 8, hipMemcpyHostToDevice, h->stream)); }
        if (jn) k_iota<<<nblk(E, TPB), TPB, 0, h->stream>>>((u32*)jn, E);
    }
    if (dn) HIPCHK(h, hipMemcpyAsync(dn, r.counts, E * 4, kind, h->stream));
    HIPCHK(h, hipStreamSynchronize(h->stream));
    if (!on_device) {
        if (in_) { ((int32_t*)in_)[0] = 0; ((int32_t*)in_)[1] = (int32_t)E; }
        if (jn) for (u64 i = 0; i < E; ++i) ((int32_t*)jn)[i] = (int32_t)i;
    }
    return ECB_OK;
}

}

extern "C" {

int ecb_abi_version(void) { return ECB_ABI_VERSION; }

int ecb_device_count(void) {
    int n = 0;
    if (hipGetDeviceCount(&n) != hipSuccess) return 0;
    return n;
}

const char* ecb_last_error(const ecb_handle* h) { return h ? h->err.c_str() : t_err.c_str(); }

int ecb_create(const ecb_config* cfg, ecb_handle** out) {
    if (!cfg || !out || cfg->struct_size != sizeof(ecb_config)) return fail(nullptr, ECB_ERR_ARG, "bad ecb_config (struct_size)");
    if (cfg->n_loci == 0 || cfg->n_loci >= MAX_LOCI) return fail(nullptr, ECB_ERR_ARG, "n_loci out of range (1 .. 2^26-3)");
    if (cfg->n_haplotypes == 0 || cfg->n_haplotypes > 31) return fail(nullptr, ECB_ERR_ARG, "n_haplotypes must be 1..31 (A stores a bitmask in int32)");
    int ndev = 0;
    if (hipGetDeviceCount(&ndev) != hipSuccess || ndev <= 0) return fail(nullptr, ECB_ERR_NO_DEVICE, "no HIP device: libecb has no CPU path");
    if (cfg->device < 0 || cfg->device >= ndev) return fail(nullptr, ECB_ERR_ARG, "device %d out of range (%d present)", cfg->device, ndev);
    std::unique_ptr<ecb_handle> owner(new ecb_handle());
    ecb_handle* const h = owner.get();
    h->cfg = *cfg;
    h->device = cfg->device;
    if (!h->cfg.ec_capacity) h->cfg.ec_capacity = 1ull << 22;
    if (!h->cfg.arena_capacity) h->cfg.arena_capacity = 1ull << 26;
    if (!h->cfg.max_batch_records) h->cfg.max_batch_records = 1ull << 24;
    h->cap = std::max<u64>(next_pow2(h->cfg.ec_capacity), 1024);
    h->arena_cap = std::min<u64>(h->cfg.arena_capacity, 1ull << 32);
#define CREATECHK(call) HIPCHK_AS(nullptr, "ecb_create: ", call)
    CREATECHK(hipSetDevice(h->device));
    CREATECHK(hipStreamCreate(&h->stream));
    CREATECHK(h->table.alloc(h->cap * sizeof(Slot)));
    CREATECHK(h->arena.alloc(h->arena_cap * sizeof(uint2)));
    CREATECHK(h->ctr.alloc(sizeof(Counters)));
    CREATECHK(pin(h->pin_ctr));
    CREATECHK(pin(h->pin_cold));
    CREATECHK(pin(h->pin_out));
    CREATECHK(h->d_cold.alloc(sizeof(StreamCold)));
    CREATECHK(hipMemsetAsync(h->table, 0, h->cap * sizeof(Slot), h->stream));
    CREATECHK(hipMemsetAsync(h->arena, 0, h->arena_cap * sizeof(uint2), h->stream));
    if (const int rc = clear_counters(h); rc != ECB_OK) return fail(nullptr, rc, "ecb_create: %s", h->err.c_str());
    if (cfg->flags & ECB_F_RANGES) {
        const u64 ns = (u64)cfg->n_loci * cfg->n_haplotypes;
        CREATECHK(h->rng.alloc(ns * sizeof(int2)));
        k_fill_minmax<<<nblk(ns, TPB), TPB, 0, h->stream>>>(h->rng, ns);
    }
    hipEventCreate(&h->ev0); hipEventCreate(&h->ev1);
    CREATECHK(hipStreamSynchronize(h->stream));
#undef CREATECHK
    *out = owner.release();
    return ECB_OK;
}

void ecb_destroy(ecb_handle* h) {
    if (!h) return;
    hipSetDevice(h->device);
    if (h->stream) hipStreamSynchronize(h->stream);
    delete h;
}

int ecb_verify_device(ecb_handle* h, const void* d_read_id, const void* d_locus, const void* d_hapflag, size_t n,
                      uint64_t* n_mismatch, uint64_t* n_long) {
    if (!h || !n_mismatch || !n_long) return ECB_ERR_ARG;
    u64 bad = 0, nl = 0;
    const int rc = verify_streams(h, d_read_id, d_locus, d_hapflag, n, 512u, &bad, &nl);
    *n_mismatch = bad; *n_long = nl;
    return rc;
}

int ecb_reset(ecb_handle* h) {
    if (!h) return ECB_ERR_ARG;
    HIPCHK(h, hipSetDevice(h->device));
    const u32* occupied = h->has_result() ? h->slot_list() : nullptr;
    const u64 n_occupied = h->run.n_list;
    const bool poison = poison_scratch();
    if (poison)
        for (int i = 0; i < ecb_handle::P_N; ++i)
            if (h->pool[i].p && i != ecb_handle::P_SLOW_KEY && i != ecb_handle::P_SLOW_MASK && i != ecb_handle::P_LIST)
                HIPCHK(h, hipMemsetAsync(h->pool[i].p, POISON_BYTE, h->pool[i].bytes, h->stream));
    if (!h->ctr_synced) sync_counters(h);
    {
        const u32 R = arena_regions(h->arena_cap);
        const u64 per = h->arena_cap / R;
        ArenaClear ac{};
        u32 n = 0;
        u64 longest = 0;
        for (u32 r = 0; r < R; ++r) {
            const u64 used = std::min<u64>(h->hctr.arena_reg[r], (u64)(r + 1) * per) - r * per;
            if (used) { ac.start[n] = r * per; ac.len[n] = used; ++n; longest = std::max(longest, used); }
        }
        if (h->hctr.arena_top) { ac.start[n] = 0; ac.len[n] = std::min<u64>(h->hctr.arena_top, h->arena_cap); longest = std::max(longest, ac.len[n]); ++n; }
        if (n) {
            const dim3 grid((unsigned)std::min<u64>(nblk(longest, TPB), 2048), n);
            k_clear_arena<<<grid, TPB, 0, h->stream>>>(h->arena, ac);
            HIPCHK(h, hipGetLastError());
        }
    }
#if defined(ECB_TIMING) || defined(ECB_EXPERIMENTS)
    if (!getenv("ECB_KEEP_TABLE"))
#endif
    {
        if (h->run.origin == Origin::ASSEMBLED) {
        } else if (occupied && n_occupied && n_occupied == h->n_ecs() && !h->hctr.err && n_occupied * 3 < h->cap)
            k_clear_slots<<<nblk(n_occupied, TPB), TPB, 0, h->stream>>>(h->table, occupied, n_occupied);
        else
            HIPCHK(h, hipMemsetAsync(h->table, 0, h->cap * sizeof(Slot), h->stream));
    }
    if (poison && h->pool[ecb_handle::P_LIST].p)
        HIPCHK(h, hipMemsetAsync(h->pool[ecb_handle::P_LIST].p, POISON_BYTE, h->pool[ecb_handle::P_LIST].bytes, h->stream));
    RCCHK(clear_counters(h));
    if (h->wave_arena) HIPCHK(h, hipMemsetAsync(h->wave_arena, 0, 2 * h->wave_arena_n * sizeof(u64), h->stream));
    if ((h->cfg.flags & ECB_F_VERIFY) && h->read_slot) HIPCHK(h, hipMemsetAsync(h->read_slot, 0xFF, h->read_slot_cap * sizeof(u32), h->stream));
    if (h->rng) {
        const u64 ns = (u64)h->cfg.n_loci * h->cfg.n_haplotypes;
        k_fill_minmax<<<nblk(ns, TPB), TPB, 0, h->stream>>>(h->rng, ns);
    }
    h->run = ecb_handle::Run{};
    h->err.clear();
    return ECB_OK;
}

int ecb_hint_reads(ecb_handle* h, uint64_t max_reads) {
    if (!h) return ECB_ERR_ARG;
    RCCHK(refused_run(h));
    if (max_reads >= (1ull << 32)) return fail(h, ECB_ERR_LIMIT, "more than 2^32 - 1 reads");
    h->reads_hint = max_reads;
    return ECB_OK;
}

int ecb_push_device(ecb_handle* h, const void* d_read_id, const void* d_locus, const void* d_hapflag,
                    const void* d_pos, size_t n) {
    RCCHK(push_refused(h, n, d_read_id && d_locus && d_hapflag));
    if ((h->cfg.flags & ECB_F_RANGES) && n && !d_pos) return fail(h, ECB_ERR_ARG, "ECB_F_RANGES needs pos");
    RCCHK(device_push_refused(h, "ecb_push_device", (uintptr_t)d_read_id | (uintptr_t)d_locus | (uintptr_t)d_hapflag | (uintptr_t)d_pos));
    return process_batch(h, (const u32*)d_read_id, (const u32*)d_locus, (const u32*)d_hapflag, (const int*)d_pos, n);
}

int ecb_push_device_tiled(ecb_handle* h, const void* d_tiles, size_t n) {
    RCCHK(push_refused(h, n, d_tiles != nullptr));
    if (h->cfg.flags & ECB_F_RANGES) return fail(h, ECB_ERR_STATE, "ECB_F_RANGES takes the four streams of ecb_push_device");
    RCCHK(device_push_refused(h, "ecb_push_device_tiled", (uintptr_t)d_tiles));
    const u32* d = (const u32*)d_tiles;
    return process_batch(h, d, d + 512, d + 1024, nullptr, n, 1536u);
}

int ecb_verify_device_tiled(ecb_handle* h, const void* d_tiles, size_t n, uint64_t* n_mismatch, uint64_t* n_long_reads) {
    if (!h || !n_mismatch) return ECB_ERR_ARG;
    u64 bad = 0, nl = 0;
    const u32* d = (const u32*)d_tiles;
    RCCHK(verify_streams(h, d, d ? d + 512 : d, d ? d + 1024 : d, n, 1536u, &bad, &nl));
    *n_mismatch = bad;
    if (n_long_reads) *n_long_reads = nl;
    return ECB_OK;
}

int ecb_push(ecb_handle* h, const uint32_t* rid, const uint32_t* loc, const uint32_t* hf, const int32_t* pos, size_t n) {
    RCCHK(push_refused(h, n, rid && loc && hf));
    const bool rg = (h->cfg.flags & ECB_F_RANGES) != 0;
    if (rg && n && !pos) return fail(h, ECB_ERR_ARG, "ECB_F_RANGES needs pos");
    HIPCHK(h, hipSetDevice(h->device));
    u64 done = 0;
    while (done < n) {
        const u64 m = std::min<u64>(h->cfg.max_batch_records, n - done);
        const u32 *r = rid + done, *l = loc + done, *f = hf + done;
        const int* ps = rg ? pos + done : nullptr;
        const u32 last = r[m - 1];
        u64 cut = m;
        while (cut > 0 && r[cut - 1] == last) --cut;
        const bool carry_continues = !h->run.c_rid.empty() && h->run.c_rid.back() == last;
        if (cut == 0 && (carry_continues || h->run.c_rid.empty())) {
            h->run.c_rid.insert(h->run.c_rid.end(), r, r + m);
            h->run.c_loc.insert(h->run.c_loc.end(), l, l + m);
            h->run.c_hf.insert(h->run.c_hf.end(), f, f + m);
            if (rg) h->run.c_pos.insert(h->run.c_pos.end(), ps, ps + m);
        } else {
            RCCHK(stage_and_process(h, r, l, f, ps, cut));
            h->run.c_rid.assign(r + cut, r + m);
            h->run.c_loc.assign(l + cut, l + m);
            h->run.c_hf.assign(f + cut, f + m);
            if (rg) h->run.c_pos.assign(ps + cut, ps + m);
        }
        done += m;
    }
    return ECB_OK;
}

int ecb_push_cells(ecb_handle* h, const uint32_t* meta, uint64_t first_read, size_t n) {
    return push_cells(h, meta, first_read, n, hipMemcpyHostToDevice);
}

int ecb_push_cells_device(ecb_handle* h, const void* d_meta, uint64_t first_read, size_t n) {
    return push_cells(h, d_meta, first_read, n, hipMemcpyDeviceToDevice);
}

int ecb_finalize(ecb_handle* h, ecb_sizes* out) {
    if (!h || !out) return ECB_ERR_ARG;
    RCCHK(refused_run(h));
    HIPCHK(h, hipSetDevice(h->device));
    if (h->run.origin == Origin::ASSEMBLED) { *out = h->run.sizes; return ECB_OK; }
    if (!h->has_result()) {
        if (h->open_read()) RCCHK(stage_and_process(h, nullptr, nullptr, nullptr, nullptr, 0));
        if (!h->ctr_synced) RCCHK(sync_counters(h));
    }
    const u64 E = h->n_ecs();
    const u64 valid = h->hctr.valid + h->run.extra_valid;
    RCCHK(refuse_no_ecs(h, E, valid));
    h->run.csr = {};
    const u64 total_reads = h->run.n_reads + h->run.extra_reads;
    const u64 words = bitmap_words(total_reads), lines = words / BM_LINE;
    const u64 nnz_max = std::min<u64>(E * INL + arena_used(h), (1ull << 32) - 1);
    u32 *bitmap = nullptr, *wpop = nullptr, *wprefix = nullptr, *ord2_raw = nullptr;
    uint2* list_fn = nullptr;
    u64* d_tot = nullptr;
    POOL(h, P_BITMAP, bitmap, words); POOL(h, P_WPOP, wpop, lines); POOL(h, P_WPREFIX, wprefix, lines);
    POOL(h, P_ROWLEN, ord2_raw, 2 * E); POOL(h, P_LISTFN, list_fn, E);
    uint2* ord2 = reinterpret_cast<uint2*>(ord2_raw);
    POOL(h, P_ORDER, h->run.csr.order, E);
    POOL(h, P_INDPTR, h->run.csr.indptr, E + 1); POOL(h, P_COUNTS, h->run.csr.counts, E);
    POOL(h, P_INDICES, h->run.csr.indices, nnz_max); POOL(h, P_DATA, h->run.csr.data, nnz_max);
    POOL(h, P_TOTALS, d_tot, 8);
    u32* big = nullptr;
    POOL(h, P_MS_X, big, E);
    u32* d_nbig = reinterpret_cast<u32*>(d_tot + 3);
    HIPCHK(h, hipMemsetAsync(bitmap, 0, words * 4, h->stream));
    HIPCHK(h, hipMemsetAsync(d_tot, 0, 8 * sizeof(u64), h->stream));
    bool listed = false;
    if (h->can_push() && h->run.n_reads) {
        u32* list = nullptr;
        POOL(h, P_LIST, list, E);
        const CompactSink sink{list, E, d_tot, bitmap, total_reads, list_fn};
        RCCHK(ensure_counts(h, &sink, &listed));
    } else if (!h->has_result()) {
        RCCHK(ensure_counts(h));
    }
    if (!listed) {
        if (!h->has_result() && h->run.d_list_n)
            k_list_fn<<<nblk(E, TPB), TPB, 0, h->stream>>>(h->table, h->slot_list(), E, h->run.d_list_n, d_tot, bitmap, total_reads, list_fn);
        else
            RCCHK(compact_table_dev(h, d_tot, bitmap, total_reads, list_fn));
    }
    k_popc<<<nblk(lines, TPB), TPB, 0, h->stream>>>(bitmap, lines, wpop);
    RCCHK(excl_scan_dev(h, wpop, lines, wprefix, d_tot + 1));
    k_rank<<<nblk(E, TPB), TPB, 0, h->stream>>>(h->slot_list(), list_fn, E, total_reads, bitmap, wprefix, ord2);
    RCCHK(excl_scan_dev(h, ord2_raw + 1, E, h->run.csr.indptr, d_tot + 2, 2, h->run.csr.indptr + E));
    k_emit_small<<<nblk(E, TPB), TPB, 0, h->stream>>>(h->table, ord2, h->run.csr.order, E, h->arena, h->run.csr.indptr, h->run.csr.indices, h->run.csr.data,
                                                       h->run.csr.counts, h->cfg.n_loci, h->cfg.n_haplotypes, big, d_nbig, h->ctr);
    k_emit_big<<<(unsigned)std::min<u64>(nblk(E * 64, TPB), 2048), TPB, 0, h->stream>>>(h->table, h->run.csr.order, big, d_nbig, h->arena, h->run.csr.indptr,
                                                                                       h->run.csr.indices, h->run.csr.data, h->cfg.n_loci, h->cfg.n_haplotypes, h->ctr);
    u64* const tot = h->pin_out->tot;
    HIPCHK(h, hipMemcpyAsync(tot, d_tot, 4 * sizeof(u64), hipMemcpyDeviceToHost, h->stream));
    RCCHK(run_refused(h, sync_counters(h)));
    h->run.n_list = tot[0];
    if (tot[0] != E) return fail(h, ECB_ERR_HIP, "internal: %llu occupied slots but %llu ECs created", (unsigned long long)tot[0], (unsigned long long)E);
    if (tot[1] != E) return fail(h, ECB_ERR_HIP, "internal: %llu distinct first-appearance indices for %llu ECs", (unsigned long long)tot[1], (unsigned long long)E);
    RCCHK(refuse_nnz(h, tot[2]));
    h->run.sizes = result_sizes(E, tot[2], h->hctr.all + h->run.extra_all, valid, total_reads);
    if (h->multisample()) {
        if (h->run.origin == Origin::ADOPTED) {
            h->run.tri.n = 0; h->run.sizes.n_samples = 0; h->run.sizes.nnz_n = 0;
        } else {
            if (h->run.extra_reads) return fail(h, ECB_ERR_STATE, "multisample across GPUs: adopt the merged ECs (ecb_table_adopt_device), then ecb_ms_adopt_triples_device");
            RCCHK(ensure_slot_ranks(h, E));
            RCCHK(ms_reduce(h, h->run.csr.rank_of_slot));
            h->run.sizes.n_samples = 0; h->run.sizes.nnz_n = h->run.tri.n;
        }
    }
    h->run.stage = Stage::FINAL;
    *out = h->run.sizes;
    return ECB_OK;
}

int ecb_export_firsts_device(ecb_handle* h, void* d_firsts) {
    if (!h || !d_firsts) return ECB_ERR_ARG;
    RCCHK(refused_run(h));
    if (!h->has_result() || h->run.origin == Origin::ASSEMBLED) return fail(h, ECB_ERR_STATE, "first reads are exported from a finalized table");
    HIPCHK(h, hipSetDevice(h->device));
    const u64 E = h->run.sizes.n_ecs;
    k_export_firsts<<<nblk(E, TPB), TPB, 0, h->stream>>>(h->table, h->run.csr.order, E, (u32*)d_firsts);
    HIPCHK(h, hipStreamSynchronize(h->stream));
    return ECB_OK;
}

int ecb_assemble_ranges_device(ecb_handle* h, uint32_t n_pieces, const void* const* d_indptr, const void* const* d_indices,
                               const void* const* d_data, const void* const* d_counts, const void* const* d_firsts,
                               const uint64_t* n_ecs, const uint64_t* nnz, uint64_t total_reads, uint64_t all_alignments,
                               uint64_t valid_alignments, ecb_sizes* out) {
    if (!h || !out) return ECB_ERR_ARG;
    RCCHK(refused_run(h));
    if (h->has_result() || h->run.origin == Origin::ADOPTED || !h->holds_nothing()) return fail(h, ECB_ERR_STATE, "assembling needs an empty handle");
    if (n_pieces && (!d_indptr || !d_indices || !d_data || !d_counts || !d_firsts || !n_ecs || !nnz)) return fail(h, ECB_ERR_ARG, "null piece lists");
    if (n_pieces > 65535u) return fail(h, ECB_ERR_LIMIT, "at most 65535 pieces");
    u64 E = 0, NNZ = 0;
    for (u32 q = 0; q < n_pieces; ++q) {
        if (n_ecs[q] && (!d_indptr[q] || !d_counts[q] || !d_firsts[q] || (nnz[q] && (!d_indices[q] || !d_data[q])))) return fail(h, ECB_ERR_ARG, "null piece buffers");
        E += n_ecs[q]; NNZ += nnz[q];
    }
    RCCHK(refuse_no_ecs(h, E, valid_alignments));
    RCCHK(refuse_nnz(h, NNZ));
    if (total_reads >= (1ull << 32) - 1) return fail(h, ECB_ERR_LIMIT, "more than 2^32-2 reads in total");
    HIPCHK(h, hipSetDevice(h->device));
    h->run.csr = {};
    const u64 words = bitmap_words(total_reads), lines = words / BM_LINE;
    u32 *bitmap = nullptr, *wpop = nullptr, *wprefix = nullptr, *place_raw = nullptr;
    u64* d_tot = nullptr;
    POOL(h, P_BITMAP, bitmap, words); POOL(h, P_WPOP, wpop, lines); POOL(h, P_WPREFIX, wprefix, lines);
    POOL(h, P_ROWLEN, place_raw, 4 * E);
    uint4* place = reinterpret_cast<uint4*>(place_raw);
    POOL(h, P_INDPTR, h->run.csr.indptr, E + 1); POOL(h, P_COUNTS, h->run.csr.counts, E);
    POOL(h, P_INDICES, h->run.csr.indices, std::max<u64>(NNZ, 1)); POOL(h, P_DATA, h->run.csr.data, std::max<u64>(NNZ, 1));
    POOL(h, P_TOTALS, d_tot, 8);
    HIPCHK(h, hipMemsetAsync(bitmap, 0, words * 4, h->stream));
    HIPCHK(h, hipMemsetAsync(d_tot, 0, 8 * sizeof(u64), h->stream));
    HIPCHK(h, hipMemsetAsync(place_raw, 0, E * 16, h->stream));
    RCCHK(clear_counters(h));
    std::vector<PieceDesc> desc;
    u64 most = 0;
    for (u32 q = 0, at = 0; q < n_pieces; ++q) {
        if (!n_ecs[q]) continue;
        desc.push_back(PieceDesc{(const u32*)d_firsts[q], (const int*)d_indptr[q], (const int*)d_indices[q], (const int*)d_data[q], (const int*)d_counts[q],
                                 n_ecs[q], nnz[q], at});
        at += n_ecs[q]; most = std::max<u64>(most, n_ecs[q]);
    }
    u64* d_desc_raw = nullptr;
    POOL(h, P_PARTS, d_desc_raw, desc.size() * sizeof(PieceDesc) / sizeof(u64));
    const PieceDesc* d_desc = reinterpret_cast<const PieceDesc*>(d_desc_raw);
    HIPCHK(h, hipMemcpyAsync(d_desc_raw, desc.data(), desc.size() * sizeof(PieceDesc), hipMemcpyHostToDevice, h->stream));
    const dim3 grid((unsigned)nblk(most, TPB), (unsigned)desc.size());
    k_mark_bits<<<grid, TPB, 0, h->stream>>>(d_desc, total_reads, bitmap, h->ctr);
    k_popc<<<nblk(lines, TPB), TPB, 0, h->stream>>>(bitmap, lines, wpop);
    RCCHK(excl_scan_dev(h, wpop, lines, wprefix, d_tot + 1));
    k_piece_place<<<grid, TPB, 0, h->stream>>>(d_desc, E, total_reads, bitmap, wprefix, place, h->ctr);
    RCCHK(excl_scan_dev(h, place_raw + 1, E, h->run.csr.indptr, d_tot + 2, 4, h->run.csr.indptr + E));
    k_piece_rows<<<nblk(E, TPB), TPB, 0, h->stream>>>(d_desc, (u32)desc.size(), place, E, h->run.csr.indptr, h->run.csr.indices, h->run.csr.data, h->run.csr.counts);
    u64 tot[8];
    HIPCHK(h, hipMemcpyAsync(tot, d_tot, sizeof(tot), hipMemcpyDeviceToHost, h->stream));
    h->ctr_synced = false;
    const int rc = sync_counters(h);
    if (rc == ECB_ERR_CONTRACT) return fail(h, rc, "a piece is malformed: a first read beyond the run's reads, or row offsets that are not its own");
    RCCHK(rc);
    if (tot[1] != E) return fail(h, ECB_ERR_CONTRACT, "the pieces hold %llu ECs but %llu distinct first reads: ranges overlap or a first read is missing",
                                 (unsigned long long)E, (unsigned long long)tot[1]);
    if (tot[2] != NNZ) return fail(h, ECB_ERR_HIP, "internal: %llu non-zeros placed, %llu received", (unsigned long long)tot[2], (unsigned long long)NNZ);
    h->run.sizes = result_sizes(E, NNZ, all_alignments, valid_alignments, total_reads);
    if (h->multisample()) { h->run.sizes.n_samples = 0; h->run.sizes.nnz_n = 0; h->run.tri.n = 0; h->run.triples = Triples::NONE; }
    h->run.stage = Stage::FINAL; h->run.origin = Origin::ASSEMBLED;
    *out = h->run.sizes;
    return ECB_OK;
}

int ecb_export_device(ecb_handle* h, void* ia, void* ja, void* da, void* in_, void* jn, void* dn) {
    if (!h) return ECB_ERR_ARG;
    RCCHK(refused_run(h));
    if (!h->has_result()) return fail(h, ECB_ERR_STATE, "export before finalize");
    return export_result(h, ia, ja, da, in_, jn, dn, hipMemcpyDeviceToDevice);
}

int ecb_export(ecb_handle* h, int32_t* ia, int32_t* ja, int32_t* da, int32_t* in_, int32_t* jn, int32_t* dn) {
    if (!h) return ECB_ERR_ARG;
    RCCHK(refused_run(h));
    if (!h->has_result()) return fail(h, ECB_ERR_STATE, "export before finalize");
    if (h->multisample() && (in_ || jn || dn))
        return fail(h, ECB_ERR_STATE, "multisample: N comes from ecb_export_pairs");
    return export_result(h, ia, ja, da, in_, jn, dn, hipMemcpyDeviceToHost);
}

int ecb_export_ranges(ecb_handle* h, int64_t* out) {
    if (!h || !out) return ECB_ERR_ARG;
    RCCHK(refused_run(h));
    if (!(h->cfg.flags & ECB_F_RANGES)) return fail(h, ECB_ERR_STATE, "handle was created without ECB_F_RANGES");
    HIPCHK(h, hipSetDevice(h->device));
    const u64 ns = (u64)h->cfg.n_loci * h->cfg.n_haplotypes;
    long long* d = nullptr;
    POOL(h, P_EXPORT, d, ns);
    k_range_len<<<nblk(ns, TPB), TPB, 0, h->stream>>>(h->rng, ns, d);
    HIPCHK(h, hipMemcpyAsync(out, d, ns * 8, hipMemcpyDeviceToHost, h->stream));
    HIPCHK(h, hipStreamSynchronize(h->stream));
    return ECB_OK;
}

int ecb_export_range_minmax(ecb_handle* h, int32_t* mn, int32_t* mx) {
    if (!h || !mn || !mx) return ECB_ERR_ARG;
    RCCHK(refused_run(h));
    if (!(h->cfg.flags & ECB_F_RANGES)) return fail(h, ECB_ERR_STATE, "handle was created without ECB_F_RANGES");
    HIPCHK(h, hipSetDevice(h->device));
    const u64 ns = (u64)h->cfg.n_loci * h->cfg.n_haplotypes;
    int* d = nullptr;
    POOL(h, P_EXPORT, d, 2 * ns);
    k_split_minmax<<<nblk(ns, TPB), TPB, 0, h->stream>>>(h->rng, ns, d, d + ns);
    HIPCHK(h, hipMemcpyAsync(mn, d, ns * 4, hipMemcpyDeviceToHost, h->stream));
    HIPCHK(h, hipMemcpyAsync(mx, d + ns, ns * 4, hipMemcpyDeviceToHost, h->stream));
    HIPCHK(h, hipStreamSynchronize(h->stream));
    return ECB_OK;
}

int ecb_export_pairs(ecb_handle* h, uint32_t* ec, uint32_t* meta, uint32_t* count, uint32_t* first_read) {
    if (!h || !ec || !meta || !count || !first_read) return ECB_ERR_ARG;
    RCCHK(refused_run(h));
    if (!h->has_ms_result()) return fail(h, ECB_ERR_STATE, "no multisample result");
    HIPCHK(h, hipSetDevice(h->device));
    const u64 nt = h->run.tri.n;
    u32* x = nullptr;
    POOL(h, P_MS_X, x, 3 * nt);
    if (h->awaits_triples()) return fail(h, ECB_ERR_STATE, "multisample across GPUs: no triples adopted yet (ecb_ms_adopt_triples_device)");
    k_ms_split<<<nblk(nt, TPB), TPB, 0, h->stream>>>(h->run.tri.okey, h->run.tri.ostart, h->run.tri.ocount, nt, x, x + nt, x + 2 * nt);
    HIPCHK(h, hipMemcpyAsync(ec, x, nt * 4, hipMemcpyDeviceToHost, h->stream));
    HIPCHK(h, hipMemcpyAsync(meta, x + nt, nt * 4, hipMemcpyDeviceToHost, h->stream));
    HIPCHK(h, hipMemcpyAsync(count, x + 2 * nt, nt * 4, hipMemcpyDeviceToHost, h->stream));
    HIPCHK(h, hipMemcpyAsync(first_read, h->run.tri.ofirst, nt * 4, hipMemcpyDeviceToHost, h->stream));
    HIPCHK(h, hipStreamSynchronize(h->stream));
    return ECB_OK;
}

int ecb_export_read_ec(ecb_handle* h, int32_t* out) {
    if (!h || !out) return ECB_ERR_ARG;
    RCCHK(refused_run(h));
    if (!h->has_result()) return fail(h, ECB_ERR_STATE, "export before finalize");
    if (h->run.extra_reads || h->run.origin == Origin::ASSEMBLED) return fail(h, ECB_ERR_STATE, "per-read EC ids are not kept across a multi-GPU merge");
    HIPCHK(h, hipSetDevice(h->device));
    int* d = nullptr;
    POOL(h, P_EXPORT, d, h->run.n_reads);
    RCCHK(ensure_slot_ranks(h, h->run.sizes.n_ecs));
    k_read_ec<<<nblk(h->run.n_reads, TPB), TPB, 0, h->stream>>>(h->read_slot, h->run.n_reads, h->run.csr.rank_of_slot, d);
    HIPCHK(h, hipMemcpyAsync(out, d, h->run.n_reads * 4, hipMemcpyDeviceToHost, h->stream));
    HIPCHK(h, hipStreamSynchronize(h->stream));
    return ECB_OK;
}

int ecb_table_sizes(ecb_handle* h, uint64_t* n_entries, uint64_t* n_pairs, uint64_t* n_reads) {
    if (!h) return ECB_ERR_ARG;
    RCCHK(refused_run(h));
    HIPCHK(h, hipSetDevice(h->device));
    if (h->open_read()) RCCHK(stage_and_process(h, nullptr, nullptr, nullptr, nullptr, 0));
    RCCHK(sync_counters(h));
    RCCHK(ensure_counts(h));
    if (n_entries) *n_entries = h->n_ecs();
    if (n_pairs) *n_pairs = h->n_ecs() * INL + arena_used(h);
    if (n_reads) *n_reads = h->run.n_reads;
    return ECB_OK;
}

int ecb_table_export_device(ecb_handle* h, void* d_entries, void* d_pairs, uint64_t read_base) {
    uint64_t eo[2], po[2];
    return ecb_table_export_parts_device(h, d_entries, d_pairs, read_base, 1, eo, po);
}

int ecb_table_merge_batch_device(ecb_handle* h, uint32_t n_tables, const void* const* d_entries, const uint64_t* n_entries,
                                const void* const* d_pairs, const uint64_t* n_pairs) {
    if (!h) return ECB_ERR_ARG;
    RCCHK(refused_run(h));
    if (h->has_result()) return fail(h, ECB_ERR_STATE, "merge after finalize");
    if (h->run.origin == Origin::ADOPTED) return fail(h, ECB_ERR_STATE, "merge into a table that adopted entries");
    if (n_tables && (!d_entries || !n_entries || !d_pairs || !n_pairs)) return fail(h, ECB_ERR_ARG, "null table lists");
    u64 total = 0;
    for (u32 t = 0; t < n_tables; ++t) {
        if (n_entries[t] && (!d_entries[t] || (n_pairs[t] && !d_pairs[t]))) return fail(h, ECB_ERR_ARG, "null table buffers");
        total += n_entries[t];
    }
    if (!total) return ECB_OK;
    HIPCHK(h, hipSetDevice(h->device));
    RCCHK(sync_counters(h));
    RCCHK(ensure_counts(h));
    while ((h->n_ecs() + total) * 2 > h->cap) { RCCHK(grow_table(h, h->cap * 4)); }
    HIPCHK(h, hipMemsetAsync(&h->ctr->n_queue, 0, sizeof(u64), h->stream));
    u32* mlist = nullptr;
    const u64 list_need = h->n_ecs() + total;
    if (h->n_ecs() == 0 || (h->run.d_list_n && h->pool[ecb_handle::P_LIST].bytes >= list_need * sizeof(u32))) {
        const bool fresh = h->n_ecs() == 0;
        POOL(h, P_LIST, mlist, list_need);
        if (fresh) { POOL(h, P_CNT, h->run.d_list_n, 1); HIPCHK(h, hipMemsetAsync(h->run.d_list_n, 0, sizeof(u64), h->stream)); }
    } else
        h->run.d_list_n = nullptr;
    std::vector<MergeDesc> desc;
    u64 most = 0;
    for (u32 t = 0; t < n_tables; ++t)
        if (n_entries[t]) { desc.push_back(MergeDesc{(const Entry*)d_entries[t], (const uint2*)d_pairs[t], n_entries[t], n_pairs[t]}); most = std::max<u64>(most, n_entries[t]); }
    if (desc.size() > 65535u) return fail(h, ECB_ERR_LIMIT, "at most 65535 tables per call");
    u64* d_desc = nullptr;
    POOL(h, P_PARTS, d_desc, desc.size() * sizeof(MergeDesc) / sizeof(u64));
    HIPCHK(h, hipMemcpyAsync(d_desc, desc.data(), desc.size() * sizeof(MergeDesc), hipMemcpyHostToDevice, h->stream));
    k_merge<<<dim3((unsigned)nblk(most, MERGE_PER_BLOCK), (unsigned)desc.size()), TPB, 0, h->stream>>>(reinterpret_cast<const MergeDesc*>(d_desc), h->table, h->cap - 1,
                                                                                                        h->arena, h->arena_cap, h->ctr,
                                                                                                        mlist, list_need, h->run.d_list_n);
    RCCHK(run_refused(h, sync_counters(h)));
    if (h->hctr.n_queue) return run_refused(h, fail(h, ECB_ERR_TABLE_FULL, "internal: merge found no slot in a half-empty table"));
    return ECB_OK;
}

int ecb_table_rebase_device(ecb_handle* h, void* d_entries, uint64_t n_entries, uint64_t read_base) {
    if (!h || (n_entries && !d_entries)) return ECB_ERR_ARG;
    RCCHK(refused_run(h));
    if (read_base >= (1ull << 32) - 1) return fail(h, ECB_ERR_LIMIT, "more than 2^32-2 reads in total");
    if (!n_entries || !read_base) return ECB_OK;
    HIPCHK(h, hipSetDevice(h->device));
    k_rebase<<<nblk(n_entries, TPB), TPB, 0, h->stream>>>((Entry*)d_entries, n_entries, (u32)read_base, (u32)((1ull << 32) - 1 - read_base), h->ctr);
    h->ctr_synced = false;
    return ECB_OK;
}

int ecb_table_merge_device(ecb_handle* h, const void* d_entries, uint64_t n_entries, const void* d_pairs, uint64_t n_pairs) {
    return ecb_table_merge_batch_device(h, 1, &d_entries, &n_entries, &d_pairs, &n_pairs);
}

int ecb_table_export_parts_device(ecb_handle* h, void* d_entries, void* d_pairs, uint64_t read_base, uint32_t n_parts,
                                  uint64_t* entry_offsets, uint64_t* pair_offsets) {
    if (!h || !d_entries || !d_pairs || !entry_offsets || !pair_offsets) return ECB_ERR_ARG;
    RCCHK(refused_run(h));
    if (n_parts == 0 || n_parts > MAX_PARTS) return fail(h, ECB_ERR_LIMIT, "1 .. %u parts", MAX_PARTS);
    HIPCHK(h, hipSetDevice(h->device));
    RCCHK(sync_counters(h));
    if (read_base + h->run.n_reads >= (1ull << 32) - 1) return fail(h, ECB_ERR_LIMIT, "more than 2^32-2 reads in total");
    RCCHK(ensure_counts(h));
    RCCHK(compact_table(h));
    const u64 E = h->n_ecs();
    u64* d_cnt = nullptr;
    POOL(h, P_PARTS, d_cnt, 3 * (u64)n_parts);
    HIPCHK(h, hipMemsetAsync(d_cnt, 0, 2 * n_parts * sizeof(u64), h->stream));
    if (E) k_parts_count<<<nblk(E, PARTS_PER_BLOCK), TPB, 0, h->stream>>>(h->table, h->slot_list(), E, n_parts, d_cnt);
    std::vector<u64> cnt(2 * n_parts), cur(3 * n_parts);
    HIPCHK(h, hipMemcpyAsync(cnt.data(), d_cnt, 2 * n_parts * sizeof(u64), hipMemcpyDeviceToHost, h->stream));
    HIPCHK(h, hipStreamSynchronize(h->stream));
    entry_offsets[0] = pair_offsets[0] = 0;
    for (u32 q = 0; q < n_parts; ++q) {
        entry_offsets[q + 1] = entry_offsets[q] + cnt[q];
        pair_offsets[q + 1] = pair_offsets[q] + cnt[n_parts + q];
        cur[q] = entry_offsets[q]; cur[n_parts + q] = pair_offsets[q]; cur[2 * n_parts + q] = pair_offsets[q];
    }
    HIPCHK(h, hipMemcpyAsync(d_cnt, cur.data(), 3 * n_parts * sizeof(u64), hipMemcpyHostToDevice, h->stream));
    if (E) {
        u64* big = nullptr;
        POOL(h, P_BIG, big, 2 * E + 1);
        u32* d_nbig = reinterpret_cast<u32*>(big + 2 * E);
        HIPCHK(h, hipMemsetAsync(d_nbig, 0, sizeof(u64), h->stream));
        k_parts_export<<<nblk(E, PARTS_PER_BLOCK), TPB, 0, h->stream>>>(h->table, h->slot_list(), E, h->arena, n_parts, d_cnt, d_cnt + 2 * n_parts,
                                                                   (Entry*)d_entries, (uint2*)d_pairs, (u32)read_base, big, d_nbig);
        u32 n_big = 0;
        HIPCHK(h, hipMemcpyAsync(&n_big, d_nbig, sizeof(u32), hipMemcpyDeviceToHost, h->stream));
        HIPCHK(h, hipStreamSynchronize(h->stream));
        if (n_big) k_parts_sort_big<<<nblk((u64)n_big * 64, TPB), TPB, 0, h->stream>>>(h->table, h->arena, big, n_big, (uint2*)d_pairs);
    }
    HIPCHK(h, hipStreamSynchronize(h->stream));
    return ECB_OK;
}

int ecb_table_adopt_batch_device(ecb_handle* h, uint32_t n_tables, const void* const* d_entries, const uint64_t* n_entries,
                                const void* const* d_pairs, const uint64_t* n_pairs) {
    if (!h) return ECB_ERR_ARG;
    RCCHK(refused_run(h));
// ... 2237 lines not shown
```

Before: 318.5 billion.

## Queue gated partition kernels during counter sync and fold memsets into kernels

While the host waits on the counter readback after the final stream launch, the partition pipeline (histogram, scan, scatter, work build) is enqueued speculatively. A device-side gate makes those kernels return early when the counters show the batch is incomplete. Separate memsets and the pinned StreamCold H2D copy are folded into the init kernel and into the clearing of scan words inside the preceding kernels, which cuts launch and copy overhead. This adds complexity and risks wasted or stale work if the gate and host validity checks fall out of step.

```diff
diff --git a/alntools_amd/csrc/ecb.hip b/alntools_amd/csrc/ecb.hip
--- a/alntools_amd/csrc/ecb.hip
+++ b/alntools_amd/csrc/ecb.hip
@@ -376,11 +376,27 @@
 #undef ECB_KS_PAR
 #undef ECB_KS_SHORT
 
-__global__ void k_init_resume(u64* resume, u64 slices, u64 chunk, Counters* ctr = nullptr) {
-    const u64 b = blockIdx.x * (u64)blockDim.x + threadIdx.x;
+__global__ void k_init_resume(u64* resume, u64 slices, u64 chunk, Counters* ctr, StreamCold* d_cold, const StreamCold cold, u64* wave_arena, u64 wa_words,
+                              u32* wave_counts, u64 wc_words) {
+    const u64 b = blockIdx.x * (u64)blockDim.x + threadIdx.x, T = gridDim.x * (u64)blockDim.x;
     if (b < slices) { resume[2 * b] = b * chunk; resume[2 * b + 1] = b * chunk; }
-    if (b == 0 && ctr) { ctr->n_queue = 0; ctr->full = 0; ctr->next_slice = 0; }
-    if (b < QSTRIPES && ctr) ctr->n_queue_s[b] = 0;
+    if (b == 0) {
+        ctr->n_queue = 0; ctr->full = 0; ctr->next_slice = 0;
+        if (wave_counts) ctr->n_mismatch = 0;
+        *d_cold = cold;
+    }
+    if (b < QSTRIPES) ctr->n_queue_s[b] = 0;
+    for (u64 i = b; i < wa_words; i += T) wave_arena[i] = 0;
+    for (u64 i = b; i < wc_words; i += T) wave_counts[i] = 0;
+}
+
+struct Gate { const Counters* ctr; u64 reads; };
+__device__ __forceinline__ bool gate_shut(const Gate g) {
+    if (!g.ctr) return false;
+    return g.ctr->err != 0u || g.ctr->full != 0u || g.ctr->n_queue != 0ull || (u64)(u32)(g.ctr->last_rid + 1u) != g.reads;
+}
+__device__ __forceinline__ void clear_scan_words(u64* sc, u32 sc_n) {
+    for (u64 i = blockIdx.x * (u64)blockDim.x + threadIdx.x; i < sc_n; i += gridDim.x * (u64)blockDim.x) sc[i] = 0;
 }
 
 __global__ __launch_bounds__(1024) void k_sum_counts(const u32* wave_counts, u64 waves, Counters* ctr, u32 verify, u64 offered, u64 queue_cap, const u32* d_last = nullptr) {
@@ -419,8 +435,10 @@
 constexpr int TPB_PART = 1024;
 constexpr u32 PART_G = 512;
 __device__ __forceinline__ u64 part_per(u64 n_reads, u64 G) { return (((n_reads + G - 1) / G) + 3ull) & ~3ull; }
-__global__ __launch_bounds__(TPB_PART) void k_part_hist(const u32* read_slot, u64 n_reads, u32 n_buckets, u32 bb, u32* hist) {
+__global__ __launch_bounds__(TPB_PART) void k_part_hist(const u32* read_slot, u64 n_reads, u32 n_buckets, u32 bb, u32* hist, u64* sc, u32 sc_n, const Gate gate) {
     extern __shared__ u32 sh[];
+    if (gate_shut(gate)) return;
+    clear_scan_words(sc, sc_n);
     const u64 G = gridDim.x, g = blockIdx.x, per = part_per(n_reads, G);
     const u64 r0 = min(g * per, n_reads), r1 = min(r0 + per, n_reads);
     for (u32 b = threadIdx.x; b < n_buckets; b += TPB_PART) sh[b] = 0;
@@ -440,8 +458,9 @@
 }
 
 __global__ __launch_bounds__(TPB_PART) void k_part_scatter(const u32* read_slot, u64 n_reads, u32 n_buckets, u32 bb, const u32* offs,
-                                                      u16* pairs) {
+                                                      u16* pairs, const Gate gate) {
     extern __shared__ u32 sh[];
+    if (gate_shut(gate)) return;
     const u64 G = gridDim.x, g = blockIdx.x, per = part_per(n_reads, G);
     const u64 r0 = min(g * per, n_reads), r1 = min(r0 + per, n_reads);
     for (u32 b = threadIdx.x; b < n_buckets; b += TPB_PART) sh[b] = offs[(u64)b * G + g];
@@ -464,8 +483,9 @@
 constexpr u32 STAGE = 8 * TPB_PART;
 constexpr u32 STAGE_MAX_BUCKETS = 4096;
 __global__ __launch_bounds__(TPB_PART) void k_part_scatter_staged(const u32* read_slot, u64 n_reads, u32 n_buckets, u32 bb, const u32* offs,
-                                                             u16* pairs) {
+                                                             u16* pairs, const Gate gate) {
     extern __shared__ u32 sh[];
+    if (gate_shut(gate)) return;
     u32 *cnt = sh, *start = sh + n_buckets, *gcur = sh + 2 * n_buckets;
     u32* stage = sh + 3 * n_buckets;
     __shared__ u32 s_wave[TPB_PART / 64];
@@ -519,9 +539,11 @@
 
 constexpr int TPB_COUNT = 1024;
 struct CountWork { u32 bucket, start, end, shared; };
-__global__ __launch_bounds__(1024) void k_build_work(const u32* offs, u32 G, const u64* total, u32 n_buckets, u32 piece, CountWork* work, u32 max_work, u32* n_work) {
+__global__ __launch_bounds__(1024) void k_build_work(const u32* offs, u32 G, const u64* total, u32 n_buckets, u32 piece, CountWork* work, u32 max_work, u32* n_work,
+                                                    const Gate gate) {
     __shared__ u32 s_w[16];
     __shared__ u32 s_carry;
+    if (gate_shut(gate)) return;
     const u32 tid = threadIdx.x, lane = tid & 63u, w = tid >> 6;
     if (tid == 0) s_carry = 0;
     __syncthreads();
@@ -1152,7 +1174,13 @@
 
 constexpr u32 BM_LINE = 16;
 inline u64 bitmap_words(u64 n_bits) { return ((n_bits + 31) / 32 + BM_LINE) / BM_LINE * BM_LINE; }
-__global__ void k_popc(const u32* in, u64 n_lines, u32* out) {
+__global__ void k_clear_bitmap(uint4* bitmap16, u64 n16, u64* tot) {
+    const u64 t = blockIdx.x * (u64)blockDim.x + threadIdx.x;
+    for (u64 i = t; i < n16; i += gridDim.x * (u64)blockDim.x) bitmap16[i] = make_uint4(0u, 0u, 0u, 0u);
+    if (t < 8) tot[t] = 0;
+}
+__global__ void k_popc(const u32* in, u64 n_lines, u32* out, u64* sc = nullptr, u32 sc_n = 0) {
+    clear_scan_words(sc, sc_n);
     const u64 i = blockIdx.x * (u64)blockDim.x + threadIdx.x;
     if (i >= n_lines) return;
     const uint4* q = reinterpret_cast<const uint4*>(in + i * BM_LINE);
@@ -1177,9 +1205,10 @@
 constexpr u64 SC_AGG = 1ull << 62, SC_PFX = 2ull << 62, SC_VAL = (1ull << 62) - 1ull;
 inline u64 scan_blocks(u64 n) { return std::max<u64>(1, (n + SCB - 1) / SCB); }
 inline u64 scan_words(u64 n) { return 2 * (scan_blocks(n) + 2); }
-__global__ __launch_bounds__(SCB_TPB) void k_scan_lb(const u32* in, u64 n, u32* out, u64* st, u64 nb, u64* d_total, u32 stride, u32* last32) {
+__global__ __launch_bounds__(SCB_TPB) void k_scan_lb(const u32* in, u64 n, u32* out, u64* st, u64 nb, u64* d_total, u32 stride, u32* last32, const Gate gate) {
     __shared__ u64 s_b, s_excl;
     __shared__ u32 s_w[SCB_TPB / 64];
+    if (gate_shut(gate)) return;
     const u32 tid = threadIdx.x, lane = tid & 63u, w = tid >> 6;
     if (tid == 0) s_b = atomicAdd(reinterpret_cast<unsigned long long*>(&st[nb]), 1ull);
     __syncthreads();
@@ -1252,17 +1281,21 @@
         for (int k = 0; k < SCB_ITEMS; ++k) { if (base + k < n) out[base + k] = run; run += v[k]; }
     }
 }
-inline hipError_t scan_launch(hipStream_t st, const u32* in, u64 n, u32* out, u32* scratch, u64* d_total, u32 stride = 1, u32* last32 = nullptr) {
+inline hipError_t scan_launch(hipStream_t st, const u32* in, u64 n, u32* out, u32* scratch, u64* d_total, u32 stride = 1, u32* last32 = nullptr,
+                              bool cleared = false, const Gate gate = Gate{nullptr, 0}) {
     const u64 nb = scan_blocks(n);
     u64* words = reinterpret_cast<u64*>(scratch);
-    hipError_t e = hipMemsetAsync(words, 0, ((nb + 1) * 8 + 15) & ~15ull, st);
-    if (e != hipSuccess) return e;
-    k_scan_lb<<<(unsigned)nb, SCB_TPB, 0, st>>>(in, n, out, words, nb, d_total, stride, last32);
+    if (!cleared) {
+        hipError_t e = hipMemsetAsync(words, 0, ((nb + 1) * 8 + 15) & ~15ull, st);
+        if (e != hipSuccess) return e;
+    }
+    k_scan_lb<<<(unsigned)nb, SCB_TPB, 0, st>>>(in, n, out, words, nb, d_total, stride, last32, gate);
     return hipGetLastError();
 }
 
 __global__ void k_rank(const u32* list, const uint2* list_fn, u64 n, u64 n_bits, const u32* bitmap, const u32* wprefix,
-                       uint2* ord2) {
+                       uint2* ord2, u64* sc, u32 sc_n) {
+    clear_scan_words(sc, sc_n);
     const u64 e = blockIdx.x * (u64)blockDim.x + threadIdx.x;
     if (e >= n) return;
     const u32 si = list[e];
@@ -2124,6 +2157,8 @@
     hipStream_t stream = nullptr;
     std::string err;
     u64 wave_arena_n = 0;
+    bool wave_arena_stale = false;
+    hipEvent_t ev_ctr = nullptr;
     bool scatter_attr_set = false, count_attr_set = false;
     u64 resident_blocks[SV_VERIFY] = {}, rounds = 24, min_tiles = 32;
     bool par_stream = false;
@@ -2154,6 +2189,8 @@
         std::string refusal;
         std::vector<u32> c_rid, c_loc, c_hf; std::vector<int> c_pos;
         u64* d_list_n = nullptr;
+        struct Partition { bool valid = false; u64 reads = 0, cap = 0; u32 bb = 0, max_work = 0; const u16* pairs = nullptr;
+                           const CountWork* work = nullptr; const u32* n_work = nullptr; } part;
         struct Csr { u32 *order = nullptr, *rank_of_slot = nullptr , *indptr = nullptr;
                      int *indices = nullptr, *data = nullptr, *counts = nullptr; } csr;
         u64 n_list = 0;
@@ -2187,7 +2224,6 @@
     DevBuf<u32> st_rid;
     DevBuf<> pool[P_N];
     DevBuf<StreamCold> d_cold;
-    Pinned<StreamCold> pin_cold;
     Pinned<PinOut> pin_out;
     Pinned<Counters> pin_ctr;
     DevBuf<u64> wave_arena;
@@ -2202,6 +2238,7 @@
     ~ecb_handle() {
         if (ev0) hipEventDestroy(ev0);
         if (ev1) hipEventDestroy(ev1);
+        if (ev_ctr) hipEventDestroy(ev_ctr);
         if (stream) hipStreamDestroy(stream);
     }
 };
@@ -2302,7 +2339,7 @@
     HIPCHK_AS(h, "grow_table: ", hipStreamSynchronize(h->stream));
     HIPCHK(h, h->table.reset());
     h->table = std::move(nt);
-    h->cap = new_cap; h->run.d_list_n = nullptr;
+    h->cap = new_cap; h->run.d_list_n = nullptr; h->run.part = {};
     return ECB_OK;
 }
 
@@ -2359,6 +2396,21 @@
 }
 
 int excl_scan(ecb_handle* h, const u32* in, u64 n, u32* out, u64* total);
+int queue_partition(ecb_handle* h, u64 R, const Gate gate, ecb_handle::Run::Partition* P);
+
+int sync_counters_ahead(ecb_handle* h, u64 R, ecb_handle::Run::Partition* P, bool* queued) {
+    HIPCHK(h, hipMemcpyAsync(&h->pin_out->c, h->ctr, sizeof(Counters), hipMemcpyDeviceToHost, h->stream));
+    HIPCHK(h, hipEventRecord(h->ev_ctr, h->stream));
+    {
+        const std::string text = h->err;
+        *queued = queue_partition(h, R, Gate{h->ctr, R}, P) == ECB_OK;
+        if (!*queued) { hipGetLastError(); h->err = text; }
+    }
+    HIPCHK(h, hipEventSynchronize(h->ev_ctr));
+    h->hctr = h->pin_out->c;
+    h->ctr_synced = true;
+    return refuse_bits(h, COUNTER_ERRS, h->hctr.err, h->arena_cap);
+}
 
 struct StreamVariantRow { void (*kernel)(StreamArgs); const char* name; int blocks_per_cu; };
 const StreamVariantRow STREAM_VARIANTS[SV_N] = {
@@ -2436,21 +2488,19 @@
     int2* const rng = verify ? nullptr : (int2*)h->rng;
     u64* d_resume = nullptr; u32* d_wcounts = nullptr;
     POOL(h, P_RESUME, d_resume, 2 * P.slices);
-    if (!launch) k_init_resume<<<nblk(P.slices, TPB), TPB, 0, h->stream>>>(d_resume, P.slices, P.chunk, verify ? nullptr : (Counters*)h->ctr);
+    if (!launch && !verify && h->wave_arena_n < P.pwaves) {
+        HIPCHK(h, h->wave_arena.grow(2 * P.pwaves * sizeof(u64), 0, 2 * h->wave_arena_n * sizeof(u64), h->stream));
+        h->wave_arena_n = P.pwaves;
+    }
     POOL(h, P_WCOUNTS, d_wcounts, 3 * P.pwaves);
     if (launch) RCCHK(zero_launch_words(h));
     else {
-        if (verify) {
-            HIPCHK(h, hipMemsetAsync(d_wcounts, 0, 3 * P.pwaves * sizeof(u32), h->stream));
-            RCCHK(zero_launch_words(h));
-            HIPCHK(h, hipMemsetAsync(&h->ctr->n_mismatch, 0, sizeof(u64), h->stream));
-        } else if (h->wave_arena_n < P.pwaves) {
-            HIPCHK(h, h->wave_arena.grow(2 * P.pwaves * sizeof(u64), 0, 2 * h->wave_arena_n * sizeof(u64), h->stream));
-            h->wave_arena_n = P.pwaves;
-        }
-        *h->pin_cold = StreamCold{h->arena, h->arena_cap, h->queue, h->queue_cap, d_resume, d_wcounts, verify ? nullptr : (u64*)h->wave_arena, timing,
-                                  P.chunk, prev_rid, d_pos, rng, verify ? 0u : h->cfg.n_loci, verify ? 0u : h->cfg.n_haplotypes};
-        HIPCHK(h, hipMemcpyAsync(h->d_cold, h->pin_cold.get(), sizeof(StreamCold), hipMemcpyHostToDevice, h->stream));
+        const bool wa = !verify && h->wave_arena_stale;
+        const StreamCold cold{h->arena, h->arena_cap, h->queue, h->queue_cap, d_resume, d_wcounts, verify ? nullptr : (u64*)h->wave_arena, timing,
+                              P.chunk, prev_rid, d_pos, rng, verify ? 0u : h->cfg.n_loci, verify ? 0u : h->cfg.n_haplotypes};
+        k_init_resume<<<nblk(P.slices, TPB), TPB, 0, h->stream>>>(d_resume, P.slices, P.chunk, h->ctr, h->d_cold, cold, wa ? (u64*)h->wave_arena : nullptr,
+                                                                 wa ? 2 * h->wave_arena_n : 0, verify ? d_wcounts : nullptr, verify ? 3 * P.pwaves : 0);
+        if (wa) h->wave_arena_stale = false;
     }
     const StreamArgs a{d_rid, d_loc, d_hf, n, h->table, h->cap - 1, h->ctr, h->read_slot, h->run.reads_hi, h->d_cold,
                        !verify && getenv("ECB_ABLATE") ? (u32)atoi(getenv("ECB_ABLATE")) : 0u, d_pos, rng};
@@ -2513,12 +2563,21 @@
 #endif
     h->ctr_synced = false;
     *launched = true;
+    h->run.part = {};
+    const bool ahead = hinted && reads_after == h->reads_hint && h->run.records_pushed + n >= reads_after && !getenv("ECB_NO_COUNT_AHEAD");
+    ecb_handle::Run::Partition part_ahead;
+    bool part_queued = false;
     const u64 probe_before = h->hctr.n_probe_tiles;
     int rc = ECB_OK;
     for (u32 launch = 0;; ++launch) {
         rc = launch_stream(h, v, P, d_rid, d_loc, d_hf, d_pos, n, h->run.prev_rid, d_rid + rec_at(n - 1, tw), launch, launch ? 0 : n, timing);
         if (rc != ECB_OK) break;
-        rc = sync_counters(h);
+        if (ahead && !launch) {
+            rc = sync_counters_ahead(h, reads_after, &part_ahead, &part_queued);
+            part_queued = part_queued && h->hctr.err == 0u && h->hctr.full == 0u && h->hctr.n_queue == 0ull &&
+                          (u64)(u32)(h->hctr.last_rid + 1u) == reads_after;
+        } else
+            rc = sync_counters(h);
         if (h->prof) {
             float ms = 0; hipEventElapsedTime(&ms, h->ev0, h->ev1);
             h->prof_ms += ms; h->prof_launches += 1;
@@ -2563,6 +2622,7 @@
     h->run.prev_rid = last_rid;
     h->run.n_reads = reads_after;
     h->run.records_pushed += n;
+    if (part_queued && part_ahead.reads == reads_after && part_ahead.cap == h->cap) { h->run.part = part_ahead; h->run.part.valid = true; }
     return ECB_OK;
 }
 int process_batch(ecb_handle* h, const u32* d_rid, const u32* d_loc, const u32* d_hf, const int* d_pos, u64 n, u32 tw = 512u) {
@@ -2600,10 +2660,18 @@
     return process_batch(h, h->st_rid, h->st_loc, h->st_hf, rg ? h->st_pos : nullptr, n);
 }
 
-int excl_scan_dev(ecb_handle* h, const u32* in, u64 n, u32* out, u64* d_total, u32 stride = 1, u32* last32 = nullptr) {
+int excl_scan_dev(ecb_handle* h, const u32* in, u64 n, u32* out, u64* d_total, u32 stride = 1, u32* last32 = nullptr, bool cleared = false,
+                  const Gate gate = Gate{nullptr, 0}) {
     u32* sums = nullptr;
     POOL(h, P_SUMS, sums, scan_words(n));
-    HIPCHK(h, scan_launch(h->stream, in, n, out, sums, d_total, stride, last32));
+    HIPCHK(h, scan_launch(h->stream, in, n, out, sums, d_total, stride, last32, cleared, gate));
+    return ECB_OK;
+}
+int scan_words_dev(ecb_handle* h, u64 n, u64** sc, u32* sc_n) {
+    u32* sums = nullptr;
+    POOL(h, P_SUMS, sums, scan_words(n));
+    *sc = reinterpret_cast<u64*>(sums);
+    *sc_n = (u32)(scan_blocks(n) + 1);
     return ECB_OK;
 }
 int excl_scan(ecb_handle* h, const u32* in, u64 n, u32* out, u64* total) {
@@ -2683,6 +2751,54 @@
     return ECB_OK;
 }
 
+int queue_partition(ecb_handle* h, u64 R, const Gate gate, ecb_handle::Run::Partition* P) {
+    u32 bb = BIN_BITS;
+    {
+        u32 lc = 0;
+        while ((1ull << (lc + 1)) <= h->cap) ++lc;
+        bb = std::min<u32>(std::max<u32>(lc, 9u + MIN_BIN_BITS) - 9u, BIN_BITS);
+    }
+    if (const char* e = getenv("ECB_BIN_BITS")) bb = (u32)std::min<long>(std::max<long>(atol(e), MIN_BIN_BITS), MAX_BIN_BITS);
+    while (bb < MAX_BIN_BITS && (h->cap >> bb) > MAX_BUCKETS) ++bb;
+    const u32 nb = (u32)std::max<u64>(1, h->cap >> bb);
+    if (nb > MAX_BUCKETS) return fail(h, ECB_ERR_LIMIT, "EC table larger than 2^28 slots is not supported");
+    if (bb > 14 && !h->count_attr_set) {
+        HIPCHK(h, hipFuncSetAttribute((const void*)k_count_bins, hipFuncAttributeMaxDynamicSharedMemorySize, 4 << MAX_BIN_BITS));
+        h->count_attr_set = true;
+    }
+    const u32 G = (u32)std::min<u64>(PART_G, (R + 4095) / 4096);
+    u32 *hist = nullptr, *offs = nullptr;
+    u16* pairs = nullptr;
+    u64 *d_tot = nullptr, *sc = nullptr;
+    u32 sc_n = 0;
+    POOL(h, P_HIST, hist, (u64)nb * G); POOL(h, P_OFFS, offs, (u64)nb * G);
+    POOL(h, P_PAIRS, pairs, R);
+    POOL(h, P_TOTALS, d_tot, 8);
+    RCCHK(scan_words_dev(h, (u64)nb * G, &sc, &sc_n));
+    k_part_hist<<<G, TPB_PART, nb * 4, h->stream>>>(h->read_slot, R, nb, bb, hist, sc, sc_n, gate);
+    d_tot += 6;
+    RCCHK(excl_scan_dev(h, hist, (u64)nb * G, offs, d_tot, 1, nullptr, true, gate));
+    if (nb <= STAGE_MAX_BUCKETS) {
+        if (!h->scatter_attr_set) {
+            HIPCHK(h, hipFuncSetAttribute((const void*)k_part_scatter_staged, hipFuncAttributeMaxDynamicSharedMemorySize,
+                                          3 * STAGE_MAX_BUCKETS * 4 + STAGE * 4));
+            h->scatter_attr_set = true;
+        }
+        k_part_scatter_staged<<<G, TPB_PART, 3 * nb * 4 + STAGE * 4, h->stream>>>(h->read_slot, R, nb, bb, offs, pairs, gate);
+    } else
+        k_part_scatter<<<G, TPB_PART, nb * 4, h->stream>>>(h->read_slot, R, nb, bb, offs, pairs, gate);
+    const u32 piece = std::max<u32>(32768u, 2u * (u32)((R + nb - 1) / nb));
+    const u32 max_work = nb + (u32)(R / piece) + 1;
+    CountWork* d_work = nullptr;
+    POOL(h, P_WORK, d_work, (u64)max_work + 1);
+    u32* d_nwork = reinterpret_cast<u32*>(d_work + max_work);
+    k_build_work<<<1, 1024, 0, h->stream>>>(offs, G, d_tot, nb, piece, d_work, max_work, d_nwork, gate);
+    HIPCHK(h, hipGetLastError());
+    P->valid = false; P->reads = R; P->cap = h->cap; P->bb = bb; P->max_work = max_work;
+    P->pairs = pairs; P->work = d_work; P->n_work = d_nwork;
+    return ECB_OK;
+}
+
 int ensure_counts(ecb_handle* h, const CompactSink* sink = nullptr, bool* listed = nullptr) {
     if (h->counted()) return ECB_OK;
     const u64 R = h->run.n_reads;
@@ -2697,46 +2813,10 @@
         sink = &own;
     }
     if (R) {
-        u32 bb = BIN_BITS;
-        {
-            u32 lc = 0;
-            while ((1ull << (lc + 1)) <= h->cap) ++lc;
-            bb = std::min<u32>(std::max<u32>(lc, 9u + MIN_BIN_BITS) - 9u, BIN_BITS);
-        }
-        if (const char* e = getenv("ECB_BIN_BITS")) bb = (u32)std::min<long>(std::max<long>(atol(e), MIN_BIN_BITS), MAX_BIN_BITS);
-        while (bb < MAX_BIN_BITS && (h->cap >> bb) > MAX_BUCKETS) ++bb;
-        const u32 nb = (u32)std::max<u64>(1, h->cap >> bb);
-        if (nb > MAX_BUCKETS) return fail(h, ECB_ERR_LIMIT, "EC table larger than 2^28 slots is not supported");
-        if (bb > 14 && !h->count_attr_set) {
-            HIPCHK(h, hipFuncSetAttribute((const void*)k_count_bins, hipFuncAttributeMaxDynamicSharedMemorySize, 4 << MAX_BIN_BITS));
-            h->count_attr_set = true;
-        }
-        const u32 G = (u32)std::min<u64>(PART_G, (R + 4095) / 4096);
-        u32 *hist = nullptr, *offs = nullptr;
-        u16* pairs = nullptr;
-        u64* d_tot = nullptr;
-        POOL(h, P_HIST, hist, (u64)nb * G); POOL(h, P_OFFS, offs, (u64)nb * G);
-        POOL(h, P_PAIRS, pairs, R);
-        POOL(h, P_TOTALS, d_tot, 8);
-        k_part_hist<<<G, TPB_PART, nb * 4, h->stream>>>(h->read_slot, R, nb, bb, hist);
-        d_tot += 6;
-        RCCHK(excl_scan_dev(h, hist, (u64)nb * G, offs, d_tot));
-        if (nb <= STAGE_MAX_BUCKETS) {
-            if (!h->scatter_attr_set) {
-                HIPCHK(h, hipFuncSetAttribute((const void*)k_part_scatter_staged, hipFuncAttributeMaxDynamicSharedMemorySize,
-                                              3 * STAGE_MAX_BUCKETS * 4 + STAGE * 4));
-                h->scatter_attr_set = true;
-            }
-            k_part_scatter_staged<<<G, TPB_PART, 3 * nb * 4 + STAGE * 4, h->stream>>>(h->read_slot, R, nb, bb, offs, pairs);
-        } else
-            k_part_scatter<<<G, TPB_PART, nb * 4, h->stream>>>(h->read_slot, R, nb, bb, offs, pairs);
-        const u32 piece = std::max<u32>(32768u, 2u * (u32)((R + nb - 1) / nb));
-        const u32 max_work = nb + (u32)(R / piece) + 1;
-        CountWork* d_work = nullptr;
-        POOL(h, P_WORK, d_work, (u64)max_work + 1);
-        u32* d_nwork = reinterpret_cast<u32*>(d_work + max_work);
-        k_build_work<<<1, 1024, 0, h->stream>>>(offs, G, d_tot, nb, piece, d_work, max_work, d_nwork);
-        k_count_bins<<<max_work, TPB_COUNT, 4u << bb, h->stream>>>(pairs, d_work, d_nwork, bb, h->table, sink ? *sink : CompactSink{nullptr, 0, nullptr, nullptr, 0, nullptr});
+        ecb_handle::Run::Partition P = h->run.part;
+        if (!P.valid || P.reads != R || P.cap != h->cap) RCCHK(queue_partition(h, R, Gate{nullptr, 0}, &P));
+        h->run.part = {};
+        k_count_bins<<<P.max_work, TPB_COUNT, 4u << P.bb, h->stream>>>(P.pairs, P.work, P.n_work, P.bb, h->table, sink ? *sink : CompactSink{nullptr, 0, nullptr, nullptr, 0, nullptr});
         if (sink == &own) h->run.d_list_n = own.n_list;
         else if (sink && listed) *listed = true;
         HIPCHK(h, hipGetLastError());
@@ -2943,7 +3023,6 @@
     CREATECHK(h->arena.alloc(h->arena_cap * sizeof(uint2)));
     CREATECHK(h->ctr.alloc(sizeof(Counters)));
     CREATECHK(pin(h->pin_ctr));
-    CREATECHK(pin(h->pin_cold));
     CREATECHK(pin(h->pin_out));
     CREATECHK(h->d_cold.alloc(sizeof(StreamCold)));
     CREATECHK(hipMemsetAsync(h->table, 0, h->cap * sizeof(Slot), h->stream));
@@ -2955,6 +3034,7 @@
         k_fill_minmax<<<nblk(ns, TPB), TPB, 0, h->stream>>>(h->rng, ns);
     }
     hipEventCreate(&h->ev0); hipEventCreate(&h->ev1);
+    CREATECHK(hipEventCreateWithFlags(&h->ev_ctr, hipEventDisableTiming));
     CREATECHK(hipStreamSynchronize(h->stream));
 #undef CREATECHK
     *out = owner.release();
@@ -3018,7 +3098,7 @@
     if (poison && h->pool[ecb_handle::P_LIST].p)
         HIPCHK(h, hipMemsetAsync(h->pool[ecb_handle::P_LIST].p, POISON_BYTE, h->pool[ecb_handle::P_LIST].bytes, h->stream));
     RCCHK(clear_counters(h));
-    if (h->wave_arena) HIPCHK(h, hipMemsetAsync(h->wave_arena, 0, 2 * h->wave_arena_n * sizeof(u64), h->stream));
+    if (h->wave_arena) h->wave_arena_stale = true;
     if ((h->cfg.flags & ECB_F_VERIFY) && h->read_slot) HIPCHK(h, hipMemsetAsync(h->read_slot, 0xFF, h->read_slot_cap * sizeof(u32), h->stream));
     if (h->rng) {
         const u64 ns = (u64)h->cfg.n_loci * h->cfg.n_haplotypes;
@@ -3131,8 +3211,7 @@
     u32* big = nullptr;
     POOL(h, P_MS_X, big, E);
     u32* d_nbig = reinterpret_cast<u32*>(d_tot + 3);
-    HIPCHK(h, hipMemsetAsync(bitmap, 0, words * 4, h->stream));
-    HIPCHK(h, hipMemsetAsync(d_tot, 0, 8 * sizeof(u64), h->stream));
+    k_clear_bitmap<<<(unsigned)std::min<u64>(nblk(words / 4, TPB), 2048), TPB, 0, h->stream>>>(reinterpret_cast<uint4*>(bitmap), words / 4, d_tot);
     bool listed = false;
     if (h->can_push() && h->run.n_reads) {
         u32* list = nullptr;
@@ -3148,10 +3227,14 @@
         else
             RCCHK(compact_table_dev(h, d_tot, bitmap, total_reads, list_fn));
     }
-    k_popc<<<nblk(lines, TPB), TPB, 0, h->stream>>>(bitmap, lines, wpop);
-    RCCHK(excl_scan_dev(h, wpop, lines, wprefix, d_tot + 1));
-    k_rank<<<nblk(E, TPB), TPB, 0, h->stream>>>(h->slot_list(), list_fn, E, total_reads, bitmap, wprefix, ord2);
-    RCCHK(excl_scan_dev(h, ord2_raw + 1, E, h->run.csr.indptr, d_tot + 2, 2, h->run.csr.indptr + E));
+    u64* sc = nullptr;
+    u32 sc_n = 0;
+    RCCHK(scan_words_dev(h, lines, &sc, &sc_n));
+    k_popc<<<nblk(lines, TPB), TPB, 0, h->stream>>>(bitmap, lines, wpop, sc, sc_n);
+    RCCHK(excl_scan_dev(h, wpop, lines, wprefix, d_tot + 1, 1, nullptr, true));
+    RCCHK(scan_words_dev(h, E, &sc, &sc_n));
+    k_rank<<<nblk(E, TPB), TPB, 0, h->stream>>>(h->slot_list(), list_fn, E, total_reads, bitmap, wprefix, ord2, sc, sc_n);
+    RCCHK(excl_scan_dev(h, ord2_raw + 1, E, h->run.csr.indptr, d_tot + 2, 2, h->run.csr.indptr + E, true));
     k_emit_small<<<nblk(E, TPB), TPB, 0, h->stream>>>(h->table, ord2, h->run.csr.order, E, h->arena, h->run.csr.indptr, h->run.csr.indices, h->run.csr.data,
                                                        h->run.csr.counts, h->cfg.n_loci, h->cfg.n_haplotypes, big, d_nbig, h->ctr);
     k_emit_big<<<(unsigned)std::min<u64>(nblk(E * 64, TPB), 2048), TPB, 0, h->stream>>>(h->table, h->run.csr.order, big, d_nbig, h->arena, h->run.csr.indptr,
```

Result: no change. 319.7 billion, median of 6 (+0.4%).
